# deepomicslab/PALACE

Measured on AMD Instinct MI355X. Metric: contigs/sec eref+generate_graph+matching, 1M-contig synth, 1/2/4/8 GPU, higher is better.
Workload: dtype u32

## Files before the change

include/palace_hip.h:

```cpp
#ifndef PALACE_HIP_H
#define PALACE_HIP_H

#include <stddef.h>
#include <stdint.h>

#ifdef __cplusplus
extern "C" {
#endif

#define PALACE_OK 0
#define PALACE_EINVAL (-1)
#define PALACE_EHIP (-2)
#define PALACE_ENOMEM (-3)
#define PALACE_ESTATE (-4)

typedef struct palace_ctx palace_ctx;

const char *palace_last_error(void);
const char *palace_version(void);

int palace_ctx_create(int device, palace_ctx **out);
int palace_ctx_create_prio(int device, int high_priority, palace_ctx **out);
int palace_ctx_create_on_stream(int device, void *hip_stream, palace_ctx **out);
int palace_ctx_destroy(palace_ctx *ctx);
int palace_sync(palace_ctx *ctx);
void *palace_stream(palace_ctx *ctx);
int palace_malloc(palace_ctx *ctx, size_t bytes, void **d_out);
int palace_free(palace_ctx *ctx, void *d_ptr);
int palace_memset(palace_ctx *ctx, void *d_ptr, int value, size_t bytes);
int palace_h2d(palace_ctx *ctx, void *d_dst, const void *h_src, size_t bytes);
int palace_d2h(palace_ctx *ctx, void *h_dst, const void *d_src, size_t bytes);
int palace_d2d(palace_ctx *ctx, void *d_dst, const void *d_src, size_t bytes);
int palace_host_alloc(palace_ctx *ctx, size_t bytes, void **h_out);
int palace_host_free(palace_ctx *ctx, void *h_ptr);
int palace_h2d_async(palace_ctx *ctx, void *d_dst, const void *h_src, size_t bytes);
int palace_d2h_async(palace_ctx *ctx, void *h_dst, const void *d_src, size_t bytes);
int palace_timer_begin(palace_ctx *ctx);
int palace_timer_end(palace_ctx *ctx, float *ms_out);
int palace_mark(palace_ctx *ctx, int i);
int palace_mark_elapsed(palace_ctx *ctx, int a, int b, float *ms_out);
int palace_mark_wait(palace_ctx *ctx, int i);
int palace_mark_wait_for(palace_ctx *ctx, int i, double seconds);
int palace_wait_for_mark(palace_ctx *ctx, palace_ctx *other, int i);


int palace_eref_set_coder(palace_ctx *ctx, const uint8_t header400[400]);

int palace_eref_index_refs(palace_ctx *ctx, const uint8_t *d_bases, const int64_t *d_offsets,
                           int64_t n_refs, uint32_t *d_out, const int64_t *d_out_offsets);

int palace_eref_table_reset(palace_ctx *ctx);
int palace_eref_reserve(palace_ctx *ctx, int64_t total_bases);
int palace_eref_count_reads(palace_ctx *ctx, const uint8_t *d_bases, const int64_t *d_offsets,
                            int64_t n_reads, const uint8_t *d_keep, int64_t total_bases);

size_t palace_eref_packed_bytes(int64_t n_positions);
int palace_eref_pack_reads(palace_ctx *ctx, const uint8_t *d_bases, const int64_t *d_offsets, int64_t n_reads,
                           const uint8_t *d_keep, int64_t total_bases, uint32_t *d_p0, uint32_t *d_p1, uint32_t *d_u);
int palace_eref_count_reads_packed(palace_ctx *ctx, const uint32_t *d_p0, const uint32_t *d_p1, const uint32_t *d_u,
                                   int64_t n_positions, int64_t n_reads_hint);

int palace_eref_set_count_mode(palace_ctx *ctx, int mode, int64_t bucket_cap);
int palace_eref_set_key_buckets(palace_ctx *ctx, const uint32_t mask128[4]);
int palace_eref_set_option(palace_ctx *ctx, const char *name, int64_t value);

int palace_eref_scan_refs(palace_ctx *ctx, const uint8_t *d_bases, const int64_t *d_offsets,
                          int64_t n_refs, int64_t total_bases, int one_min, int three_min,
                          int32_t *d_rows);

typedef struct palace_eref_probe_index palace_eref_probe_index;
int palace_eref_probe_index_build(palace_ctx *ctx, const uint8_t *d_bases, const int64_t *d_offsets, int64_t n_refs,
                                  int64_t total_bases, palace_eref_probe_index **out);
int palace_eref_probe_index_free(palace_ctx *ctx, palace_eref_probe_index *ix);
int palace_eref_scan_refs_indexed(palace_ctx *ctx, const palace_eref_probe_index *ix, const uint8_t *d_bases,
                                  const int64_t *d_offsets, int64_t n_refs, int64_t total_bases, int one_min,
                                  int three_min, int32_t *d_rows);

int palace_eref_attach_probe_index(palace_ctx *ctx, const palace_eref_probe_index *ix);

int palace_eref_entry_layout(const palace_eref_probe_index *ix, size_t *counts_bytes, size_t *hits_bytes);
int palace_eref_entry_buffers_attach(palace_ctx *ctx, palace_eref_probe_index *ix, void *d_counts, void *d_hits);
int palace_eref_entry_buffers(const palace_eref_probe_index *ix, void **d_counts, void **d_hits);
int palace_eref_entry_hits_from_counts(palace_ctx *ctx, const palace_eref_probe_index *ix, const void *d_parts, int n_parts, size_t part_stride,
                                       size_t off, size_t bytes);
int palace_eref_entry_hits_complete(palace_ctx *ctx, const palace_eref_probe_index *ix, int64_t keys_counted);
int palace_eref_entry_counts_valid(const palace_ctx *ctx, const palace_eref_probe_index *ix);


int palace_eref_table_planes(palace_ctx *ctx, void **d_planes3, size_t *bytes_per_plane);
int palace_eref_table_attach(palace_ctx *ctx, void *const d_planes3[3]);
int palace_eref_table_invalidate(palace_ctx *ctx);
int palace_eref_table_merge_slices(palace_ctx *ctx, const void *d_parts, int n_parts,
                                   size_t slice_off, size_t slice_bytes);

int palace_eref_table_pack_low(palace_ctx *ctx, void *d_low);
int palace_eref_table_merge_slices_packed(palace_ctx *ctx, const void *d_parts, int n_parts, size_t slice_off,
                                          size_t slice_bytes);

int palace_eref_plane_pack(palace_ctx *ctx, const uint32_t mask128[4], uint32_t *d_counts, uint16_t *d_keys, int64_t cap_keys,
                           unsigned long long *d_first);
int palace_eref_plane_unpack(palace_ctx *ctx, const uint32_t mask128[4], const uint32_t *d_counts, const uint16_t *d_keys, int64_t cap_keys,
                             unsigned long long *d_first);

int palace_eref_table_lookup(palace_ctx *ctx, const uint32_t *d_keys, int64_t n, uint8_t *d_counts);
int palace_eref_table_popcounts(palace_ctx *ctx, uint64_t out3[3]);


typedef struct {
    int32_t max_end;
    int32_t min_mapq;
    int32_t max_nm;
    int32_t enable_paired;
    int32_t both_order;
    int32_t reserved;
    double max_span_frac;
} palace_graph_params;

typedef struct {
    int64_t n;
    const int32_t *tid, *pos, *mtid, *mpos, *nm, *ref_len, *read_len, *clip_s, *clip_e;
    const uint16_t *flag;
    const uint8_t *mapq;
    const uint64_t *qkey;
    const int32_t *sa_off;
} palace_bam_cols;

typedef struct {
    int32_t tid2, pos2, mapq2, nm2, clip_s2, clip_e2, len2, rev2;
} palace_sa_item;

typedef struct {
    int64_t ord;
    uint64_t qkey;
    int32_t left, right;
    int32_t mtid, ref_len;
    int32_t dL, dR;
    int32_t nmL, nmR;
    int16_t mapqL, mapqR;
    uint8_t kind, cls, found, in_fastg, oL, oR, pad0, pad1;
    int32_t sa_index;
} palace_graph_cand;

typedef struct {
    int32_t left, right;
    uint32_t counts[4];
    uint8_t oL, oR, pad[6];
} palace_graph_edge;

int palace_graph_classify(palace_ctx *ctx, const palace_bam_cols *cols, const palace_sa_item *d_sa,
                          int32_t n_targets, const int32_t *d_tlen, const int32_t *d_trank,
                          const uint64_t *d_fastg, int64_t n_fastg, const palace_graph_params *prm,
                          int64_t ord_base, uint64_t *d_consumed, palace_graph_cand *d_cands,
                          int64_t cand_cap, int64_t *n_cands_out);

int palace_graph_classify_ex(palace_ctx *ctx, const palace_bam_cols *cols, const palace_sa_item *d_sa,
                             int32_t n_targets, const int32_t *d_tlen, const int32_t *d_trank,
                             const uint64_t *d_fastg, int64_t n_fastg, const palace_graph_params *prm,
                             int64_t ord_base, uint64_t *d_consumed, palace_graph_cand *d_cands,
                             int64_t cand_cap, int64_t *n_cands_out, int64_t *n_border_out);

int palace_graph_fastg_offsets(palace_ctx *ctx, const uint64_t *d_fastg, int64_t n_fastg, int32_t n_targets, uint32_t *d_first);
int palace_graph_classify_ix(palace_ctx *ctx, const palace_bam_cols *cols, const palace_sa_item *d_sa,
                             int32_t n_targets, const int32_t *d_tlen, const int32_t *d_trank,
                             const uint64_t *d_fastg, int64_t n_fastg, const uint32_t *d_fastg_first, const palace_graph_params *prm,
                             int64_t ord_base, uint64_t *d_consumed, palace_graph_cand *d_cands,
                             int64_t cand_cap, int64_t *n_cands_out, int64_t *n_border_out);

int palace_graph_resolve(palace_ctx *ctx, palace_graph_cand *d_cands, int64_t n_cands,
                         int64_t n_records_total, const palace_graph_params *prm, uint64_t *d_consumed,
                         palace_graph_edge *d_edges, int64_t edge_cap, int64_t *n_edges_out);

int palace_graph_resolve_ex(palace_ctx *ctx, palace_graph_cand *d_cands, int64_t n_cands, int64_t n_border,
                            int64_t n_records_total, const palace_graph_params *prm, uint64_t *d_consumed,
                            palace_graph_edge *d_edges, int64_t edge_cap, int64_t *d_n_edges, int64_t *n_edges_out);

int palace_graph_score_border(palace_ctx *ctx, palace_graph_cand *d_cands, int64_t n_cands, int64_t n_border,
                              const palace_graph_params *prm);

int palace_graph_copy_numbers(palace_ctx *ctx, const uint64_t *d_consumed, const int32_t *d_tlen,
                              int32_t n_targets, double avg_depth, int32_t *d_cn);


int palace_bgzf_inflate(palace_ctx *ctx, const uint8_t *d_in, int64_t n_members, const int64_t *d_in_off, const int32_t *d_in_len,
                        const int64_t *d_out_off, const int32_t *d_out_len, uint8_t *d_out, int32_t *d_status);


int palace_bgzf_deflate(palace_ctx *ctx, const uint8_t *d_text, int64_t n_members, const int64_t *d_off, const int32_t *d_len,
                        const uint32_t *d_crc, uint8_t *d_slots, int32_t *d_member_len);

int palace_bgzf_compact(palace_ctx *ctx, const uint8_t *d_slots, int64_t n_members, const int32_t *d_member_len, uint8_t *d_file,
                        int64_t *d_member_off);


int palace_crc32_members(palace_ctx *ctx, const uint8_t *d_data, int64_t n_members, const int64_t *d_off, const int32_t *d_len,
                         uint32_t *d_crc);

typedef struct {
    int64_t line, reads, bases;
    int32_t open, error;
} palace_fastq_cursor;

size_t palace_fastq_scratch_bytes(int64_t max_window);
int palace_fastq_parse(palace_ctx *ctx, const uint8_t *d_text, int64_t n, int final_window, palace_fastq_cursor *d_cursor,
                       uint8_t *d_bases, int64_t bases_cap, int64_t *d_offsets, int64_t offsets_cap, void *d_scratch,
                       size_t scratch_bytes);


typedef struct {
    int64_t stride, span, text_cap;
    int64_t check_guards;
} palace_gzip_params;

enum {
    PALACE_GZ_NONE = 0,
    PALACE_GZ_HEADER = 1,
    PALACE_GZ_DECODE = 2,
    PALACE_GZ_CHAIN_OPEN = 3,
    PALACE_GZ_NO_PROGRESS = 4,
    PALACE_GZ_TOO_BIG = 5,
    PALACE_GZ_TRUNCATED = 6,
    PALACE_GZ_CRC = 7,
    PALACE_GZ_ISIZE = 8,
    PALACE_GZ_TRAILING = 9,
    PALACE_GZ_SINK = 10,
    PALACE_GZ_MARKER = 11
};

typedef struct {
    int64_t chunks_found, chunks_accepted, false_hits, rounds, members, spans, batches, text_bytes;
    int32_t fallback, guards_bad;
    double ms_upload, ms_find, ms_size, ms_decode, ms_chain, ms_resolve, ms_crc, ms_sink;
} palace_gzip_stats;

typedef int (*palace_gzip_sink)(void *user, const uint8_t *d_text, int64_t n, int last);

int palace_gzip_inflate(palace_ctx *ctx, const uint8_t *file, int64_t size, const palace_gzip_params *prm, palace_gzip_sink sink,
                        void *user, palace_gzip_stats *stats);


int palace_depth_sum_covered(palace_ctx *ctx, int64_t n_segs, const int32_t *d_seg_tid, const int32_t *d_seg_pos,
                             const int32_t *d_seg_len, int32_t n_targets, const int32_t *d_tlen, const int64_t *d_tbase,
                             int64_t total_len, uint64_t *sum_out, uint64_t *covered_out);

int palace_depth_per_contig(palace_ctx *ctx, int64_t n_segs, const int32_t *d_seg_tid, const int32_t *d_seg_pos,
                            const int32_t *d_seg_len, int32_t n_targets, const int32_t *d_tlen, const int64_t *d_tbase,
                            int64_t total_len, uint64_t *sum_out, uint64_t *covered_out, uint64_t *d_contig_sum,
                            uint64_t *d_contig_covered);

typedef struct palace_depth_text palace_depth_text;
int palace_depth_text_create(palace_ctx *ctx, int64_t n_segs, const int32_t *d_seg_tid, const int32_t *d_seg_pos,
                             const int32_t *d_seg_len, int32_t n_targets, const int32_t *d_tlen, const int64_t *d_tbase,
                             int64_t total_len, const uint8_t *d_names, const int64_t *d_name_off, palace_depth_text **out,
                             uint64_t *text_bytes_out, uint64_t *lines_out, uint64_t *sum_out);
int palace_depth_text_destroy(palace_ctx *ctx, palace_depth_text *dt);
int palace_depth_text_emit(palace_ctx *ctx, const palace_depth_text *dt, uint64_t text_begin, uint64_t text_end, uint8_t *d_out);
int palace_depth_text_windows(palace_ctx *ctx, const palace_depth_text *dt, int64_t n_windows, const int64_t *d_win_beg,
                              const int64_t *d_win_end, uint64_t *d_text_beg, uint64_t *d_text_end, uint64_t *d_lines);


int palace_match_greedy(palace_ctx *ctx, int32_t n_vertices, int64_t n_arcs, const int32_t *d_src,
                        const int32_t *d_dst, const int64_t *d_out_off, const int32_t *d_out_arcs,
                        const int64_t *d_in_off, const int32_t *d_in_arcs, const uint8_t *d_alive,
                        int32_t *d_next, int32_t *d_prev, int32_t *d_next_arc, int32_t *rounds_out);

int palace_match_arcs_from_edges(const int32_t *cn, int32_t n_segs, const palace_graph_edge *edges, int64_t n_edges,
                                 int32_t min_count, int64_t *copies, int32_t *src, int32_t *dst, int64_t *weight,
                                 int64_t *n_arcs_out);

typedef struct palace_match_result palace_match_result;
int palace_match_set_option(palace_ctx *ctx, const char *name, int64_t value);
int palace_match_decompose(palace_ctx *ctx, int32_t n_segs, const int64_t *copies, int64_t n_arcs,
                           const int32_t *src, const int32_t *dst, int32_t iterations, int32_t aggressive,
                           palace_match_result **out);
int palace_match_decompose_ex(palace_ctx *ctx, int32_t n_segs, const int64_t *copies, int64_t n_arcs,
                              const int32_t *src, const int32_t *dst, int32_t iterations, int32_t aggressive,
                              int32_t compact, palace_match_result **out);
const uint64_t *palace_match_result_bare(const palace_match_result *r);
int64_t palace_match_result_bare_count(const palace_match_result *r);
int64_t palace_match_result_count(const palace_match_result *r);
const int64_t *palace_match_result_offsets(const palace_match_result *r);
const int32_t *palace_match_result_verts(const palace_match_result *r);
const uint8_t *palace_match_result_kind(const palace_match_result *r);
const int32_t *palace_match_result_iter(const palace_match_result *r);
const int32_t *palace_match_result_open_at(const palace_match_result *r);
void palace_match_result_free(palace_match_result *r);


typedef struct {
    int32_t n_segs;
    int32_t min_count;
    const uint8_t *seed;
    const int32_t *tlen;
    const int32_t *rank;
    const int32_t *name_len;
    int64_t n_paths;
    const int64_t *path_off;
    const int32_t *path_tok;
} palace_stage04_inputs;

typedef struct palace_stage04 palace_stage04;
int palace_stage04_create(palace_ctx *ctx, const palace_stage04_inputs *in, palace_stage04 **out);
int palace_stage04_destroy(palace_ctx *ctx, palace_stage04 *s);

int palace_stage04_reserve(palace_ctx *ctx, palace_stage04 *s, int64_t edge_bound);

int palace_stage04_filter(palace_ctx *ctx, palace_stage04 *s, const palace_graph_edge *d_edges, const int64_t *d_n_edges,
                          int64_t edge_bound);
int palace_stage04_flags(palace_ctx *ctx, palace_stage04 *s, uint8_t *h_seg_flags, uint8_t *h_edge_flags, int64_t n_edges);
int palace_stage04_counts(palace_ctx *ctx, palace_stage04 *s, int64_t counts[8]);

int palace_stage04_match(palace_ctx *ctx, palace_stage04 *s, const palace_graph_edge *d_edges, const int32_t *d_cn,
                         int32_t iterations, int32_t aggressive, int32_t use_paths);
int palace_stage04_result(palace_ctx *ctx, palace_stage04 *s, palace_match_result **out, const int32_t **contig_of_out,
                          int64_t *n_segs_filtered_out);

#ifdef __cplusplus
}
#endif
#endif
```

palace_amd/capi.py:

```python
from __future__ import annotations

import ctypes as C
import os
import subprocess

import numpy as np

_HERE = os.path.dirname(os.path.abspath(__file__))
SO_PATH = os.environ.get("PALACE_HIP_SO") or os.path.join(_HERE, "libpalace_hip.so")
_LIB = None


class PalaceError(RuntimeError):
    pass


def build(force: bool = False) -> str:
    args = ["make", "-C", os.path.join(_HERE, "csrc")]
    if force:
        subprocess.run(args + ["clean"], check=True, stdout=subprocess.DEVNULL)
    subprocess.run(args, check=True, stdout=subprocess.DEVNULL)
    return SO_PATH


class GraphParams(C.Structure):
    _fields_ = [("max_end", C.c_int32), ("min_mapq", C.c_int32), ("max_nm", C.c_int32), ("enable_paired", C.c_int32),
                ("both_order", C.c_int32), ("reserved", C.c_int32), ("max_span_frac", C.c_double)]

    @classmethod
    def default(cls):
        return cls(300, 0, 5, 1, 0, 0, 0.80)


class BamCols(C.Structure):
    _fields_ = [("n", C.c_int64)] + [(k, C.c_void_p) for k in
                                     ("tid", "pos", "mtid", "mpos", "nm", "ref_len", "read_len", "clip_s", "clip_e",
                                      "flag", "mapq", "qkey", "sa_off")]


class GzipParams(C.Structure):
    _fields_ = [("stride", C.c_int64), ("span", C.c_int64), ("text_cap", C.c_int64), ("check_guards", C.c_int64)]


class GzipStats(C.Structure):
    _fields_ = [(k, C.c_int64) for k in ("chunks_found", "chunks_accepted", "false_hits", "rounds", "members", "spans", "batches", "text_bytes")] + \
        [("fallback", C.c_int32), ("guards_bad", C.c_int32)] + \
        [(k, C.c_double) for k in ("ms_upload", "ms_find", "ms_size", "ms_decode", "ms_chain", "ms_resolve", "ms_crc", "ms_sink")]


GZIP_SINK = C.CFUNCTYPE(C.c_int, C.c_void_p, C.c_void_p, C.c_int64, C.c_int)


class Stage04Inputs(C.Structure):
    _fields_ = [("n_segs", C.c_int32), ("min_count", C.c_int32), ("seed", C.c_void_p), ("tlen", C.c_void_p), ("rank", C.c_void_p),
                ("name_len", C.c_void_p), ("n_paths", C.c_int64), ("path_off", C.c_void_p), ("path_tok", C.c_void_p)]


SA_ITEM_DTYPE = np.dtype([(k, np.int32) for k in ("tid2", "pos2", "mapq2", "nm2", "clip_s2", "clip_e2", "len2", "rev2")])
CAND_DTYPE = np.dtype([("ord", np.int64), ("qkey", np.uint64), ("left", np.int32), ("right", np.int32),
                       ("mtid", np.int32), ("ref_len", np.int32), ("dL", np.int32), ("dR", np.int32),
                       ("nmL", np.int32), ("nmR", np.int32), ("mapqL", np.int16), ("mapqR", np.int16),
                       ("kind", np.uint8), ("cls", np.uint8), ("found", np.uint8), ("in_fastg", np.uint8),
                       ("oL", np.uint8), ("oR", np.uint8), ("pad0", np.uint8), ("pad1", np.uint8), ("sa_index", np.int32)])
EDGE_DTYPE = np.dtype([("left", np.int32), ("right", np.int32), ("counts", np.uint32, 4), ("oL", np.uint8),
                       ("oR", np.uint8), ("pad", np.uint8, 6)])
FASTQ_CURSOR_DTYPE = np.dtype([("line", np.int64), ("reads", np.int64), ("bases", np.int64), ("open", np.int32), ("error", np.int32)])
assert CAND_DTYPE.itemsize == 64 and EDGE_DTYPE.itemsize == 32 and SA_ITEM_DTYPE.itemsize == 32

_SIGS = {
    "palace_ctx_create": [C.c_int, C.POINTER(C.c_void_p)],
    "palace_ctx_create_prio": [C.c_int, C.c_int, C.POINTER(C.c_void_p)],
    "palace_ctx_create_on_stream": [C.c_int, C.c_void_p, C.POINTER(C.c_void_p)],
    "palace_ctx_destroy": [C.c_void_p],
    "palace_sync": [C.c_void_p],
    "palace_malloc": [C.c_void_p, C.c_size_t, C.POINTER(C.c_void_p)],
    "palace_free": [C.c_void_p, C.c_void_p],
    "palace_memset": [C.c_void_p, C.c_void_p, C.c_int, C.c_size_t],
    "palace_h2d": [C.c_void_p, C.c_void_p, C.c_void_p, C.c_size_t],
    "palace_d2h": [C.c_void_p, C.c_void_p, C.c_void_p, C.c_size_t],
    "palace_d2d": [C.c_void_p, C.c_void_p, C.c_void_p, C.c_size_t],
    "palace_host_alloc": [C.c_void_p, C.c_size_t, C.POINTER(C.c_void_p)],
    "palace_host_free": [C.c_void_p, C.c_void_p],
    "palace_d2h_async": [C.c_void_p, C.c_void_p, C.c_void_p, C.c_size_t],
    "palace_h2d_async": [C.c_void_p, C.c_void_p, C.c_void_p, C.c_size_t],
    "palace_mark_wait": [C.c_void_p, C.c_int],
    "palace_mark_wait_for": [C.c_void_p, C.c_int, C.c_double],
    "palace_wait_for_mark": [C.c_void_p, C.c_void_p, C.c_int],
    "palace_timer_begin": [C.c_void_p],
    "palace_timer_end": [C.c_void_p, C.POINTER(C.c_float)],
    "palace_mark": [C.c_void_p, C.c_int],
    "palace_mark_elapsed": [C.c_void_p, C.c_int, C.c_int, C.POINTER(C.c_float)],
    "palace_eref_set_coder": [C.c_void_p, C.c_void_p],
    "palace_eref_index_refs": [C.c_void_p, C.c_void_p, C.c_void_p, C.c_int64, C.c_void_p, C.c_void_p],
    "palace_eref_table_reset": [C.c_void_p],
    "palace_eref_reserve": [C.c_void_p, C.c_int64],
    "palace_eref_count_reads": [C.c_void_p, C.c_void_p, C.c_void_p, C.c_int64, C.c_void_p, C.c_int64],
    "palace_eref_pack_reads": [C.c_void_p, C.c_void_p, C.c_void_p, C.c_int64, C.c_void_p, C.c_int64, C.c_void_p, C.c_void_p, C.c_void_p],
    "palace_eref_count_reads_packed": [C.c_void_p, C.c_void_p, C.c_void_p, C.c_void_p, C.c_int64, C.c_int64],
    "palace_eref_set_count_mode": [C.c_void_p, C.c_int, C.c_int64],
    "palace_eref_set_key_buckets": [C.c_void_p, C.c_void_p],
    "palace_eref_set_option": [C.c_void_p, C.c_char_p, C.c_int64],
    "palace_eref_scan_refs": [C.c_void_p, C.c_void_p, C.c_void_p, C.c_int64, C.c_int64, C.c_int, C.c_int,
                              C.c_void_p],
    "palace_eref_probe_index_build": [C.c_void_p, C.c_void_p, C.c_void_p, C.c_int64, C.c_int64, C.POINTER(C.c_void_p)],
    "palace_eref_attach_probe_index": [C.c_void_p, C.c_void_p],
    "palace_eref_entry_layout": [C.c_void_p, C.POINTER(C.c_size_t), C.POINTER(C.c_size_t)],
    "palace_eref_entry_buffers_attach": [C.c_void_p, C.c_void_p, C.c_void_p, C.c_void_p],
    "palace_eref_entry_buffers": [C.c_void_p, C.POINTER(C.c_void_p), C.POINTER(C.c_void_p)],
    "palace_eref_entry_hits_from_counts": [C.c_void_p, C.c_void_p, C.c_void_p, C.c_int, C.c_size_t, C.c_size_t, C.c_size_t],
    "palace_eref_entry_hits_complete": [C.c_void_p, C.c_void_p, C.c_int64],
    "palace_eref_entry_counts_valid": [C.c_void_p, C.c_void_p],
    "palace_eref_probe_index_free": [C.c_void_p, C.c_void_p],
    "palace_eref_scan_refs_indexed": [C.c_void_p, C.c_void_p, C.c_void_p, C.c_void_p, C.c_int64, C.c_int64, C.c_int, C.c_int,
                                      C.c_void_p],
    "palace_eref_table_planes": [C.c_void_p, C.POINTER(C.c_void_p), C.POINTER(C.c_size_t)],
    "palace_eref_table_attach": [C.c_void_p, C.POINTER(C.c_void_p)],
    "palace_eref_table_invalidate": [C.c_void_p],
    "palace_eref_table_merge_slices": [C.c_void_p, C.c_void_p, C.c_int, C.c_size_t, C.c_size_t],
    "palace_eref_table_merge_slices_packed": [C.c_void_p, C.c_void_p, C.c_int, C.c_size_t, C.c_size_t],
    "palace_eref_table_pack_low": [C.c_void_p, C.c_void_p],
    "palace_eref_plane_pack": [C.c_void_p, C.c_void_p, C.c_void_p, C.c_void_p, C.c_int64, C.c_void_p],
    "palace_eref_plane_unpack": [C.c_void_p, C.c_void_p, C.c_void_p, C.c_void_p, C.c_int64, C.c_void_p],
    "palace_eref_table_lookup": [C.c_void_p, C.c_void_p, C.c_int64, C.c_void_p],
    "palace_eref_table_popcounts": [C.c_void_p, C.POINTER(C.c_uint64)],
    "palace_graph_classify": [C.c_void_p, C.POINTER(BamCols), C.c_void_p, C.c_int32, C.c_void_p, C.c_void_p,
                              C.c_void_p, C.c_int64, C.POINTER(GraphParams), C.c_int64, C.c_void_p, C.c_void_p,
                              C.c_int64, C.POINTER(C.c_int64)],
    "palace_depth_sum_covered": [C.c_void_p, C.c_int64, C.c_void_p, C.c_void_p, C.c_void_p, C.c_int32, C.c_void_p, C.c_void_p, C.c_int64,
                                 C.POINTER(C.c_uint64), C.POINTER(C.c_uint64)],
    "palace_depth_per_contig": [C.c_void_p, C.c_int64, C.c_void_p, C.c_void_p, C.c_void_p, C.c_int32, C.c_void_p, C.c_void_p, C.c_int64,
                                C.POINTER(C.c_uint64), C.POINTER(C.c_uint64), C.c_void_p, C.c_void_p],
    "palace_graph_copy_numbers": [C.c_void_p, C.c_void_p, C.c_void_p, C.c_int32, C.c_double, C.c_void_p],
    "palace_match_greedy": [C.c_void_p, C.c_int32, C.c_int64] + [C.c_void_p] * 10 + [C.POINTER(C.c_int32)],
    "palace_match_arcs_from_edges": [C.c_void_p, C.c_int32, C.c_void_p, C.c_int64, C.c_int32, C.c_void_p, C.c_void_p,
                                     C.c_void_p, C.c_void_p, C.POINTER(C.c_int64)],
    "palace_match_set_option": [C.c_void_p, C.c_char_p, C.c_int64],
    "palace_match_decompose": [C.c_void_p, C.c_int32, C.c_void_p, C.c_int64, C.c_void_p, C.c_void_p, C.c_int32,
                               C.c_int32, C.POINTER(C.c_void_p)],
    "palace_match_decompose_ex": [C.c_void_p, C.c_int32, C.c_void_p, C.c_int64, C.c_void_p, C.c_void_p, C.c_int32,
                                  C.c_int32, C.c_int32, C.POINTER(C.c_void_p)],
    "palace_graph_resolve": [C.c_void_p, C.c_void_p, C.c_int64, C.c_int64, C.POINTER(GraphParams), C.c_void_p,
                             C.c_void_p, C.c_int64, C.POINTER(C.c_int64)],
    "palace_graph_classify_ex": [C.c_void_p, C.POINTER(BamCols), C.c_void_p, C.c_int32, C.c_void_p, C.c_void_p,
                                 C.c_void_p, C.c_int64, C.POINTER(GraphParams), C.c_int64, C.c_void_p, C.c_void_p,
                                 C.c_int64, C.POINTER(C.c_int64), C.POINTER(C.c_int64)],
    "palace_graph_classify_ix": [C.c_void_p, C.POINTER(BamCols), C.c_void_p, C.c_int32, C.c_void_p, C.c_void_p,
                                 C.c_void_p, C.c_int64, C.c_void_p, C.POINTER(GraphParams), C.c_int64, C.c_void_p, C.c_void_p,
                                 C.c_int64, C.POINTER(C.c_int64), C.POINTER(C.c_int64)],
    "palace_graph_fastg_offsets": [C.c_void_p, C.c_void_p, C.c_int64, C.c_int32, C.c_void_p],
    "palace_bgzf_inflate": [C.c_void_p, C.c_void_p, C.c_int64, C.c_void_p, C.c_void_p, C.c_void_p, C.c_void_p, C.c_void_p, C.c_void_p],
    "palace_fastq_scratch_bytes": [C.c_int64],
    "palace_crc32_members": [C.c_void_p, C.c_void_p, C.c_int64, C.c_void_p, C.c_void_p, C.c_void_p],
    "palace_bgzf_deflate": [C.c_void_p, C.c_void_p, C.c_int64, C.c_void_p, C.c_void_p, C.c_void_p, C.c_void_p, C.c_void_p],
    "palace_bgzf_compact": [C.c_void_p, C.c_void_p, C.c_int64, C.c_void_p, C.c_void_p, C.c_void_p],
    "palace_depth_text_create": [C.c_void_p, C.c_int64, C.c_void_p, C.c_void_p, C.c_void_p, C.c_int32, C.c_void_p, C.c_void_p, C.c_int64,
                                 C.c_void_p, C.c_void_p, C.POINTER(C.c_void_p), C.POINTER(C.c_uint64), C.POINTER(C.c_uint64), C.POINTER(C.c_uint64)],
    "palace_depth_text_destroy": [C.c_void_p, C.c_void_p],
    "palace_depth_text_emit": [C.c_void_p, C.c_void_p, C.c_uint64, C.c_uint64, C.c_void_p],
    "palace_depth_text_windows": [C.c_void_p, C.c_void_p, C.c_int64, C.c_void_p, C.c_void_p, C.c_void_p, C.c_void_p, C.c_void_p],
    "palace_gzip_inflate": [C.c_void_p, C.c_void_p, C.c_int64, C.POINTER(GzipParams), GZIP_SINK, C.c_void_p, C.POINTER(GzipStats)],
    "palace_fastq_parse": [C.c_void_p, C.c_void_p, C.c_int64, C.c_int, C.c_void_p, C.c_void_p, C.c_int64, C.c_void_p, C.c_int64,
                           C.c_void_p, C.c_size_t],
    "palace_graph_score_border": [C.c_void_p, C.c_void_p, C.c_int64, C.c_int64, C.POINTER(GraphParams)],
    "palace_graph_resolve_ex": [C.c_void_p, C.c_void_p, C.c_int64, C.c_int64, C.c_int64, C.POINTER(GraphParams), C.c_void_p,
                                C.c_void_p, C.c_int64, C.c_void_p, C.POINTER(C.c_int64)],
    "palace_stage04_create": [C.c_void_p, C.POINTER(Stage04Inputs), C.POINTER(C.c_void_p)],
    "palace_stage04_destroy": [C.c_void_p, C.c_void_p],
    "palace_stage04_reserve": [C.c_void_p, C.c_void_p, C.c_int64],
    "palace_stage04_filter": [C.c_void_p, C.c_void_p, C.c_void_p, C.c_void_p, C.c_int64],
    "palace_stage04_flags": [C.c_void_p, C.c_void_p, C.c_void_p, C.c_void_p, C.c_int64],
    "palace_stage04_counts": [C.c_void_p, C.c_void_p, C.POINTER(C.c_int64)],
    "palace_stage04_match": [C.c_void_p, C.c_void_p, C.c_void_p, C.c_void_p, C.c_int32, C.c_int32, C.c_int32],
    "palace_stage04_result": [C.c_void_p, C.c_void_p, C.POINTER(C.c_void_p), C.POINTER(C.c_void_p), C.POINTER(C.c_int64)],
}


def declared_symbols():
    import re
    text = open(os.path.join(_HERE, "..", "include", "palace_hip.h")).read()
    text = re.sub(r"/\*.*?\*/", "", text, flags=re.S)
    return sorted(set(re.findall(r"\b(palace_[a-z0-9_]+)\s*\(", text)))


def lib() -> C.CDLL:
    global _LIB
    if _LIB is None:
        if not os.path.exists(SO_PATH):
            raise PalaceError(f"{SO_PATH} is missing: run `python -c 'import __graft_entry__ as g; g.build()'` "
                              "(hipcc --offload-arch=gfx950). There is no CPU fallback.")
        _LIB = C.CDLL(SO_PATH)
        _LIB.palace_last_error.restype = C.c_char_p
        _LIB.palace_version.restype = C.c_char_p
        _LIB.palace_stream.restype = C.c_void_p
        _LIB.palace_stream.argtypes = [C.c_void_p]
        _LIB.palace_eref_packed_bytes.restype = C.c_size_t
        _LIB.palace_eref_packed_bytes.argtypes = [C.c_int64]
        for nm, rt in (("count", C.c_int64), ("bare_count", C.c_int64), ("bare", C.POINTER(C.c_uint64)), ("offsets", C.POINTER(C.c_int64)), ("verts", C.POINTER(C.c_int32)),
                       ("kind", C.POINTER(C.c_uint8)), ("iter", C.POINTER(C.c_int32)), ("open_at", C.POINTER(C.c_int32))):
            fn = getattr(_LIB, "palace_match_result_" + nm)
            fn.argtypes = [C.c_void_p]
            fn.restype = rt
        _LIB.palace_match_result_free.argtypes = [C.c_void_p]
        _LIB.palace_match_result_free.restype = None
        for name, sig in _SIGS.items():
            fn = getattr(_LIB, name)
            fn.argtypes = sig
            fn.restype = C.c_int
        _LIB.palace_fastq_scratch_bytes.restype = C.c_size_t
    return _LIB


def _check(rc: int, what: str):
    if rc != 0:
        raise PalaceError(f"{what} -> {rc}: {lib().palace_last_error().decode()}")


class DevBuf:

    def __init__(self, ctx: "Ctx", nbytes: int, dtype=np.uint8, shape=None):
        self.ctx, self.nbytes, self.dtype, self.shape = ctx, int(nbytes), np.dtype(dtype), shape
        p = C.c_void_p()
        _check(lib().palace_malloc(ctx.h, self.nbytes, C.byref(p)), "palace_malloc")
        self.ptr = p.value

    def to_host(self) -> np.ndarray:
        out = np.empty(self.nbytes // self.dtype.itemsize, dtype=self.dtype)
        _check(lib().palace_d2h(self.ctx.h, out.ctypes.data, self.ptr, self.nbytes), "palace_d2h")
        return out.reshape(self.shape) if self.shape is not None else out

    def free(self):
        if self.ptr:
            lib().palace_free(self.ctx.h, self.ptr)
            self.ptr = None


class Ctx:

    def __init__(self, device: int = 0, high_priority: bool = False, stream: int | None = None):
        h = C.c_void_p()
        if stream:
            _check(lib().palace_ctx_create_on_stream(device, C.c_void_p(stream), C.byref(h)), "palace_ctx_create_on_stream")
        else:
            _check(lib().palace_ctx_create_prio(device, int(high_priority), C.byref(h)), "palace_ctx_create_prio")
        self.h = h
        self.device = device

    def close(self):
        if self.h:
            lib().palace_ctx_destroy(self.h)
            self.h = None

    def __enter__(self):
        return self

    def __exit__(self, *a):
        self.close()

    def upload(self, arr: np.ndarray) -> DevBuf:
        a = np.ascontiguousarray(arr)
        b = DevBuf(self, max(a.nbytes, 1), a.dtype, a.shape)
        if a.nbytes:
            _check(lib().palace_h2d(self.h, b.ptr, a.ctypes.data, a.nbytes), "palace_h2d")
        return b

    def empty(self, shape, dtype) -> DevBuf:
        n = int(np.prod(shape)) * np.dtype(dtype).itemsize
        return DevBuf(self, max(n, 1), dtype, tuple(np.atleast_1d(shape)))

    def d2d(self, dst_ptr: int, src_ptr: int, nbytes: int):
        _check(lib().palace_d2d(self.h, dst_ptr, src_ptr, nbytes), "palace_d2d")

    def sync(self):
        _check(lib().palace_sync(self.h), "palace_sync")

    def timer_begin(self):
        _check(lib().palace_timer_begin(self.h), "palace_timer_begin")

    def timer_end(self) -> float:
        ms = C.c_float()
        _check(lib().palace_timer_end(self.h, C.byref(ms)), "palace_timer_end")
        return ms.value

    def mark(self, i: int):
        _check(lib().palace_mark(self.h, i), "palace_mark")

    def mark_wait(self, i: int):
        _check(lib().palace_mark_wait(self.h, i), "palace_mark_wait")

    def wait_for_mark(self, other: "Ctx", i: int):
        _check(lib().palace_wait_for_mark(self.h, other.h, i), "palace_wait_for_mark")

    def mark_elapsed(self, a: int, b: int) -> float:
        ms = C.c_float()
        _check(lib().palace_mark_elapsed(self.h, a, b, C.byref(ms)), "palace_mark_elapsed")
        return ms.value

    @property
    def stream(self) -> int:
        return lib().palace_stream(self.h)

    def eref_set_coder(self, header400: np.ndarray):
        h = np.ascontiguousarray(header400, dtype=np.uint8)
        assert h.size == 400
        _check(lib().palace_eref_set_coder(self.h, h.ctypes.data), "palace_eref_set_coder")

    def eref_table_reset(self):
        _check(lib().palace_eref_table_reset(self.h), "palace_eref_table_reset")

    def eref_count_reads(self, d_bases: DevBuf, d_offsets: DevBuf, n_reads: int, d_keep: DevBuf | None = None,
                         total_bases: int = -1):
        _check(lib().palace_eref_count_reads(self.h, d_bases.ptr, d_offsets.ptr, n_reads,
                                             d_keep.ptr if d_keep else None, total_bases), "palace_eref_count_reads")

    def eref_pack_reads(self, d_bases: DevBuf, d_offsets: DevBuf, n_reads: int, d_keep, total_bases: int, d_p0: DevBuf, d_p1: DevBuf, d_u: DevBuf):
        _check(lib().palace_eref_pack_reads(self.h, d_bases.ptr, d_offsets.ptr, n_reads, d_keep.ptr if d_keep else None, total_bases,
                                            d_p0.ptr, d_p1.ptr, d_u.ptr), "palace_eref_pack_reads")

    def eref_count_reads_packed(self, d_p0: DevBuf, d_p1: DevBuf, d_u: DevBuf, n_positions: int, n_reads_hint: int = 0):
        _check(lib().palace_eref_count_reads_packed(self.h, d_p0.ptr, d_p1.ptr, d_u.ptr, n_positions, n_reads_hint),
               "palace_eref_count_reads_packed")

    def eref_set_count_mode(self, mode: int, bucket_cap: int = 0):
        _check(lib().palace_eref_set_count_mode(self.h, mode, bucket_cap), "palace_eref_set_count_mode")

    def eref_set_key_buckets(self, buckets=None):
        m = (C.c_uint32 * 4)(*([0xFFFFFFFF] * 4 if buckets is None else [0] * 4))
        for b in ([] if buckets is None else buckets):
            m[b >> 5] |= 1 << (b & 31)
        _check(lib().palace_eref_set_key_buckets(self.h, m), "palace_eref_set_key_buckets")

    def eref_set_option(self, name: str, value: int):
        _check(lib().palace_eref_set_option(self.h, name.encode(), value), "palace_eref_set_option")

    def eref_scan_refs(self, d_bases: DevBuf, d_offsets: DevBuf, n_refs: int, total_bases: int,
                       one_min: int, three_min: int, d_rows: DevBuf):
        _check(lib().palace_eref_scan_refs(self.h, d_bases.ptr, d_offsets.ptr, n_refs, total_bases,
                                           one_min, three_min, d_rows.ptr), "palace_eref_scan_refs")

    def eref_probe_index_build(self, d_bases: DevBuf, d_offsets: DevBuf, n_refs: int, total_bases: int) -> C.c_void_p:
        h = C.c_void_p()
        _check(lib().palace_eref_probe_index_build(self.h, d_bases.ptr, d_offsets.ptr, n_refs, total_bases, C.byref(h)),
               "palace_eref_probe_index_build")
        return h

    def eref_attach_probe_index(self, index):
        _check(lib().palace_eref_attach_probe_index(self.h, index), "palace_eref_attach_probe_index")

    def eref_entry_layout(self, index):
        cb, hb = C.c_size_t(), C.c_size_t()
        _check(lib().palace_eref_entry_layout(index, C.byref(cb), C.byref(hb)), "palace_eref_entry_layout")
        return int(cb.value), int(hb.value)

    def eref_entry_buffers_attach(self, index, counts_ptr: int | None, hits_ptr: int | None):
        _check(lib().palace_eref_entry_buffers_attach(self.h, index, counts_ptr, hits_ptr), "palace_eref_entry_buffers_attach")

    def eref_entry_hits_from_counts(self, index, parts_ptr: int, n_parts: int, part_stride: int, off: int, nbytes: int):
        _check(lib().palace_eref_entry_hits_from_counts(self.h, index, parts_ptr, n_parts, part_stride, off, nbytes), "palace_eref_entry_hits_from_counts")

    def eref_entry_counts_valid(self, index) -> bool:
        return bool(lib().palace_eref_entry_counts_valid(self.h, index))

    def eref_entry_hits_complete(self, index, keys_counted: int = -1):
        _check(lib().palace_eref_entry_hits_complete(self.h, index, keys_counted), "palace_eref_entry_hits_complete")

    def eref_probe_index_free(self, index: C.c_void_p):
        _check(lib().palace_eref_probe_index_free(self.h, index), "palace_eref_probe_index_free")

    def eref_scan_refs_indexed(self, index: C.c_void_p, d_bases: DevBuf, d_offsets: DevBuf, n_refs: int, total_bases: int,
                               one_min: int, three_min: int, d_rows: DevBuf):
        _check(lib().palace_eref_scan_refs_indexed(self.h, index, d_bases.ptr, d_offsets.ptr, n_refs, total_bases,
                                                   one_min, three_min, d_rows.ptr), "palace_eref_scan_refs_indexed")

    def eref_index_refs(self, d_bases: DevBuf, d_offsets: DevBuf, n_refs: int, d_out: DevBuf, d_out_offsets: DevBuf):
        _check(lib().palace_eref_index_refs(self.h, d_bases.ptr, d_offsets.ptr, n_refs, d_out.ptr,
                                            d_out_offsets.ptr), "palace_eref_index_refs")

    def eref_table_lookup(self, keys: np.ndarray) -> np.ndarray:
        k = self.upload(np.ascontiguousarray(keys, dtype=np.uint32))
        out = self.empty(len(keys), np.uint8)
        _check(lib().palace_eref_table_lookup(self.h, k.ptr, len(keys), out.ptr), "palace_eref_table_lookup")
        res = out.to_host()
        k.free()
        out.free()
        return res

    def eref_table_popcounts(self):
        out = (C.c_uint64 * 3)()
        _check(lib().palace_eref_table_popcounts(self.h, out), "palace_eref_table_popcounts")
        return [int(v) for v in out]

    def eref_table_planes(self):
        ptrs = (C.c_void_p * 3)()
        nbytes = C.c_size_t()
        _check(lib().palace_eref_table_planes(self.h, ptrs, C.byref(nbytes)), "palace_eref_table_planes")
        return [int(p) for p in ptrs], int(nbytes.value)

    def eref_table_attach(self, ptrs):
        arr = (C.c_void_p * 3)(*[int(p) for p in ptrs])
        _check(lib().palace_eref_table_attach(self.h, arr), "palace_eref_table_attach")

    def match_set_option(self, name: str, value: int):
        _check(lib().palace_match_set_option(self.h, name.encode(), value), "palace_match_set_option")

    def eref_table_invalidate(self):
        _check(lib().palace_eref_table_invalidate(self.h), "palace_eref_table_invalidate")

    def eref_table_merge_slices(self, parts_ptr: int, n_parts: int, slice_off: int, slice_bytes: int, packed: bool = False):
        fn = lib().palace_eref_table_merge_slices_packed if packed else lib().palace_eref_table_merge_slices
        _check(fn(self.h, parts_ptr, n_parts, slice_off, slice_bytes), "palace_eref_table_merge_slices")

    def eref_table_pack_low(self, low_ptr: int):
        _check(lib().palace_eref_table_pack_low(self.h, low_ptr), "palace_eref_table_pack_low")

    @staticmethod
    def _bucket_mask(buckets):
        m = (C.c_uint32 * 4)(0, 0, 0, 0)
        for b in buckets:
            m[b >> 5] |= 1 << (b & 31)
        return m

    def eref_plane_pack(self, buckets, counts_ptr: int, keys_ptr: int, cap_keys: int, first_ptr: int):
        _check(lib().palace_eref_plane_pack(self.h, self._bucket_mask(buckets), counts_ptr, keys_ptr, cap_keys, first_ptr), "palace_eref_plane_pack")

    def eref_plane_unpack(self, buckets, counts_ptr: int, keys_ptr: int, cap_keys: int, first_ptr: int):
        _check(lib().palace_eref_plane_unpack(self.h, self._bucket_mask(buckets), counts_ptr, keys_ptr, cap_keys, first_ptr), "palace_eref_plane_unpack")

    def crc32_members(self, d_data_ptr: int, n_members: int, d_off: DevBuf, d_len: DevBuf, d_crc: DevBuf):
        _check(lib().palace_crc32_members(self.h, d_data_ptr, n_members, d_off.ptr, d_len.ptr, d_crc.ptr), "palace_crc32_members")

    def bgzf_deflate(self, d_text_ptr: int, n_members: int, d_off: DevBuf, d_len: DevBuf, d_crc: DevBuf, d_slots: DevBuf, d_member_len: DevBuf):
        _check(lib().palace_bgzf_deflate(self.h, d_text_ptr, n_members, d_off.ptr, d_len.ptr, d_crc.ptr, d_slots.ptr, d_member_len.ptr),
               "palace_bgzf_deflate")

    def bgzf_compact(self, d_slots: DevBuf, n_members: int, d_member_len: DevBuf, d_file: DevBuf, d_member_off: DevBuf):
        _check(lib().palace_bgzf_compact(self.h, d_slots.ptr, n_members, d_member_len.ptr, d_file.ptr, d_member_off.ptr), "palace_bgzf_compact")

    def fastq_parse(self, d_text_ptr: int, n: int, final_window: bool, d_cursor: DevBuf, d_bases: DevBuf, bases_cap: int,
                    d_offsets: DevBuf, offsets_cap: int, d_scratch: DevBuf):
        _check(lib().palace_fastq_parse(self.h, d_text_ptr, n, int(final_window), d_cursor.ptr, d_bases.ptr, bases_cap, d_offsets.ptr,
                                        offsets_cap, d_scratch.ptr, d_scratch.nbytes), "palace_fastq_parse")


def fastq_scratch_bytes(max_window: int) -> int:
    return int(lib().palace_fastq_scratch_bytes(max_window))


def crc32_members(ctx: Ctx, data: bytes, lengths) -> np.ndarray:
    lens = np.asarray(lengths, dtype=np.int32)
    offs = np.concatenate([[0], np.cumsum(lens, dtype=np.int64)[:-1]]).astype(np.int64) if len(lens) else np.zeros(0, np.int64)
    d_data = ctx.upload(np.frombuffer(bytes(data), dtype=np.uint8) if len(data) else np.zeros(1, np.uint8))
    d_off, d_len, d_crc = ctx.upload(offs), ctx.upload(lens), ctx.empty(max(1, len(lens)), np.uint32)
    try:
        ctx.crc32_members(d_data.ptr, len(lens), d_off, d_len, d_crc)
        return d_crc.to_host()[:len(lens)]
    finally:
        for b in (d_data, d_off, d_len, d_crc):
            b.free()


def bgzf_deflate(ctx: Ctx, pieces, lead: int = 0):
    lens = np.array([len(p) for p in pieces], dtype=np.int32)
    n = len(lens)
    offs = (lead + np.concatenate([[0], np.cumsum(lens, dtype=np.int64)[:-1]])).astype(np.int64) if n else np.zeros(0, np.int64)
    blob = bytes(lead) + b"".join(bytes(p) for p in pieces) + bytes(4)
    bufs = [ctx.upload(np.frombuffer(blob, dtype=np.uint8)), ctx.upload(offs if n else np.zeros(1, np.int64)),
            ctx.upload(lens if n else np.zeros(1, np.int32)), ctx.empty(max(1, n), np.uint32), ctx.empty(max(1, n) * 65536, np.uint8),
            ctx.empty(max(1, n), np.int32), ctx.empty(max(1, n) * 65536, np.uint8), ctx.empty(n + 1, np.int64)]
    d_text, d_off, d_len, d_crc, d_slots, d_mlen, d_file, d_moff = bufs
    try:
        ctx.crc32_members(d_text.ptr, n, d_off, d_len, d_crc)
        ctx.bgzf_deflate(d_text.ptr, n, d_off, d_len, d_crc, d_slots, d_mlen)
        ctx.bgzf_compact(d_slots, n, d_mlen, d_file, d_moff)
        moff = d_moff.to_host()
        return d_file.to_host()[:int(moff[-1])].tobytes(), moff
    finally:
        for b in bufs:
            b.free()


def gzip_inflate(ctx: Ctx, blob: bytes, stride: int = 0, span: int = 0, text_cap: int = 0, check_guards: bool = False):
    blob = bytes(blob)
    parts, seen_last = [], []

    def take(_user, d_text, n, last):
        if n:
            part = np.empty(n, np.uint8)
            if lib().palace_d2h(ctx.h, part.ctypes.data, d_text, n):
                return 1
            parts.append(part.tobytes())
        if last:
            seen_last.append(True)
        return 0

    prm = GzipParams(stride, span, text_cap, int(check_guards))
    st = GzipStats()
    buf = np.frombuffer(blob, dtype=np.uint8) if blob else np.zeros(1, np.uint8)
    _check(lib().palace_gzip_inflate(ctx.h, buf.ctypes.data, len(blob), C.byref(prm), GZIP_SINK(take), None, C.byref(st)), "palace_gzip_inflate")
    stats = {k: getattr(st, k) for k, _ in GzipStats._fields_}
    text = b"".join(parts) if stats["fallback"] == 0 and seen_last else None
    return text, stats


def fastq_read_set(ctx: Ctx, text: bytes, cuts=(), reads0: int = 0, bases0: int = 0):
    text = bytes(text)
    bounds = [0] + [c for c in cuts if 0 < c < len(text)] + [len(text)]
    widest = max(b - a for a, b in zip(bounds, bounds[1:])) if len(bounds) > 1 else 0
    bases_cap = bases0 + len(text) + 1
    offsets_cap = reads0 + len(text) // 4 + 3
    d_win = DevBuf(ctx, max(16, widest + 16))
    d_bases, d_offsets = DevBuf(ctx, bases_cap), ctx.empty(offsets_cap, np.int64)
    d_scratch = DevBuf(ctx, fastq_scratch_bytes(widest))
    cur = np.zeros(1, FASTQ_CURSOR_DTYPE)
    cur["reads"], cur["bases"] = reads0, bases0
    d_cur = ctx.upload(cur)
    try:
        first = np.zeros(1, np.int64)
        first[0] = bases0
        _check(lib().palace_h2d(ctx.h, d_offsets.ptr + 8 * reads0, first.ctypes.data, 8), "palace_h2d")
        for k, (a, b) in enumerate(zip(bounds, bounds[1:])):
            chunk = np.frombuffer(text[a:b], dtype=np.uint8)
            if len(chunk):
                _check(lib().palace_h2d(ctx.h, d_win.ptr, chunk.ctypes.data, len(chunk)), "palace_h2d")
            ctx.fastq_parse(d_win.ptr, len(chunk), k == len(bounds) - 2, d_cur, d_bases, bases_cap, d_offsets, offsets_cap, d_scratch)
            ctx.sync()
        cur = d_cur.to_host()[0]
        if cur["error"]:
            raise PalaceError("palace_fastq_parse: capacity exceeded")
        n_reads = int(cur["reads"]) - reads0
        offsets = d_offsets.to_host()[reads0:reads0 + n_reads + 1].copy()
        bases = d_bases.to_host()[bases0:int(cur["bases"])].copy()
        return bases, offsets, cur
    finally:
        for buf in (d_win, d_bases, d_offsets, d_scratch, d_cur):
            buf.free()


_ARC_BUFFERS = {}


def match_arcs_from_edges(cn: np.ndarray, edges: np.ndarray, min_count: int = 5, reuse: bool = False):
    cn = np.ascontiguousarray(cn, dtype=np.int32)
    e = np.ascontiguousarray(edges, dtype=EDGE_DTYPE)
    key = (len(cn), len(e))
    if reuse and key in _ARC_BUFFERS:
        copies, src, dst, w = _ARC_BUFFERS[key]
    else:
        copies = np.empty(len(cn), np.int64)
        src = np.empty(2 * len(e), np.int32); dst = np.empty(2 * len(e), np.int32); w = np.empty(2 * len(e), np.int64)
        if reuse:
            _ARC_BUFFERS.clear()
            _ARC_BUFFERS[key] = (copies, src, dst, w)
    n = C.c_int64()
    _check(lib().palace_match_arcs_from_edges(cn.ctypes.data, len(cn), e.ctypes.data, len(e), min_count, copies.ctypes.data,
                                              src.ctypes.data, dst.ctypes.data, w.ctypes.data, C.byref(n)),
           "palace_match_arcs_from_edges")
    return copies, src[:n.value], dst[:n.value], w[:n.value]


class MatchResult:

    def __init__(self, handle):
        L = lib()
        self._h = handle
        n = self.n = L.palace_match_result_count(handle)
        self.off = np.ctypeslib.as_array(L.palace_match_result_offsets(handle), shape=(n + 1,))
        nv = int(self.off[-1])
        self.verts = np.ctypeslib.as_array(L.palace_match_result_verts(handle), shape=(max(nv, 1),))[:nv]
        mk = lambda f, dt: (np.ctypeslib.as_array(f(handle), shape=(max(n, 1),))[:n] if n else np.zeros(0, dt))
        self.kind = mk(L.palace_match_result_kind, np.uint8)
        self.iter = mk(L.palace_match_result_iter, np.int32)
        self.open_at = mk(L.palace_match_result_open_at, np.int32)

    def free(self):
        if self._h is not None:
            self.off = self.verts = self.kind = self.iter = self.open_at = None
            lib().palace_match_result_free(self._h)
            self._h = None

    def __enter__(self):
        return self

    def __exit__(self, *exc):
        self.free()


def match_decompose_views(ctx: "Ctx", copies: np.ndarray, src: np.ndarray, dst: np.ndarray, iterations: int = 10,
                          aggressive: bool = False, compact: bool = False) -> MatchResult:
    cp = np.ascontiguousarray(copies, dtype=np.int64)
    s = np.ascontiguousarray(src, dtype=np.int32)
    d = np.ascontiguousarray(dst, dtype=np.int32)
    res = C.c_void_p()
    _check(lib().palace_match_decompose_ex(ctx.h, len(cp), cp.ctypes.data, len(s), s.ctypes.data, d.ctypes.data,
                                           iterations, int(aggressive), int(compact), C.byref(res)), "palace_match_decompose")
    r = MatchResult(res)
    if compact:
        r.n_bare = int(lib().palace_match_result_bare_count(res))
        words = (len(cp) + 63) // 64
        r.bare = np.ctypeslib.as_array(lib().palace_match_result_bare(res), shape=(max(1, words),))[:words]
    return r


def match_decompose(ctx: "Ctx", copies: np.ndarray, src: np.ndarray, dst: np.ndarray, iterations: int = 10,
                    aggressive: bool = False):
    with match_decompose_views(ctx, copies, src, dst, iterations, aggressive) as r:
        return r.off.copy(), r.verts.copy(), r.kind.copy(), r.iter.copy(), r.open_at.copy()


class Stage04:
    COUNT_NAMES = ("edges", "juncs", "kept_pass2", "kept_pass3_more", "segs_selected", "segs_rescued", "arcs", "segs_filtered")

    def __init__(self, ctx: "Ctx", seed, tlen, rank, name_len, path_off, path_tok, min_count: int = 5):
        self.ctx = ctx
        self._keep = [np.ascontiguousarray(seed, np.uint8), np.ascontiguousarray(tlen, np.int32), np.ascontiguousarray(rank, np.int32),
                      np.ascontiguousarray(name_len, np.int32), np.ascontiguousarray(path_off, np.int64),
                      np.ascontiguousarray(path_tok, np.int32)]
        sd, tl, rk, nl, po, pt = self._keep
        assert len(sd) == len(tl) == len(rk) == len(nl) and len(po) >= 1
        inp = Stage04Inputs(len(sd), min_count, sd.ctypes.data, tl.ctypes.data, rk.ctypes.data, nl.ctypes.data, len(po) - 1,
                            po.ctypes.data, pt.ctypes.data if len(pt) else None)
        h = C.c_void_p()
        _check(lib().palace_stage04_create(ctx.h, C.byref(inp), C.byref(h)), "palace_stage04_create")
        self.h, self.n_segs = h, len(sd)

    def filter(self, d_edges_ptr: int, d_n_edges_ptr: int, edge_bound: int):
        _check(lib().palace_stage04_filter(self.ctx.h, self.h, d_edges_ptr, d_n_edges_ptr, edge_bound), "palace_stage04_filter")

    def counts(self) -> dict:
        out = (C.c_int64 * 8)()
        _check(lib().palace_stage04_counts(self.ctx.h, self.h, out), "palace_stage04_counts")
        return dict(zip(self.COUNT_NAMES, (int(v) for v in out)))

    def flags(self, n_edges: int):
        seg = np.zeros(self.n_segs, np.uint8)
        edge = np.zeros(n_edges, np.uint8)
        _check(lib().palace_stage04_flags(self.ctx.h, self.h, seg.ctypes.data, edge.ctypes.data if n_edges else None, n_edges),
               "palace_stage04_flags")
        return seg, edge

    def match(self, d_edges_ptr: int, d_cn_ptr: int, iterations: int = 10, aggressive: bool = False, use_paths: bool = True):
        _check(lib().palace_stage04_match(self.ctx.h, self.h, d_edges_ptr, d_cn_ptr, iterations, int(aggressive), int(use_paths)), "palace_stage04_match")

    def result(self):
        res, cof, n = C.c_void_p(), C.c_void_p(), C.c_int64()
        _check(lib().palace_stage04_result(self.ctx.h, self.h, C.byref(res), C.byref(cof), C.byref(n)), "palace_stage04_result")
        r = MatchResult(res)
        r.n_bare = int(lib().palace_match_result_bare_count(res))
        words = (n.value + 63) // 64
        r.bare = np.ctypeslib.as_array(lib().palace_match_result_bare(res), shape=(max(1, words),))[:words]
        contig_of = np.ctypeslib.as_array(C.cast(cof, C.POINTER(C.c_int32)), shape=(max(1, n.value),))[: n.value]
        return r, contig_of

    def close(self):
        if self.h:
            lib().palace_stage04_destroy(self.ctx.h, self.h)
            self.h = None


def window_minimums(hit_ratio: float, perfect_ratio: float):
    w = np.float32(500)
    return int(w * np.float32(hit_ratio)), int(w * np.float32(perfect_ratio))
```

palace_amd/csrc/decomp.hip:

```cpp
#include "decomp.hpp"

#include <algorithm>

namespace palace {

namespace {

constexpr uint64_t kNoKey = ~0ull;
constexpr uint64_t kClosed = 0;
constexpr int kStampShift = 42;
constexpr int kPackedShift = 52, kPackedStamps = 1 << (64 - kPackedShift);
constexpr uint64_t kLenMask = (1ull << 40) - 1;


__device__ __forceinline__ uint64_t wave_incl_scan(uint64_t v, int lane)
{
#pragma unroll
    for (int d = 1; d < 64; d <<= 1) {
        const uint64_t u = __shfl_up(v, d);
        if (lane >= d) v += u;
    }
    return v;
}

constexpr int kMaxWaves = 16;

__device__ void scan_partials_body(const uint64_t *__restrict__ in, int64_t n, uint64_t *__restrict__ partials, int blk, int nblk)
{
    __shared__ uint64_t part[kMaxWaves];
    const int64_t chunk = (n + nblk - 1) / nblk;
    const int64_t a = min(n, static_cast<int64_t>(blk) * chunk), e = min(n, a + chunk);
    uint64_t s = 0;
    for (int64_t i = a + threadIdx.x; i < e; i += blockDim.x) s += in[i];
    const int lane = threadIdx.x & 63, waves = static_cast<int>(blockDim.x >> 6);
    s = wave_incl_scan(s, lane);
    if (lane == 63) part[threadIdx.x >> 6] = s;
    __syncthreads();
    if (threadIdx.x == 0) {
        uint64_t t = 0;
        for (int w = 0; w < waves; w++) t += part[w];
        partials[blk] = t;
    }
    __syncthreads();
}

__device__ void scan_prefix_body(uint64_t *__restrict__ partials, int n_parts, uint64_t *__restrict__ total)
{
    __shared__ uint64_t part[kMaxWaves];
    const int lane = threadIdx.x & 63, wv = threadIdx.x >> 6;
    const uint64_t x = static_cast<int>(threadIdx.x) < n_parts ? partials[threadIdx.x] : 0;
    const uint64_t incl = wave_incl_scan(x, lane);
    if (lane == 63) part[wv] = incl;
    __syncthreads();
    uint64_t before = 0;
    for (int w = 0; w < wv; w++) before += part[w];
    if (static_cast<int>(threadIdx.x) < n_parts) partials[threadIdx.x] = before + incl - x;
    if (threadIdx.x == blockDim.x - 1) *total = before + incl;
    __syncthreads();
}

__device__ void scan_apply_body(const uint64_t *__restrict__ in, uint64_t *__restrict__ out, int64_t n, const uint64_t *__restrict__ partials,
                                int blk, int nblk)
{
    __shared__ uint64_t part[kMaxWaves];
    const int64_t chunk = (n + nblk - 1) / nblk;
    const int64_t a = min(n, static_cast<int64_t>(blk) * chunk), e = min(n, a + chunk);
    const int lane = threadIdx.x & 63, wv = threadIdx.x >> 6, waves = static_cast<int>(blockDim.x >> 6);
    uint64_t carry = partials[blk];
    for (int64_t base = a; base < e; base += blockDim.x) {
        const int64_t i = base + threadIdx.x;
        const uint64_t x = i < e ? in[i] : 0;
        const uint64_t incl = wave_incl_scan(x, lane);
        if (lane == 63) part[wv] = incl;
        __syncthreads();
        uint64_t before = 0, all = 0;
        for (int w = 0; w < waves; w++) { if (w < wv) before += part[w]; all += part[w]; }
        if (i < e) out[i] = carry + before + incl - x;
        carry += all;
        __syncthreads();
    }
}

__global__ __launch_bounds__(kDecompBlock) void scan_partials_kernel(const uint64_t *__restrict__ in, const int32_t *__restrict__ n_dev,
                                                                     uint64_t *__restrict__ partials)
{
    scan_partials_body(in, *n_dev, partials, static_cast<int>(blockIdx.x), static_cast<int>(gridDim.x));
}
__global__ __launch_bounds__(kDecompBlock) void scan_prefix_kernel(uint64_t *__restrict__ partials, int n_parts, uint64_t *__restrict__ total)
{
    scan_prefix_body(partials, n_parts, total);
}
__global__ __launch_bounds__(kDecompBlock) void scan_apply_kernel(const uint64_t *__restrict__ in, uint64_t *__restrict__ out,
                                                                  const int32_t *__restrict__ n_dev, const uint64_t *__restrict__ partials)
{
    scan_apply_body(in, out, *n_dev, partials, static_cast<int>(blockIdx.x), static_cast<int>(gridDim.x));
}

struct Span { int tid, n; };
__device__ __forceinline__ Span whole_grid() { return Span{static_cast<int>(blockIdx.x * blockDim.x + threadIdx.x), static_cast<int>(gridDim.x * blockDim.x)}; }

__device__ void ph_init(const DecompBufs &b, Span T, int64_t comp_cap, int64_t vert_cap, int n_flags, int allow_packed)
{
    DecompState *st = b.st;
    const int V = st->V;
    for (int i = T.tid; i < V; i += T.n) { b.bo_hi[i] = kNoKey; b.bi_hi[i] = kNoKey; b.on_path[i] = 0; }
    for (int i = T.tid; i < n_flags; i += T.n) b.changed[i] = 0;
    if (T.tid == 0) {
        st->n_comp = 0; st->n_vert = 0; st->comp_cap = comp_cap; st->vert_cap = vert_cap;
        st->unsettled = 0; st->overflow = 0; st->bad = 0; st->dead = 0; st->scan_total = 0; st->alive_after = 0;
        st->packed = (allow_packed && b.kc && b.pack_bad && *b.pack_bad == 0) ? 1u : 0u;
        if (comp_cap >= 0) b.o_off[0] = 0;
    }
}

__device__ void ph_round_begin(const DecompBufs &b, Span T, int reset_left)
{
    const int V = b.st->V;
    if (!reset_left && b.st->dead) return;
    if (T.tid == 0) { b.st->alive_after = 0; if (reset_left) b.st->dead = 0; }
    const int64_t E = b.st->E;
    for (int64_t e = T.tid; e < E; e += T.n) b.done[e] = 0;
    const bool packed = b.st->packed != 0;
    for (int i = T.tid; i < V; i += T.n) {
        const int s = i >> 1;
        const int64_t l = reset_left ? 1 : b.left[s];
        if (reset_left && !(i & 1)) b.left[s] = 1;
        b.alive[i] = l > 0;
        b.next[i] = -1; b.prev[i] = -1;
        b.bo_hi[i] = b.bi_hi[i] = l > 0 ? kNoKey : kClosed;
        if (!packed) { b.bo_lo[i] = kNoKey; b.bo_lo[V + i] = kNoKey; b.bi_lo[i] = kNoKey; b.bi_lo[V + i] = kNoKey; }
        b.len_a[i] = 0;
    }
}

struct IterArgs {
    uint64_t stamp;
    uint64_t stamp_p;
    int parity;
    int prev_flag, flag;
    int unique_hi;
};


__device__ void ph_propose_hi(const DecompBufs &b, Span T, const IterArgs &a)
{
    if (b.st->dead) return;
    if (a.prev_flag >= 0 && !b.changed[a.prev_flag]) return;
    const int64_t E = b.st->E;
    const int V = b.st->V;
    const int other = (a.parity ^ 1) * V;
    const bool packed = b.st->packed != 0;
    for (int64_t e = T.tid; e < E; e += T.n) {
        if (b.done[e]) continue;
        const int u = b.src[e], v = b.dst[e];
        if (b.bi_hi[v] == kClosed) { b.done[e] = 1; continue; }
        const uint64_t k = packed ? (a.stamp_p | b.kc[e]) : (a.stamp | b.khi[e]);
        if (atomicMin(reinterpret_cast<unsigned long long *>(&b.bo_hi[u]), static_cast<unsigned long long>(k)) == kClosed) { b.done[e] = 1; continue; }
        atomicMin(reinterpret_cast<unsigned long long *>(&b.bi_hi[v]), static_cast<unsigned long long>(k));
        if (!a.unique_hi && !packed) { b.bo_lo[other + u] = kNoKey; b.bi_lo[other + v] = kNoKey; }
    }
}

__device__ void ph_propose_lo(const DecompBufs &b, Span T, const IterArgs &a)
{
    if (b.st->dead) return;
    if (a.prev_flag >= 0 && !b.changed[a.prev_flag]) return;
    if (b.st->packed) return;
    const int64_t E = b.st->E;
    const int mine = a.parity * b.st->V;
    for (int64_t e = T.tid; e < E; e += T.n) {
        if (b.done[e]) continue;
        const int u = b.src[e], v = b.dst[e];
        const uint64_t k = a.stamp | b.khi[e], lo = b.klo[e];
        if (b.bo_hi[u] == k) atomicMin(reinterpret_cast<unsigned long long *>(&b.bo_lo[mine + u]), static_cast<unsigned long long>(lo));
        if (b.bi_hi[v] == k) atomicMin(reinterpret_cast<unsigned long long *>(&b.bi_lo[mine + v]), static_cast<unsigned long long>(lo));
    }
}

__device__ void ph_commit_flag(const DecompBufs &b, Span T, const IterArgs &a, volatile unsigned int *took);
__device__ void ph_commit(const DecompBufs &b, Span T, const IterArgs &a)
{
    if (b.st->dead) return;
    if (a.prev_flag >= 0 && !b.changed[a.prev_flag]) return;
    ph_commit_flag(b, T, a, b.changed + a.flag);
}
__device__ void ph_commit_flag(const DecompBufs &b, Span T, const IterArgs &a, volatile unsigned int *took)
{
    bool any = false;
    const int64_t E = b.st->E;
    const int mine = a.parity * b.st->V;
    const bool packed = b.st->packed != 0;
    for (int64_t e = T.tid; e < E; e += T.n) {
        if (b.done[e]) continue;
        const int u = b.src[e], v = b.dst[e];
        const uint64_t k = packed ? (a.stamp_p | b.kc[e]) : (a.stamp | b.khi[e]);
        if (b.bo_hi[u] != k || b.bi_hi[v] != k) continue;
        const uint64_t lo = b.klo[e];
        if (!a.unique_hi && !packed && (b.bo_lo[mine + u] != lo || b.bi_lo[mine + v] != lo)) continue;
        b.next[u] = v; b.prev[v] = u;
        b.nhi[u] = b.khi[e]; b.nlo[u] = lo;
        b.bo_hi[u] = kClosed; b.bi_hi[v] = kClosed;
        b.done[e] = 1;
        any = true;
    }
    if (__syncthreads_or(any) && threadIdx.x == 0) *took = 1u;
}

__device__ void ph_heads(const DecompBufs &b, Span T, int round, int last_flag)
{
    DecompState *st = b.st;
    if (st->dead) return;
    if (T.tid == 0 && last_flag >= 0 && b.changed[last_flag]) st->unsettled = 1;
    const int V = st->V;
    for (int v = T.tid; v < V; v += T.n) {
        if (!b.alive[v] || b.prev[v] >= 0) continue;
        int len = 0, last = v;
        int64_t least = b.left[v >> 1];
        for (int x = v; x >= 0; x = b.next[x]) {
            b.on_path[x] = round + 1;
            last = x;
            len++;
            least = min(least, b.left[x >> 1]);
        }
        const int twin_first = last ^ 1;
        if (v > twin_first) continue;
        const int64_t uses = twin_first == v ? 2 : 1;
        b.len_a[v] = (1ull << 40) | static_cast<uint64_t>(len);
        b.pay[v] = max(static_cast<int64_t>(1), least / uses);
        b.kind[v] = 0;
        b.open_at[v] = 0;
    }
}

__device__ void ph_cycles(const DecompBufs &b, Span T, int round)
{
    const int V = b.st->V;
    if (b.st->dead) return;
    for (int v = T.tid; v < V; v += T.n) {
        if (!b.alive[v] || b.on_path[v] == round + 1) continue;
        int len = 1, twin_least = v ^ 1, worst = 0;
        uint64_t whi = b.nhi[v], wlo = b.nlo[v];
        int64_t least = b.left[v >> 1];
        bool first = true;
        for (int x = b.next[v]; x != v; x = b.next[x]) {
            if (x < v) { first = false; break; }
            twin_least = min(twin_least, x ^ 1);
            const uint64_t hi = b.nhi[x], lo = b.nlo[x];
            if (hi > whi || (hi == whi && lo > wlo)) { whi = hi; wlo = lo; worst = len; }
            least = min(least, b.left[x >> 1]);
            len++;
        }
        if (!first || v > twin_least) continue;
        const int64_t uses = twin_least == v ? 2 : 1;
        b.len_a[v] = (1ull << 40) | static_cast<uint64_t>(len);
        b.pay[v] = max(static_cast<int64_t>(1), least / uses);
        b.kind[v] = 1;
        b.open_at[v] = (worst + 1) % len;
    }
}

__device__ void ph_emit(const DecompBufs &b, Span T, int round, int64_t c0, int64_t v0)
{
    DecompState *st = b.st;
    const int V = st->V;
    if (st->dead) return;
    int64_t alive = 0;
    for (int v = T.tid; v < V; v += T.n) {
        const uint64_t la = b.len_a[v];
        if (!la) continue;
        const int64_t len = static_cast<int64_t>(la & kLenMask);
        const uint64_t p = b.pos[v];
        const int64_t c = c0 + static_cast<int64_t>(p >> 40), at = v0 + static_cast<int64_t>(p & kLenMask);
        const int64_t pay = b.pay[v];
        const bool room = c < st->comp_cap && at + len <= st->vert_cap;
        if (!room) st->overflow = 1;
        else { b.o_off[c] = at; b.o_kind[c] = b.kind[v]; b.o_iter[c] = round; b.o_open[c] = b.open_at[v]; }
        int x = v;
        int64_t still = 0;
        for (int64_t k = 0; k < len; k++) {
            if (room) b.o_verts[at + k] = 2 * b.orig[x >> 1] + (x & 1);
            const int64_t l = b.left[x >> 1];
            b.left[x >> 1] = max(static_cast<int64_t>(0), l - pay);
            still += l - pay > 0;
            x = b.next[x];
        }
        alive += still;
    }
    __shared__ unsigned long long wg_alive;
    if (threadIdx.x == 0) wg_alive = 0;
    __syncthreads();
    if (alive) atomicAdd(&wg_alive, static_cast<unsigned long long>(alive));
    __syncthreads();
    if (threadIdx.x == 0 && wg_alive) atomicAdd(reinterpret_cast<unsigned long long *>(&st->alive_after), wg_alive);
}


__global__ void dec_init_kernel(DecompBufs b, int64_t comp_cap, int64_t vert_cap, int n_flags, int allow_packed) { ph_init(b, whole_grid(), comp_cap, vert_cap, n_flags, allow_packed); }
__global__ void dec_round_begin_kernel(DecompBufs b, int reset_left) { ph_round_begin(b, whole_grid(), reset_left); }
__global__ void dec_propose_hi_kernel(DecompBufs b, IterArgs a) { ph_propose_hi(b, whole_grid(), a); }
__global__ void dec_propose_lo_kernel(DecompBufs b, IterArgs a) { ph_propose_lo(b, whole_grid(), a); }
__global__ void dec_commit_kernel(DecompBufs b, IterArgs a) { ph_commit(b, whole_grid(), a); }
__global__ void dec_heads_kernel(DecompBufs b, int round, int last_flag) { ph_heads(b, whole_grid(), round, last_flag); }
__global__ void dec_cycles_kernel(DecompBufs b, int round) { ph_cycles(b, whole_grid(), round); }
__global__ void dec_emit_kernel(DecompBufs b, int round) { ph_emit(b, whole_grid(), round, b.st->n_comp, b.st->n_vert); }

__global__ void dec_round_end_kernel(DecompBufs b)
{
    DecompState *st = b.st;
    if (blockIdx.x || threadIdx.x || st->dead) return;
    st->dead = st->alive_after == 0;
    st->n_comp += static_cast<int64_t>(st->scan_total >> 40);
    st->n_vert += static_cast<int64_t>(st->scan_total & kLenMask);
    if (st->n_comp <= st->comp_cap) b.o_off[st->n_comp] = st->n_vert;
}

size_t up256(size_t v) { return (v + 255) / 256 * 256; }

struct Carver {
    char *base;
    size_t used = 0;
    template <class T>
    T *take(size_t n)
    {
        T *p = base ? reinterpret_cast<T *>(base + used) : nullptr;
        used += up256(std::max<size_t>(1, n) * sizeof(T));
        return p;
    }
};

size_t carve_all(DecompBufs &b, char *base, int64_t s_cap, int64_t e_cap, int64_t comp_cap, int64_t vert_cap, int rounds, int iters)
{
    Carver c{base};
    const size_t S = static_cast<size_t>(std::max<int64_t>(1, s_cap)), V = 2 * S, E = static_cast<size_t>(std::max<int64_t>(1, e_cap));
    b.st = c.take<DecompState>(1);
    b.src = c.take<int32_t>(E); b.dst = c.take<int32_t>(E);
    b.khi = c.take<uint64_t>(E); b.klo = c.take<uint64_t>(E);
    b.done = c.take<uint8_t>(E);
    b.kc = c.take<uint64_t>(E);
    b.left = c.take<int64_t>(S); b.orig = c.take<int32_t>(S);
    b.next = c.take<int32_t>(V); b.prev = c.take<int32_t>(V); b.on_path = c.take<int32_t>(V); b.open_at = c.take<int32_t>(V);
    b.nhi = c.take<uint64_t>(V); b.nlo = c.take<uint64_t>(V);
    b.bo_hi = c.take<uint64_t>(V); b.bi_hi = c.take<uint64_t>(V);
    b.bo_lo = c.take<uint64_t>(2 * V); b.bi_lo = c.take<uint64_t>(2 * V);
    b.len_a = c.take<uint64_t>(V); b.pos = c.take<uint64_t>(V);
    b.pay = c.take<int64_t>(V);
    b.alive = c.take<uint8_t>(V); b.kind = c.take<uint8_t>(V);
    b.partials = c.take<uint64_t>(kDecompGrid + 1);
    b.changed = c.take<uint32_t>(static_cast<size_t>(rounds) * static_cast<size_t>(iters));
    b.o_off = c.take<int64_t>(static_cast<size_t>(comp_cap) + 1);
    b.o_verts = c.take<int32_t>(static_cast<size_t>(vert_cap));
    b.o_iter = c.take<int32_t>(static_cast<size_t>(comp_cap));
    b.o_open = c.take<int32_t>(static_cast<size_t>(comp_cap));
    b.o_kind = c.take<uint8_t>(static_cast<size_t>(comp_cap));
    return c.used;
}

}

size_t decomp_bytes(int64_t s_cap, int64_t e_cap, int64_t comp_cap, int64_t vert_cap, int rounds, int iters)
{
    DecompBufs tmp;
    return carve_all(tmp, nullptr, s_cap, e_cap, comp_cap, vert_cap, rounds, iters);
}

void decomp_carve(DecompBufs &b, char *base, int64_t s_cap, int64_t e_cap, int64_t comp_cap, int64_t vert_cap, int rounds, int iters)
{
    carve_all(b, base, s_cap, e_cap, comp_cap, vert_cap, rounds, iters);
}

int scan_u64(palace_ctx *ctx, const uint64_t *in, uint64_t *out, const int32_t *n_dev, uint64_t *partials, uint64_t *total_dev)
{
    hipLaunchKernelGGL(scan_partials_kernel, dim3(kDecompGrid), dim3(kDecompBlock), 0, ctx->stream, in, n_dev, partials);
    hipLaunchKernelGGL(scan_prefix_kernel, dim3(1), dim3(kDecompBlock), 0, ctx->stream, partials, kDecompGrid, total_dev);
    hipLaunchKernelGGL(scan_apply_kernel, dim3(kDecompGrid), dim3(kDecompBlock), 0, ctx->stream, in, out, n_dev, partials);
    PALACE_HIP_TRY(hipGetLastError());
    return PALACE_OK;
}

namespace {

const dim3 kBlock(kDecompBlock);
constexpr int kWideGridDefault = 2048;
inline dim3 wide_grid(const palace_ctx *ctx) { return dim3(ctx->match_grid > 0 ? ctx->match_grid : kWideGridDefault); }

void enqueue_iterations(palace_ctx *ctx, const DecompBufs &b, int first, int n, uint64_t *count, int flag0, bool unique_hi)
{
    for (int k = 0; k < n; k++) {
        IterArgs a{((1ull << 21) - 1 - *count) << kStampShift, static_cast<uint64_t>((kPackedStamps - 1 - *count) & (kPackedStamps - 1)) << kPackedShift,
                   (first + k) & 1, k ? flag0 + k - 1 : -1, flag0 + k, unique_hi ? 1 : 0};
        (*count)++;
        hipLaunchKernelGGL(dec_propose_hi_kernel, wide_grid(ctx), kBlock, 0, ctx->stream, b, a);
        if (!unique_hi) hipLaunchKernelGGL(dec_propose_lo_kernel, wide_grid(ctx), kBlock, 0, ctx->stream, b, a);
        hipLaunchKernelGGL(dec_commit_kernel, wide_grid(ctx), kBlock, 0, ctx->stream, b, a);
    }
}

int enqueue_read_off(palace_ctx *ctx, const DecompBufs &b, int round, int last_flag)
{
    hipLaunchKernelGGL(dec_heads_kernel, wide_grid(ctx), kBlock, 0, ctx->stream, b, round, last_flag);
    hipLaunchKernelGGL(dec_cycles_kernel, wide_grid(ctx), kBlock, 0, ctx->stream, b, round);
    int rc = scan_u64(ctx, b.len_a, b.pos, &b.st->V, b.partials, &b.st->scan_total);
    if (rc) return rc;
    hipLaunchKernelGGL(dec_emit_kernel, wide_grid(ctx), kBlock, 0, ctx->stream, b, round);
    hipLaunchKernelGGL(dec_round_end_kernel, dim3(1), dim3(64), 0, ctx->stream, b);
    PALACE_HIP_TRY(hipGetLastError());
    return PALACE_OK;
}

}

int decomp_begin(palace_ctx *ctx, const DecompBufs &b, int rounds, int64_t comp_cap, int64_t vert_cap)
{
    PALACE_REQUIRE(rounds >= 1 && rounds <= kMaxRounds, "round count out of range");
    static_assert(kDecompGrid <= kDecompBlock, "scan_prefix_kernel scans the block sums with one workgroup");
    const int allow_packed = !ctx->match_two_word_keys && static_cast<int64_t>(rounds) * kMaxIters < kPackedStamps ? 1 : 0;
    hipLaunchKernelGGL(dec_init_kernel, wide_grid(ctx), kBlock, 0, ctx->stream, b, comp_cap, vert_cap, rounds * kMaxIters, allow_packed);
    PALACE_HIP_TRY(hipGetLastError());
    return PALACE_OK;
}

int decomp_rounds(palace_ctx *ctx, const DecompBufs &b, int t0, int t1, int rounds, int aggressive, int iters, bool unique_hi,
                  uint64_t *count)
{
    PALACE_REQUIRE(0 <= t0 && t0 <= t1 && t1 <= rounds && rounds <= kMaxRounds && iters >= 1 && iters <= kMaxIters, "round / iteration count out of range");
    for (int t = t0; t < t1; t++) {
        hipLaunchKernelGGL(dec_round_begin_kernel, wide_grid(ctx), kBlock, 0, ctx->stream, b, (aggressive && t == rounds - 1) ? 1 : 0);
        enqueue_iterations(ctx, b, 0, iters, count, t * kMaxIters, unique_hi);
        int rc = enqueue_read_off(ctx, b, t, t * kMaxIters + iters - 1);
        if (rc) return rc;
    }
    PALACE_HIP_TRY(hipGetLastError());
    return PALACE_OK;
}

int decomp_run_checked(palace_ctx *ctx, const DecompBufs &b, int rounds, int aggressive, bool unique_hi, int64_t comp_cap,
                       int64_t vert_cap, int64_t max_iterations)
{
    PALACE_REQUIRE(rounds >= 1 && rounds <= kMaxRounds, "round count out of range");
    constexpr int kBatch = 16;
    hipLaunchKernelGGL(dec_init_kernel, wide_grid(ctx), kBlock, 0, ctx->stream, b, comp_cap, vert_cap, kBatch, 0);
    uint64_t count = 0;
    for (int t = 0; t < rounds; t++) {
        hipLaunchKernelGGL(dec_round_begin_kernel, wide_grid(ctx), kBlock, 0, ctx->stream, b, (aggressive && t == rounds - 1) ? 1 : 0);
        for (int first = 0;; first += kBatch) {
            PALACE_HIP_TRY(hipMemsetAsync(b.changed, 0, kBatch * sizeof(uint32_t), ctx->stream));
            enqueue_iterations(ctx, b, first, kBatch, &count, 0, unique_hi);
            uint32_t last = 0;
            PALACE_HIP_TRY(hipMemcpyAsync(&last, b.changed + kBatch - 1, sizeof last, hipMemcpyDeviceToHost, ctx->stream));
            PALACE_HIP_TRY(hipStreamSynchronize(ctx->stream));
            if (!last) break;
            if (static_cast<int64_t>(count) > max_iterations || count + kBatch >= (1ull << 21)) {
                set_error("matching: no fixed point after %llu iterations", static_cast<unsigned long long>(count));
                return PALACE_ESTATE;
            }
        }
        PALACE_HIP_TRY(hipMemsetAsync(b.changed, 0, kBatch * sizeof(uint32_t), ctx->stream));
        int rc = enqueue_read_off(ctx, b, t, kBatch - 1);
        if (rc) return rc;
    }
    return PALACE_OK;
}

int decomp_group(palace_ctx *ctx, const DecompBufs &b, DecompRun &run, int rounds, int aggressive, bool unique_hi)
{
    const int first = kFirstGroupRounds;
    const int t0 = run.next_round, t1 = std::min(rounds, t0 + (t0 == 0 ? first : kRoundsPerGroup));
    for (int t = t0; t < t1; t++) {
        const int iters = ctx->match_iters > 0 ? std::min(ctx->match_iters, kMaxIters) : (t == 0 ? kFirstRoundIters : kLaterRoundIters);
        int rc = decomp_rounds(ctx, b, t, t + 1, rounds, aggressive, iters, unique_hi, &run.count);
        if (rc) return rc;
    }
    run.next_round = t1;
    return PALACE_OK;
}

int decomp_finish(palace_ctx *ctx, const DecompBufs &b, DecompRun &run, int rounds, int aggressive, bool unique_hi, int64_t comp_cap,
                  int64_t vert_cap, int64_t max_iterations, DecompState *h_state, const std::function<int()> &reset_left)
{
    for (;;) {
        PALACE_HIP_TRY(hipMemcpyAsync(h_state, b.st, sizeof *h_state, hipMemcpyDeviceToHost, ctx->stream));
        PALACE_HIP_TRY(hipStreamSynchronize(ctx->stream));
        if (h_state->unsettled) {
            int rc = reset_left();
            if (rc) return rc;
            rc = decomp_run_checked(ctx, b, rounds, aggressive, unique_hi, comp_cap, vert_cap, max_iterations);
            if (rc) return rc;
            PALACE_HIP_TRY(hipMemcpyAsync(h_state, b.st, sizeof *h_state, hipMemcpyDeviceToHost, ctx->stream));
            PALACE_HIP_TRY(hipStreamSynchronize(ctx->stream));
            return PALACE_OK;
        }
        if (run.next_round >= rounds) return PALACE_OK;
        if (h_state->alive_after == 0) {
            if (!aggressive) return PALACE_OK;
            run.next_round = rounds - 1;
        }
        int rc = decomp_group(ctx, b, run, rounds, aggressive, unique_hi);
        if (rc) return rc;
    }
}

}
```

palace_amd/csrc/decomp.hpp:

```cpp
#pragma once
#include <functional>

#include "common.hpp"

struct palace_match_result {
    int64_t n = 0;
    int64_t *off = nullptr;
    int32_t *verts = nullptr, *iter = nullptr, *open_at = nullptr;
    uint8_t *kind = nullptr;
    uint64_t *bare = nullptr;
    int64_t n_bare = 0;
    bool borrowed = false;
    ~palace_match_result();
};

namespace palace {

constexpr int kDecompGrid = 256;
constexpr int kDecompBlock = 256;
constexpr int kMaxRounds = 1024;
constexpr int kMaxIters = 64;

struct DecompState {
    int32_t S, V;
    int64_t E;
    int64_t n_comp, n_vert;
    int64_t comp_cap, vert_cap;
    uint32_t unsettled;
    uint32_t overflow;
    uint32_t bad;
    uint32_t dead;
    uint32_t packed;
    uint64_t scan_total;
    int64_t alive_after;
};

struct DecompBufs {
    DecompState *st = nullptr;
    int32_t *src = nullptr, *dst = nullptr;
    uint64_t *khi = nullptr, *klo = nullptr;
    uint8_t *done = nullptr;
    uint64_t *kc = nullptr;
    const uint32_t *pack_bad = nullptr;
    int64_t *left = nullptr;
    int32_t *orig = nullptr;
    int32_t *next = nullptr, *prev = nullptr, *on_path = nullptr, *open_at = nullptr;
    uint64_t *nhi = nullptr, *nlo = nullptr;
    uint64_t *bo_hi = nullptr, *bi_hi = nullptr;
    uint64_t *bo_lo = nullptr, *bi_lo = nullptr;
    uint64_t *len_a = nullptr, *pos = nullptr;
    int64_t *pay = nullptr;
    uint8_t *alive = nullptr, *kind = nullptr;
    uint64_t *partials = nullptr;
    uint32_t *changed = nullptr;
    int64_t *o_off = nullptr;
    int32_t *o_verts = nullptr, *o_iter = nullptr, *o_open = nullptr;
    uint8_t *o_kind = nullptr;
};

size_t decomp_bytes(int64_t s_cap, int64_t e_cap, int64_t comp_cap, int64_t vert_cap, int rounds, int iters);
void decomp_carve(DecompBufs &b, char *base, int64_t s_cap, int64_t e_cap, int64_t comp_cap, int64_t vert_cap, int rounds, int iters);
constexpr int kFirstRoundIters = 7, kLaterRoundIters = 4, kRoundsPerGroup = 5, kFirstGroupRounds = 5;
int decomp_begin(palace_ctx *ctx, const DecompBufs &b, int rounds, int64_t comp_cap, int64_t vert_cap);
int decomp_rounds(palace_ctx *ctx, const DecompBufs &b, int t0, int t1, int rounds, int aggressive, int iters, bool unique_hi,
                  uint64_t *count);

struct DecompRun { int next_round = 0; uint64_t count = 0; };
int decomp_group(palace_ctx *ctx, const DecompBufs &b, DecompRun &run, int rounds, int aggressive, bool unique_hi);
int decomp_finish(palace_ctx *ctx, const DecompBufs &b, DecompRun &run, int rounds, int aggressive, bool unique_hi, int64_t comp_cap,
                  int64_t vert_cap, int64_t max_iterations, DecompState *h_state, const std::function<int()> &reset_left);

int decomp_run_checked(palace_ctx *ctx, const DecompBufs &b, int rounds, int aggressive, bool unique_hi, int64_t comp_cap,
                       int64_t vert_cap, int64_t max_iterations);

int scan_u64(palace_ctx *ctx, const uint64_t *in, uint64_t *out, const int32_t *n_dev, uint64_t *partials, uint64_t *total_dev);

}
```

palace_amd/csrc/filter.hip:

```cpp
#include <algorithm>
#include <cstdlib>
#include <memory>
#include <vector>

#include "common.hpp"
#include "decomp.hpp"

namespace palace {
namespace {

constexpr uint64_t kEmptyKey = ~0ull;
constexpr uint64_t kWeightTop = 1ull << 40;

struct FilterState {
    int32_t n_segs, S_f, n_sel, n_resc;
    int64_t n_edges, n_junc, n_kept2, n_kept3, n_arcs;
    int64_t n_static, n_dyn;
    int64_t n_path_arcs;
    uint32_t bad, pack_bad;
    uint64_t scan_total;
};
enum : uint32_t { kBadPathToken = 1, kBadNoSeg = 2, kBadEdgeBound = 4, kBadArcTable = 8 };

struct ArcTable {
    uint64_t *key;
    unsigned long long *w;
    uint32_t *backed;
    uint64_t mask;
    int64_t *list, list_cap;
};

struct PathArcs {
    uint64_t *key;
    int32_t *idx;
    uint64_t mask;
    int32_t *u, *v;
    int32_t *arc_of;
    int64_t n, cap;
};

struct F {
    FilterState *fs;
    int32_t n_segs, min_count;
    const uint8_t *seed;
    const int32_t *tlen, *rank, *name_len;
    int32_t *by_rank;
    int64_t n_paths;
    const int64_t *path_off;
    const int32_t *path_tok;
    uint8_t *core, *sel, *near, *resc, *seg_flags, *edge_flags, *has_arc;
    int32_t *fid, *contig_of;
    uint64_t *scan_in, *scan_out;
    int64_t edge_bound;
    ArcTable t;
    PathArcs pa;
    int32_t *arc_u, *arc_v;
    unsigned long long *arc_w;
    uint8_t *arc_backed;
    int64_t arc_cap;
    int use_paths;
    uint64_t *bare;
};

__device__ __forceinline__ int gtid() { return static_cast<int>(blockIdx.x * blockDim.x + threadIdx.x); }
__device__ __forceinline__ int gsize() { return static_cast<int>(gridDim.x * blockDim.x); }

__global__ void st4_by_rank_kernel(F f)
{
    for (int s = gtid(); s < f.n_segs; s += gsize()) f.by_rank[f.rank[s]] = s;
}

__global__ void st4_begin_kernel(F f, const int64_t *__restrict__ d_n_edges, int64_t call_bound)
{
    for (int s = gtid(); s < f.n_segs; s += gsize()) {
        const uint8_t c = f.seed[s] != 0 && f.tlen[s] > 0;
        f.core[s] = c; f.sel[s] = c; f.near[s] = 0; f.resc[s] = 0;
    }
    if (gtid() == 0) {
        FilterState *fs = f.fs;
        const int64_t n = *d_n_edges;
        fs->n_segs = f.n_segs; fs->S_f = 0; fs->n_sel = 0; fs->n_resc = 0;
        const int64_t bound = call_bound < f.edge_bound ? call_bound : f.edge_bound;
        fs->n_edges = n < 0 ? 0 : (n > bound ? bound : n);
        fs->n_junc = 0; fs->n_kept2 = 0; fs->n_kept3 = 0; fs->n_arcs = 0; fs->n_static = 0; fs->n_dyn = 0;
        fs->bad = n > bound ? kBadEdgeBound : 0u;
        fs->pack_bad = 0;
        fs->scan_total = 0;
    }
}

__device__ __forceinline__ int64_t edge_total(const palace_graph_edge &e)
{
    return static_cast<int64_t>(e.counts[0]) + e.counts[1] + e.counts[2] + e.counts[3];
}

__global__ void st4_pass2_kernel(F f, const palace_graph_edge *__restrict__ edges)
{
    const int64_t n = f.fs->n_edges;
    int64_t juncs = 0, kept = 0;
    for (int64_t i = gtid(); i < n; i += gsize()) {
        const palace_graph_edge e = edges[i];
        uint8_t fl = 0;
        if (edge_total(e) >= f.min_count) {
            fl = 1; juncs++;
            if (e.left == e.right || f.core[e.left] || f.core[e.right]) {
                fl |= 2; kept++;
                f.near[e.left] = 1; f.near[e.right] = 1;
                f.sel[e.left] = 1; f.sel[e.right] = 1;
            }
        }
        f.edge_flags[i] = fl;
    }
    if (juncs) atomicAdd(reinterpret_cast<unsigned long long *>(&f.fs->n_junc), static_cast<unsigned long long>(juncs));
    if (kept) atomicAdd(reinterpret_cast<unsigned long long *>(&f.fs->n_kept2), static_cast<unsigned long long>(kept));
}

__global__ void st4_pass3_kernel(F f, const palace_graph_edge *__restrict__ edges)
{
    const int64_t n = f.fs->n_edges;
    int64_t kept = 0;
    for (int64_t i = gtid(); i < n; i += gsize()) {
        const uint8_t fl = f.edge_flags[i];
        if (!(fl & 1)) continue;
        const palace_graph_edge e = edges[i];
        if (f.core[e.left] || f.near[e.left] || f.core[e.right] || f.near[e.right]) {
            f.edge_flags[i] = fl | 4;
            if (!(fl & 2)) kept++;
            f.sel[e.left] = 1; f.sel[e.right] = 1;
        }
    }
    if (kept) atomicAdd(reinterpret_cast<unsigned long long *>(&f.fs->n_kept3), static_cast<unsigned long long>(kept));
}

__global__ void st4_paths_kernel(F f)
{
    for (int64_t p = gtid(); p < f.n_paths; p += gsize()) {
        const int64_t a = f.path_off[p], b = f.path_off[p + 1];
        int64_t total = 0, backed = 0;
        bool known = true;
        for (int64_t k = a; k < b; k++) {
            const int32_t t = f.path_tok[k];
            if (t < 0) { known = false; break; }
            const int32_t m = t >> 1;
            total += f.name_len[m];
            if (f.seed[m]) backed += f.name_len[m];
        }
        if (!known) { atomicOr(&f.fs->bad, kBadPathToken); continue; }
        if (backed > 0 && (static_cast<double>(backed) / static_cast<double>(total) >= 0.5 || backed > 2000))
            for (int64_t k = a; k < b; k++) f.resc[f.path_tok[k] >> 1] = 1;
    }
}

__global__ void st4_order_kernel(F f)
{
    for (int r = gtid(); r < f.n_segs; r += gsize()) {
        const int s = f.by_rank[r];
        const bool sel = f.sel[s], resc = f.resc[s] && !sel;
        if (resc && f.tlen[s] <= 0) atomicOr(&f.fs->bad, kBadNoSeg);
        f.scan_in[r] = (sel ? (1ull << 32) : 0ull) | (resc ? 1ull : 0ull);
    }
}

__global__ void st4_ids_kernel(F f)
{
    FilterState *fs = f.fs;
    const int32_t n_sel = static_cast<int32_t>(fs->scan_total >> 32), n_resc = static_cast<int32_t>(fs->scan_total & 0xffffffffu);
    for (int r = gtid(); r < f.n_segs; r += gsize()) {
        const int s = f.by_rank[r];
        const uint64_t in = f.scan_in[r], before = f.scan_out[r];
        int32_t id = -1;
        if (in >> 32) id = static_cast<int32_t>(before >> 32);
        else if (in & 1) id = n_sel + static_cast<int32_t>(before & 0xffffffffu);
        f.fid[s] = id;
        if (id >= 0) { f.contig_of[id] = s; f.has_arc[id] = 0; }
        f.seg_flags[s] = static_cast<uint8_t>((in >> 32 ? 1 : 0) | (in & 1 ? 2 : 0) | (f.core[s] ? 4 : 0));
    }
    if (gtid() == 0) { fs->n_sel = n_sel; fs->n_resc = n_resc; fs->S_f = n_sel + n_resc; }
}

__device__ __forceinline__ uint64_t mix(uint64_t x)
{
    x ^= x >> 33; x *= 0xff51afd7ed558ccdull; x ^= x >> 33; x *= 0xc4ceb9fe1a85ec53ull; x ^= x >> 33;
    return x;
}

__device__ void path_arc_insert(const F &f, int32_t u, int32_t v)
{
    const PathArcs &pa = f.pa;
    const uint64_t key = (static_cast<uint64_t>(static_cast<uint32_t>(u)) << 32) | static_cast<uint32_t>(v);
    uint64_t s = mix(key) & pa.mask;
    for (uint64_t probes = 0; probes <= pa.mask; probes++) {
        const uint64_t cur = pa.key[s];
        if (cur == key) return;
        if (cur == kEmptyKey) {
            const uint64_t old = atomicCAS(reinterpret_cast<unsigned long long *>(&pa.key[s]), kEmptyKey, key);
            if (old == kEmptyKey) {
                const int64_t at = static_cast<int64_t>(atomicAdd(reinterpret_cast<unsigned long long *>(&f.fs->n_path_arcs), 1ull));
                if (at < pa.cap) { pa.u[at] = u; pa.v[at] = v; pa.idx[s] = static_cast<int32_t>(at); }
                return;
            }
            if (old == key) return;
        }
        s = (s + 1) & pa.mask;
    }
}
__global__ void st4_path_arcs_kernel(F f)
{
    for (int64_t p = gtid(); p < f.n_paths; p += gsize()) {
        int32_t before = -1;
        for (int64_t k = f.path_off[p]; k < f.path_off[p + 1]; k++) {
            const int32_t here = f.path_tok[k];
            if (before >= 0 && here >= 0) {
                path_arc_insert(f, before, here);
                if ((here ^ 1) != before) path_arc_insert(f, here ^ 1, before ^ 1);
            }
            before = here;
        }
    }
}
__device__ __forceinline__ int32_t path_arc_find(const PathArcs &pa, int32_t u, int32_t v)
{
    const uint64_t key = (static_cast<uint64_t>(static_cast<uint32_t>(u)) << 32) | static_cast<uint32_t>(v);
    uint64_t s = mix(key) & pa.mask;
    for (;;) {
        const uint64_t cur = pa.key[s];
        if (cur == key) return pa.idx[s];
        if (cur == kEmptyKey) return -1;
        s = (s + 1) & pa.mask;
    }
}

__global__ __launch_bounds__(kDecompBlock) void st4_arcs_static_kernel(F f)
{
    __shared__ uint32_t wave_n[kDecompBlock / 64];
    __shared__ long long block_base;
    const PathArcs &pa = f.pa;
    const int lane = threadIdx.x & 63, wave = threadIdx.x >> 6;
    for (int64_t p0 = static_cast<int64_t>(blockIdx.x) * blockDim.x; p0 < pa.n; p0 += static_cast<int64_t>(gridDim.x) * blockDim.x) {
        const int64_t p = p0 + threadIdx.x;
        int32_t fu = -1, fv = -1;
        if (p < pa.n) {
            const int32_t cu = pa.u[p] >> 1, cv = pa.v[p] >> 1;
            if ((f.seg_flags[cu] & 3) && (f.seg_flags[cv] & 3)) { fu = f.fid[cu]; fv = f.fid[cv]; }
        }
        const bool in = fu >= 0 && fv >= 0;
        const unsigned long long m = __ballot(in);
        if (lane == 0) wave_n[wave] = static_cast<uint32_t>(__popcll(m));
        __syncthreads();
        if (threadIdx.x == 0) {
            uint32_t total = 0;
            for (int w = 0; w < kDecompBlock / 64; w++) { const uint32_t c = wave_n[w]; wave_n[w] = total; total += c; }
            block_base = total ? static_cast<long long>(atomicAdd(reinterpret_cast<unsigned long long *>(&f.fs->n_static), static_cast<unsigned long long>(total))) : 0ll;
        }
        __syncthreads();
        if (p < pa.n) {
            int32_t at = -1;
            if (in) {
                const int64_t slot = block_base + wave_n[wave] + __popcll(m & ((1ull << lane) - 1));
                if (slot < f.arc_cap) {
                    at = static_cast<int32_t>(slot);
                    f.arc_u[at] = 2 * fu + (pa.u[p] & 1); f.arc_v[at] = 2 * fv + (pa.v[p] & 1);
                    f.arc_w[at] = 0; f.arc_backed[at] = 1;
                } else atomicOr(&f.fs->bad, kBadArcTable);
            }
            pa.arc_of[p] = at;
        }
        __syncthreads();
    }
}

__device__ void bump_arc(const F &f, int32_t cu, int32_t cv, int32_t u, int32_t v, int64_t w)
{
    if (f.use_paths) {
        const int32_t p = path_arc_find(f.pa, cu, cv);
        if (p >= 0) {
            const int32_t at = f.pa.arc_of[p];
            if (at >= 0) { atomicAdd(&f.arc_w[at], static_cast<unsigned long long>(w)); return; }
        }
    }
    const ArcTable &t = f.t;
    const uint64_t key = (static_cast<uint64_t>(static_cast<uint32_t>(u)) << 32) | static_cast<uint32_t>(v);
    uint64_t s = mix(key) & t.mask;
    for (uint64_t probes = 0;; probes++) {
        if (probes > t.mask) { atomicOr(&f.fs->bad, kBadArcTable); return; }
        const uint64_t cur = t.key[s];
        if (cur == key) break;
        if (cur == kEmptyKey) {
            const uint64_t old = atomicCAS(reinterpret_cast<unsigned long long *>(&t.key[s]), kEmptyKey, key);
            if (old == kEmptyKey) {
                const int64_t at = static_cast<int64_t>(atomicAdd(reinterpret_cast<unsigned long long *>(&f.fs->n_dyn), 1ull));
                if (at < t.list_cap) t.list[at] = static_cast<int64_t>(s);
                else atomicOr(&f.fs->bad, kBadArcTable);
                break;
            }
            if (old == key) break;
        }
        s = (s + 1) & t.mask;
    }
    if (w) atomicAdd(&t.w[s], static_cast<unsigned long long>(w));
}

__global__ void st4_arcs_juncs_kernel(F f, const palace_graph_edge *__restrict__ edges)
{
    const int64_t n = f.fs->n_edges;
    for (int64_t i = gtid(); i < n; i += gsize()) {
        if (!(f.edge_flags[i] & 6)) continue;
        const palace_graph_edge e = edges[i];
        const int64_t w = min(edge_total(e), static_cast<int64_t>(kWeightTop - 1));
        const int32_t cu = 2 * e.left + (e.oL & 1), cv = 2 * e.right + (e.oR & 1);
        const int32_t u = 2 * f.fid[e.left] + (e.oL & 1), v = 2 * f.fid[e.right] + (e.oR & 1);
        bump_arc(f, cu, cv, u, v, w);
        if ((v ^ 1) != u) bump_arc(f, cv ^ 1, cu ^ 1, v ^ 1, u ^ 1, w);
    }
}

__global__ void st4_arcs_dyn_kernel(F f)
{
    FilterState *fs = f.fs;
    const int64_t n_static = min(fs->n_static, f.arc_cap), n = min(fs->n_dyn, f.t.list_cap);
    for (int64_t a = gtid(); a < n; a += gsize()) {
        const int64_t s = f.t.list[a];
        const uint64_t key = f.t.key[s];
        const int64_t at = n_static + a;
        if (at < f.arc_cap) {
            f.arc_u[at] = static_cast<int32_t>(key >> 32); f.arc_v[at] = static_cast<int32_t>(key & 0xffffffffu);
            f.arc_w[at] = f.t.w[s]; f.arc_backed[at] = 0;
        } else atomicOr(&fs->bad, kBadArcTable);
        f.t.key[s] = kEmptyKey; f.t.w[s] = 0;
    }
    if (gtid() == 0) fs->n_arcs = min(n_static + n, f.arc_cap);
}

__global__ void st4_arc_keys_kernel(F f, DecompBufs b)
{
    const int64_t n = min(f.fs->n_static, f.arc_cap) + min(f.fs->n_dyn, f.t.list_cap);
    for (int64_t a = gtid(); a < n && a < f.arc_cap; a += gsize()) {
        const int32_t u = f.arc_u[a], v = f.arc_v[a];
        const uint64_t w = min(static_cast<uint64_t>(f.arc_w[a]), kWeightTop - 1);
        b.khi[a] = ((kWeightTop - w) << 1) | (f.arc_backed[a] ? 0u : 1u);
        const uint64_t key = (static_cast<uint64_t>(static_cast<uint32_t>(u)) << 32) | static_cast<uint32_t>(v);
        const uint64_t twin = (static_cast<uint64_t>(static_cast<uint32_t>(v ^ 1)) << 32) | static_cast<uint32_t>(u ^ 1);
        const uint64_t cls = min(key, twin);
        b.klo[a] = (cls << 1) | (key != cls ? 1u : 0u);
        f.has_arc[u >> 1] = 1; f.has_arc[v >> 1] = 1;
    }
}

__global__ void st4_sub_in_kernel(F f)
{
    const int n = f.fs->S_f;
    for (int i = gtid(); i < n; i += gsize()) f.scan_in[i] = f.has_arc[i];
}

__global__ void st4_sub_kernel(F f, DecompBufs b, const int32_t *__restrict__ cn)
{
    FilterState *fs = f.fs;
    const int n = fs->S_f;
    const int32_t n_sub = static_cast<int32_t>(fs->scan_total);
    for (int i = gtid(); i < n; i += gsize()) {
        if (!f.has_arc[i]) continue;
        const int32_t sub = static_cast<int32_t>(f.scan_out[i]);
        b.orig[sub] = i;
        b.left[sub] = max(1, cn[f.contig_of[i]]);
    }
    const int64_t n_arcs = min(fs->n_arcs, f.arc_cap);
    const int vbits = 32 - __clz(max(1, 2 * n_sub - 1)), wbits = min(40, 51 - 2 * vbits);
    const uint64_t wmax = wbits > 0 ? (1ull << wbits) - 1 : 0;
    if (gtid() == 0 && wbits <= 0) fs->pack_bad = 1;
    for (int64_t a = gtid(); a < n_arcs; a += gsize()) {
        const int32_t u = f.arc_u[a], v = f.arc_v[a];
        const int32_t su = 2 * static_cast<int32_t>(f.scan_out[u >> 1]) + (u & 1), sv = 2 * static_cast<int32_t>(f.scan_out[v >> 1]) + (v & 1);
        b.src[a] = su;
        b.dst[a] = sv;
        if (wbits > 0) {
            const uint64_t w = f.arc_w[a];
            if (w > wmax) atomicOr(&fs->pack_bad, 1u);
            const uint64_t key = (static_cast<uint64_t>(su) << vbits) | static_cast<uint32_t>(sv);
            const uint64_t twin = (static_cast<uint64_t>(sv ^ 1) << vbits) | static_cast<uint32_t>(su ^ 1);
            b.kc[a] = ((wmax - min(w, wmax)) << (2 * vbits + 1)) | (static_cast<uint64_t>(f.arc_backed[a] ? 0u : 1u) << (2 * vbits)) | min(key, twin);
        }
    }
    if (gtid() == 0) { b.st->S = n_sub; b.st->V = 2 * n_sub; b.st->E = n_arcs; }
}

__global__ void st4_left_kernel(F f, DecompBufs b, const int32_t *__restrict__ cn)
{
    const int n = f.fs->S_f;
    for (int i = gtid(); i < n; i += gsize())
        if (f.has_arc[i]) b.left[static_cast<int32_t>(f.scan_out[i])] = max(1, cn[f.contig_of[i]]);
}

__global__ void st4_bare_kernel(F f)
{
    const int n = f.fs->S_f, words = (n + 63) / 64;
    for (int w = gtid(); w < words; w += gsize()) {
        uint64_t bits = 0;
        for (int k = 0; k < 64 && w * 64 + k < n; k++)
            if (!f.has_arc[w * 64 + k]) bits |= 1ull << k;
        f.bare[w] = bits;
    }
}

size_t up(size_t v) { return (v + 255) / 256 * 256; }
uint64_t pow2_at_least(uint64_t v) { uint64_t p = 1024; while (p < v) p <<= 1; return p; }

template <class T>
T *carve(char *&p, size_t n)
{
    T *r = reinterpret_cast<T *>(p);
    p += up(std::max<size_t>(1, n) * sizeof(T));
    return r;
}

}
}

struct palace_stage04 {
    palace::F f{};
    palace::DecompBufs b{};
    char *fixed = nullptr;
    char *grown = nullptr;
    size_t grown_bytes = 0;
    int64_t n_tok = 0, edge_bound = 0, s_cap = 0, e_cap = 0, comp_cap = 0, vert_cap = 0;
    int rounds = 0, aggressive = 0, last_rounds = 0;
    palace::DecompRun run;
    bool filtered = false, matched = false;
    const int32_t *d_cn = nullptr;
    char *pin = nullptr;
    size_t pin_bytes = 0;
    palace::FilterState *h_fs = nullptr;
    palace::DecompState *h_ds = nullptr;
    palace_match_result res;
    int32_t *h_contig_of = nullptr;
};

using namespace palace;

namespace {

const dim3 kG(1024), kB(kDecompBlock);

int grow_pinned(palace_ctx *ctx, palace_stage04 *s, size_t bytes)
{
    if (s->pin_bytes >= bytes) return PALACE_OK;
    if (s->pin) { PALACE_HIP_TRY(hipStreamSynchronize(ctx->stream)); PALACE_HIP_TRY(hipHostFree(s->pin)); s->pin = nullptr; s->pin_bytes = 0; }
    const size_t want = bytes + bytes / 4 + (1 << 16);
    hipError_t e = hipHostMalloc(reinterpret_cast<void **>(&s->pin), want, hipHostMallocDefault);
    if (e != hipSuccess) { set_error("stage04: hipHostMalloc(%zu) failed: %s", want, hipGetErrorString(e)); return PALACE_ENOMEM; }
    s->pin_bytes = want;
    return PALACE_OK;
}

int grow_device(palace_ctx *ctx, palace_stage04 *s, int64_t edge_bound, int rounds)
{
    const int64_t e_dyn = 2 * edge_bound + 16;
    const int64_t e_cap = e_dyn + s->f.pa.n + 16;
    const int64_t s_cap = std::min<int64_t>(s->f.n_segs, e_cap);
    const int64_t comp_cap = static_cast<int64_t>(rounds) * s_cap + 16, vert_cap = 2 * comp_cap;
    const uint64_t slots = pow2_at_least(2 * static_cast<uint64_t>(e_dyn));
    const size_t dec = decomp_bytes(s_cap, e_cap, comp_cap, vert_cap, rounds, kMaxIters);
    const size_t bytes = up(static_cast<size_t>(edge_bound) + 1) + up(slots * 8) * 2 + up(static_cast<size_t>(e_dyn) * 8) +
                         2 * up(static_cast<size_t>(e_cap) * 4) + up(static_cast<size_t>(e_cap) * 8) + up(static_cast<size_t>(e_cap)) + dec + 8192;
    if (s->grown_bytes < bytes || s->edge_bound < edge_bound || s->rounds < rounds) {
        if (s->grown) { PALACE_HIP_TRY(hipStreamSynchronize(ctx->stream)); PALACE_HIP_TRY(hipFree(s->grown)); s->grown = nullptr; s->grown_bytes = 0; }
        hipError_t e = hipMalloc(reinterpret_cast<void **>(&s->grown), bytes);
        if (e != hipSuccess) { set_error("stage04: hipMalloc(%zu) failed: %s", bytes, hipGetErrorString(e)); return PALACE_ENOMEM; }
        s->grown_bytes = bytes;
        char *p = s->grown;
        s->f.edge_flags = carve<uint8_t>(p, static_cast<size_t>(edge_bound) + 1);
        s->f.t.key = carve<uint64_t>(p, slots);
        s->f.t.w = carve<unsigned long long>(p, slots);
        s->f.t.backed = nullptr;
        s->f.t.mask = slots - 1;
        s->f.t.list = carve<int64_t>(p, static_cast<size_t>(e_dyn));
        s->f.t.list_cap = e_dyn;
        s->f.arc_u = carve<int32_t>(p, static_cast<size_t>(e_cap));
        s->f.arc_v = carve<int32_t>(p, static_cast<size_t>(e_cap));
        s->f.arc_w = carve<unsigned long long>(p, static_cast<size_t>(e_cap));
        s->f.arc_backed = carve<uint8_t>(p, static_cast<size_t>(e_cap));
        s->f.arc_cap = e_cap;
        decomp_carve(s->b, p, s_cap, e_cap, comp_cap, vert_cap, rounds, kMaxIters);
        s->b.pack_bad = &s->f.fs->pack_bad;
        PALACE_HIP_TRY(hipMemsetAsync(s->f.t.key, 0xff, slots * 8, ctx->stream));
        PALACE_HIP_TRY(hipMemsetAsync(s->f.t.w, 0, slots * 8, ctx->stream));
        s->edge_bound = edge_bound; s->s_cap = s_cap; s->e_cap = e_cap; s->comp_cap = comp_cap; s->vert_cap = vert_cap; s->rounds = rounds;
    }
    s->f.edge_bound = s->edge_bound;
    return PALACE_OK;
}

}

extern "C" {

int palace_stage04_create(palace_ctx *ctx, const palace_stage04_inputs *in, palace_stage04 **out)
{
    PALACE_REQUIRE(ctx && in && out, "null argument");
    PALACE_REQUIRE(in->n_segs >= 0 && in->n_segs < (1 << 30) && in->n_paths >= 0 && in->min_count >= 0, "bad size");
    PALACE_REQUIRE(in->n_segs == 0 || (in->seed && in->tlen && in->rank && in->name_len), "null per-contig array");
    PALACE_REQUIRE(in->n_paths == 0 || (in->path_off && in->path_tok), "null path arrays");
    PALACE_HIP_TRY(hipSetDevice(ctx->device));
    const size_t n = static_cast<size_t>(in->n_segs);
    const int64_t n_tok = in->n_paths ? in->path_off[in->n_paths] : 0;
    PALACE_REQUIRE(n_tok >= 0 && (in->n_paths == 0 || in->path_off[0] == 0), "path offsets must start at 0 and ascend");
    int64_t n_pairs = 0;
    for (int64_t k = 0; k < in->n_paths; k++) {
        const int64_t len = in->path_off[k + 1] - in->path_off[k];
        PALACE_REQUIRE(len >= 0 && in->path_off[k + 1] <= n_tok, "path offsets must start at 0 and ascend");
        n_pairs += len > 1 ? len - 1 : 0;
    }
    for (int32_t i = 0; i < in->n_segs; i++) PALACE_REQUIRE(in->rank[i] >= 0 && in->rank[i] < in->n_segs, "rank out of range");
    for (int64_t k = 0; k < n_tok; k++) PALACE_REQUIRE(in->path_tok[k] < 2 * static_cast<int64_t>(in->n_segs), "path token out of range");
    std::unique_ptr<palace_stage04> s(new palace_stage04());
    const int64_t pa_cap = 2 * n_pairs + 16;
    const uint64_t pa_slots = pow2_at_least(2 * static_cast<uint64_t>(pa_cap));
    const size_t bytes = up(sizeof(FilterState)) + up(n) * 8 + up(n * 4) * 6 + up(n * 8) * 2 + up((static_cast<size_t>(in->n_paths) + 1) * 8) +
                         up(static_cast<size_t>(n_tok) * 4 + 4) + up((n + 63) / 64 * 8 + 8) + up(pa_slots * 8) + up(pa_slots * 4) +
                         3 * up(static_cast<size_t>(pa_cap) * 4) + 16384;
    hipError_t e = hipMalloc(reinterpret_cast<void **>(&s->fixed), bytes);
    if (e != hipSuccess) { set_error("stage04: hipMalloc(%zu) failed: %s", bytes, hipGetErrorString(e)); return PALACE_ENOMEM; }
    char *p = s->fixed;
    F &f = s->f;
    f.fs = carve<FilterState>(p, 1);
    f.n_segs = in->n_segs; f.min_count = in->min_count; f.n_paths = in->n_paths;
    uint8_t *seed = carve<uint8_t>(p, n);
    f.core = carve<uint8_t>(p, n); f.sel = carve<uint8_t>(p, n); f.near = carve<uint8_t>(p, n); f.resc = carve<uint8_t>(p, n);
    f.seg_flags = carve<uint8_t>(p, n); f.has_arc = carve<uint8_t>(p, n);
    int32_t *tlen = carve<int32_t>(p, n), *rank = carve<int32_t>(p, n), *name_len = carve<int32_t>(p, n);
    f.by_rank = carve<int32_t>(p, n); f.fid = carve<int32_t>(p, n); f.contig_of = carve<int32_t>(p, n);
    f.scan_in = carve<uint64_t>(p, n); f.scan_out = carve<uint64_t>(p, n);
    int64_t *path_off = carve<int64_t>(p, static_cast<size_t>(in->n_paths) + 1);
    int32_t *path_tok = carve<int32_t>(p, static_cast<size_t>(n_tok) + 1);
    f.bare = carve<uint64_t>(p, (n + 63) / 64 + 1);
    f.pa.key = carve<uint64_t>(p, pa_slots); f.pa.idx = carve<int32_t>(p, pa_slots); f.pa.mask = pa_slots - 1;
    f.pa.u = carve<int32_t>(p, static_cast<size_t>(pa_cap)); f.pa.v = carve<int32_t>(p, static_cast<size_t>(pa_cap));
    f.pa.arc_of = carve<int32_t>(p, static_cast<size_t>(pa_cap));
    f.pa.cap = pa_cap; f.pa.n = 0;
    f.seed = seed; f.tlen = tlen; f.rank = rank; f.name_len = name_len; f.path_off = path_off; f.path_tok = path_tok;
    s->n_tok = n_tok;
    auto fail = [&](hipError_t err) {
        set_error("stage04: upload failed: %s", hipGetErrorString(err));
        (void)hipFree(s->fixed);
        return PALACE_EHIP;
    };
    hipStream_t st = ctx->stream;
    if (n) {
        if ((e = hipMemcpyAsync(seed, in->seed, n, hipMemcpyHostToDevice, st)) != hipSuccess) return fail(e);
        if ((e = hipMemcpyAsync(tlen, in->tlen, n * 4, hipMemcpyHostToDevice, st)) != hipSuccess) return fail(e);
        if ((e = hipMemcpyAsync(rank, in->rank, n * 4, hipMemcpyHostToDevice, st)) != hipSuccess) return fail(e);
        if ((e = hipMemcpyAsync(name_len, in->name_len, n * 4, hipMemcpyHostToDevice, st)) != hipSuccess) return fail(e);
    }
    if (in->n_paths) {
        if ((e = hipMemcpyAsync(path_off, in->path_off, (static_cast<size_t>(in->n_paths) + 1) * 8, hipMemcpyHostToDevice, st)) != hipSuccess) return fail(e);
        if (n_tok && (e = hipMemcpyAsync(path_tok, in->path_tok, static_cast<size_t>(n_tok) * 4, hipMemcpyHostToDevice, st)) != hipSuccess) return fail(e);
    } else if ((e = hipMemsetAsync(path_off, 0, 8, st)) != hipSuccess) return fail(e);
    hipLaunchKernelGGL(st4_by_rank_kernel, kG, kB, 0, st, f);
    if ((e = hipMemsetAsync(f.fs, 0, sizeof(FilterState), st)) != hipSuccess) return fail(e);
    if ((e = hipMemsetAsync(f.pa.key, 0xff, pa_slots * 8, st)) != hipSuccess) return fail(e);
    hipLaunchKernelGGL(st4_path_arcs_kernel, kG, kB, 0, st, f);
    FilterState h_fs{};
    if ((e = hipMemcpyAsync(&h_fs, f.fs, sizeof h_fs, hipMemcpyDeviceToHost, st)) != hipSuccess) return fail(e);
    if ((e = hipStreamSynchronize(st)) != hipSuccess) return fail(e);
    if (h_fs.n_path_arcs > pa_cap) { (void)hipFree(s->fixed); set_error("stage04: path arc table too small"); return PALACE_ESTATE; }
    f.pa.n = h_fs.n_path_arcs;
    e = hipHostMalloc(reinterpret_cast<void **>(&s->h_fs), up(sizeof(FilterState)) + up(sizeof(DecompState)), hipHostMallocDefault);
    if (e != hipSuccess) { (void)hipFree(s->fixed); set_error("stage04: hipHostMalloc failed: %s", hipGetErrorString(e)); return PALACE_ENOMEM; }
    s->h_ds = reinterpret_cast<DecompState *>(reinterpret_cast<char *>(s->h_fs) + up(sizeof(FilterState)));
    s->res.borrowed = true;
    *out = s.release();
    return PALACE_OK;
}

int palace_stage04_destroy(palace_ctx *ctx, palace_stage04 *s)
{
    if (!s) return PALACE_OK;
    if (ctx) { (void)hipSetDevice(ctx->device); (void)hipStreamSynchronize(ctx->stream); }
    if (s->fixed) (void)hipFree(s->fixed);
    if (s->grown) (void)hipFree(s->grown);
    if (s->pin) (void)hipHostFree(s->pin);
    if (s->h_fs) (void)hipHostFree(s->h_fs);
    delete s;
    return PALACE_OK;
}

int palace_stage04_reserve(palace_ctx *ctx, palace_stage04 *s, int64_t edge_bound)
{
    PALACE_REQUIRE(ctx && s && edge_bound >= 0, "bad argument");
    PALACE_HIP_TRY(hipSetDevice(ctx->device));
    return grow_device(ctx, s, std::max<int64_t>(edge_bound, s->edge_bound), std::max(s->rounds, 11));
}

int palace_stage04_filter(palace_ctx *ctx, palace_stage04 *s, const palace_graph_edge *d_edges, const int64_t *d_n_edges,
                          int64_t edge_bound)
{
    PALACE_REQUIRE(ctx && s && d_n_edges && edge_bound >= 0, "bad argument");
    PALACE_REQUIRE(edge_bound == 0 || d_edges, "null edge array");
    PALACE_HIP_TRY(hipSetDevice(ctx->device));
    int rc = grow_device(ctx, s, std::max<int64_t>(edge_bound, s->edge_bound), std::max(s->rounds, 11));
    if (rc) return rc;
    rc = [&]() -> int {
        const F &f = s->f;
        hipStream_t st = ctx->stream;
        hipLaunchKernelGGL(st4_begin_kernel, kG, kB, 0, st, f, d_n_edges, edge_bound);
        hipLaunchKernelGGL(st4_pass2_kernel, kG, kB, 0, st, f, d_edges);
        hipLaunchKernelGGL(st4_pass3_kernel, kG, kB, 0, st, f, d_edges);
        hipLaunchKernelGGL(st4_paths_kernel, kG, kB, 0, st, f);
        hipLaunchKernelGGL(st4_order_kernel, kG, kB, 0, st, f);
        PALACE_HIP_TRY(hipGetLastError());
        int rc2 = scan_u64(ctx, f.scan_in, f.scan_out, &f.fs->n_segs, s->b.partials, &f.fs->scan_total);
        if (rc2) return rc2;
        hipLaunchKernelGGL(st4_ids_kernel, kG, kB, 0, st, f);
        PALACE_HIP_TRY(hipGetLastError());
        return PALACE_OK;
    }();
    if (rc) return rc;
    s->filtered = true;
    s->matched = false;
    return PALACE_OK;
}

static int enqueue_match(palace_ctx *ctx, palace_stage04 *s, const palace_graph_edge *d_edges, bool use_paths)
{
    s->f.use_paths = use_paths ? 1 : 0;
    const F &f = s->f;
    hipStream_t st = ctx->stream;
    if (use_paths) hipLaunchKernelGGL(st4_arcs_static_kernel, kG, kB, 0, st, f);
    hipLaunchKernelGGL(st4_arcs_juncs_kernel, kG, kB, 0, st, f, d_edges);
    hipLaunchKernelGGL(st4_arcs_dyn_kernel, kG, kB, 0, st, f);
    hipLaunchKernelGGL(st4_arc_keys_kernel, kG, kB, 0, st, f, s->b);
    hipLaunchKernelGGL(st4_sub_in_kernel, kG, kB, 0, st, f);
    PALACE_HIP_TRY(hipGetLastError());
    int rc = scan_u64(ctx, f.scan_in, f.scan_out, &f.fs->S_f, s->b.partials, &f.fs->scan_total);
    if (rc) return rc;
    hipLaunchKernelGGL(st4_sub_kernel, kG, kB, 0, st, f, s->b, s->d_cn);
    hipLaunchKernelGGL(st4_bare_kernel, kG, kB, 0, st, f);
    PALACE_HIP_TRY(hipGetLastError());
    return PALACE_OK;
}

int palace_stage04_match(palace_ctx *ctx, palace_stage04 *s, const palace_graph_edge *d_edges, const int32_t *d_cn,
                         int32_t iterations, int32_t aggressive, int32_t use_paths)
{
    PALACE_REQUIRE(ctx && s && d_cn && iterations >= 1, "bad argument");
    PALACE_REQUIRE(s->filtered, "palace_stage04_filter has not run");
    const int rounds = iterations + (aggressive ? 1 : 0);
    PALACE_REQUIRE(rounds <= kMaxRounds, "too many iterations");
    PALACE_REQUIRE(rounds <= s->rounds, "more rounds than the filter call reserved room for (at most 10 iterations + aggressive)");
    PALACE_HIP_TRY(hipSetDevice(ctx->device));
    s->d_cn = d_cn; s->aggressive = aggressive ? 1 : 0;
    s->f.use_paths = use_paths ? 1 : 0;
    int rc = enqueue_match(ctx, s, d_edges, use_paths != 0);
    if (rc) return rc;
    s->run = DecompRun{};
    if ((rc = decomp_begin(ctx, s->b, rounds, s->comp_cap, s->vert_cap))) return rc;
    if ((rc = decomp_group(ctx, s->b, s->run, rounds, s->aggressive, false))) return rc;
    PALACE_HIP_TRY(hipMemcpyAsync(s->h_fs, s->f.fs, sizeof(FilterState), hipMemcpyDeviceToHost, ctx->stream));
    s->rounds = std::max(s->rounds, rounds);
    s->matched = true;
    s->last_rounds = rounds;
    return PALACE_OK;
}

static int check_filter_state(const FilterState &fs)
{
    if (fs.bad & kBadPathToken) { set_error("stage04: contigs.paths names an unknown contig id (filter_graph.py:138 raises)"); return PALACE_EINVAL; }
    if (fs.bad & kBadNoSeg) { set_error("stage04: contigs.paths rescues a contig without SEG line (filter_graph.py:257 raises)"); return PALACE_EINVAL; }
    if (fs.bad & kBadEdgeBound) { set_error("stage04: more edges on the device than the bound given to palace_stage04_filter"); return PALACE_EINVAL; }
    if (fs.bad & kBadArcTable) { set_error("stage04: arc table full"); return PALACE_ESTATE; }
    return PALACE_OK;
}

int palace_stage04_counts(palace_ctx *ctx, palace_stage04 *s, int64_t counts[8])
{
    PALACE_REQUIRE(ctx && s && counts && s->filtered, "bad argument");
    PALACE_HIP_TRY(hipMemcpyAsync(s->h_fs, s->f.fs, sizeof(FilterState), hipMemcpyDeviceToHost, ctx->stream));
    PALACE_HIP_TRY(hipStreamSynchronize(ctx->stream));
    const FilterState &fs = *s->h_fs;
    int rc = check_filter_state(fs);
    if (rc) return rc;
    counts[0] = fs.n_edges; counts[1] = fs.n_junc; counts[2] = fs.n_kept2; counts[3] = fs.n_kept3;
    counts[4] = fs.n_sel; counts[5] = fs.n_resc; counts[6] = s->matched ? fs.n_arcs : -1; counts[7] = fs.S_f;
    return PALACE_OK;
}

int palace_stage04_flags(palace_ctx *ctx, palace_stage04 *s, uint8_t *h_seg_flags, uint8_t *h_edge_flags, int64_t n_edges)
{
    PALACE_REQUIRE(ctx && s && s->filtered && n_edges >= 0 && n_edges <= s->edge_bound, "bad argument");
    if (h_seg_flags && s->f.n_segs)
        PALACE_HIP_TRY(hipMemcpyAsync(h_seg_flags, s->f.seg_flags, static_cast<size_t>(s->f.n_segs), hipMemcpyDeviceToHost, ctx->stream));
    if (h_edge_flags && n_edges)
        PALACE_HIP_TRY(hipMemcpyAsync(h_edge_flags, s->f.edge_flags, static_cast<size_t>(n_edges), hipMemcpyDeviceToHost, ctx->stream));
    PALACE_HIP_TRY(hipStreamSynchronize(ctx->stream));
    return PALACE_OK;
}

int palace_stage04_result(palace_ctx *ctx, palace_stage04 *s, palace_match_result **out, const int32_t **contig_of_out,
                          int64_t *n_segs_filtered_out)
{
    PALACE_REQUIRE(ctx && s && out, "null argument");
    PALACE_REQUIRE(s->matched, "palace_stage04_match has not run");
    PALACE_HIP_TRY(hipSetDevice(ctx->device));
    hipStream_t st = ctx->stream;
    const int rounds = s->last_rounds;
    auto reset_left = [&]() -> int {
        hipLaunchKernelGGL(st4_left_kernel, kG, kB, 0, st, s->f, s->b, s->d_cn);
        PALACE_HIP_TRY(hipGetLastError());
        return PALACE_OK;
    };
    int rc = decomp_finish(ctx, s->b, s->run, rounds, s->aggressive, false, s->comp_cap, s->vert_cap, 2 * s->e_cap + 64, s->h_ds, reset_left);
    if (rc) return rc;
    rc = check_filter_state(*s->h_fs);
    if (rc) return rc;
    const DecompState &ds = *s->h_ds;
    if (ds.overflow || ds.n_comp > s->comp_cap || ds.n_vert > s->vert_cap) { set_error("stage04: component arrays too small"); return PALACE_ESTATE; }
    const size_t nc = static_cast<size_t>(ds.n_comp), nv = static_cast<size_t>(ds.n_vert), sf = static_cast<size_t>(s->h_fs->S_f);
    const size_t words = (sf + 63) / 64;
    rc = grow_pinned(ctx, s, up((nc + 1) * 8) + up(nv * 4 + 4) + 2 * up(nc * 4 + 4) + up(nc + 1) + up(words * 8 + 8) + up(sf * 4 + 4));
    if (rc) return rc;
    char *p = s->pin;
    palace_match_result &r = s->res;
    r.off = carve<int64_t>(p, nc + 1); r.verts = carve<int32_t>(p, nv + 1); r.iter = carve<int32_t>(p, nc + 1);
    r.open_at = carve<int32_t>(p, nc + 1); r.kind = carve<uint8_t>(p, nc + 1); r.bare = carve<uint64_t>(p, words + 1);
    s->h_contig_of = carve<int32_t>(p, sf + 1);
    PALACE_HIP_TRY(hipMemcpyAsync(r.off, s->b.o_off, (nc + 1) * 8, hipMemcpyDeviceToHost, st));
    if (nv) PALACE_HIP_TRY(hipMemcpyAsync(r.verts, s->b.o_verts, nv * 4, hipMemcpyDeviceToHost, st));
    if (nc) {
        PALACE_HIP_TRY(hipMemcpyAsync(r.iter, s->b.o_iter, nc * 4, hipMemcpyDeviceToHost, st));
        PALACE_HIP_TRY(hipMemcpyAsync(r.open_at, s->b.o_open, nc * 4, hipMemcpyDeviceToHost, st));
        PALACE_HIP_TRY(hipMemcpyAsync(r.kind, s->b.o_kind, nc, hipMemcpyDeviceToHost, st));
    }
    if (words) PALACE_HIP_TRY(hipMemcpyAsync(r.bare, s->f.bare, words * 8, hipMemcpyDeviceToHost, st));
    if (sf) PALACE_HIP_TRY(hipMemcpyAsync(s->h_contig_of, s->f.contig_of, sf * 4, hipMemcpyDeviceToHost, st));
    PALACE_HIP_TRY(hipStreamSynchronize(st));
    r.n = static_cast<int64_t>(nc);
    r.n_bare = static_cast<int64_t>(sf) - ds.S;
    *out = &s->res;
    if (contig_of_out) *contig_of_out = s->h_contig_of;
    if (n_segs_filtered_out) *n_segs_filtered_out = static_cast<int64_t>(sf);
    return PALACE_OK;
}

}
```

palace_amd/csrc/match.hip:

```cpp
#include "common.hpp"
#include "decomp.hpp"
#include <algorithm>
#include <map>
#include <memory>
#include <mutex>
#include <numeric>
#include <thread>

namespace palace {

constexpr int32_t kNone = -1;

struct MatchArgs {
    int32_t n_vertices;
    int64_t n_arcs;
    const int32_t *src, *dst;
    const int64_t *out_off, *in_off;
    const int32_t *out_arcs, *in_arcs;
    const uint8_t *alive;
    int32_t *next, *prev, *next_arc, *want_out, *want_in;
    unsigned int *changed;
};

__global__ void match_propose_kernel(MatchArgs a)
{
    int32_t v = blockIdx.x * blockDim.x + threadIdx.x;
    if (v >= a.n_vertices) return;
    int32_t wo = kNone, wi = kNone;
    if (a.alive[v]) {
        if (a.next[v] == kNone)
            for (int64_t k = a.out_off[v]; k < a.out_off[v + 1]; k++) {
                int32_t e = a.out_arcs[k], h = a.dst[e];
                if (a.alive[h] && a.prev[h] == kNone) { wo = e; break; }
            }
        if (a.prev[v] == kNone)
            for (int64_t k = a.in_off[v]; k < a.in_off[v + 1]; k++) {
                int32_t e = a.in_arcs[k], t = a.src[e];
                if (a.alive[t] && a.next[t] == kNone) { wi = e; break; }
            }
    }
    a.want_out[v] = wo;
    a.want_in[v] = wi;
}

__global__ void match_commit_kernel(MatchArgs a)
{
    int32_t v = blockIdx.x * blockDim.x + threadIdx.x;
    if (v >= a.n_vertices) return;
    int32_t e = a.want_out[v];
    if (e == kNone) return;
    int32_t h = a.dst[e];
    if (a.want_in[h] != e) return;
    a.next[v] = h;
    a.prev[h] = v;
    a.next_arc[v] = e;
    *a.changed = 1u;
}

__global__ void match_init_kernel(MatchArgs a)
{
    int32_t v = blockIdx.x * blockDim.x + threadIdx.x;
    if (v >= a.n_vertices) return;
    a.next[v] = kNone; a.prev[v] = kNone; a.next_arc[v] = kNone;
}

}

using namespace palace;

constexpr int kRoundsPerCheck = 4;

static int enqueue_rounds(palace_ctx *ctx, const MatchArgs &a, int n)
{
    const unsigned blocks = static_cast<unsigned>((a.n_vertices + 255) / 256);
    PALACE_HIP_TRY(hipMemsetAsync(a.changed, 0, 4, ctx->stream));
    for (int k = 0; k < n; k++) {
        hipLaunchKernelGGL(match_propose_kernel, dim3(blocks), dim3(256), 0, ctx->stream, a);
        hipLaunchKernelGGL(match_commit_kernel, dim3(blocks), dim3(256), 0, ctx->stream, a);
    }
    PALACE_HIP_TRY(hipGetLastError());
    return PALACE_OK;
}

extern "C" int palace_match_greedy(palace_ctx *ctx, int32_t n_vertices, int64_t n_arcs, const int32_t *d_src,
                                   const int32_t *d_dst, const int64_t *d_out_off, const int32_t *d_out_arcs,
                                   const int64_t *d_in_off, const int32_t *d_in_arcs, const uint8_t *d_alive,
                                   int32_t *d_next, int32_t *d_prev, int32_t *d_next_arc, int32_t *rounds_out)
{
    PALACE_REQUIRE(ctx && n_vertices >= 0 && n_arcs >= 0, "bad argument");
    if (rounds_out) *rounds_out = 0;
    if (n_vertices == 0) return PALACE_OK;
    PALACE_REQUIRE(d_out_off && d_in_off && d_alive && d_next && d_prev && d_next_arc, "null device pointer");
    PALACE_REQUIRE(n_arcs == 0 || (d_src && d_dst && d_out_arcs && d_in_arcs), "null arc arrays");
    PALACE_REQUIRE(n_arcs < (1ll << 31), "arc ids must fit in int32");
    PALACE_HIP_TRY(hipSetDevice(ctx->device));
    int rc = ensure_workspace(ctx, static_cast<size_t>(n_vertices) * 8 + 256);
    if (rc) return rc;
    MatchArgs a{};
    a.n_vertices = n_vertices; a.n_arcs = n_arcs; a.src = d_src; a.dst = d_dst;
    a.out_off = d_out_off; a.in_off = d_in_off; a.out_arcs = d_out_arcs; a.in_arcs = d_in_arcs;
    a.alive = d_alive; a.next = d_next; a.prev = d_prev; a.next_arc = d_next_arc;
    a.want_out = static_cast<int32_t *>(ctx->ws.ptr);
    a.want_in = a.want_out + n_vertices;
    a.changed = reinterpret_cast<unsigned int *>(ctx->d_small);
    const unsigned blocks = static_cast<unsigned>((n_vertices + 255) / 256);
    hipLaunchKernelGGL(match_init_kernel, dim3(blocks), dim3(256), 0, ctx->stream, a);
    int rounds = 0;
    for (;;) {
        unsigned int changed = 0;
        rc = enqueue_rounds(ctx, a, kRoundsPerCheck);
        if (rc) return rc;
        PALACE_HIP_TRY(hipMemcpyAsync(&changed, ctx->d_small, 4, hipMemcpyDeviceToHost, ctx->stream));
        PALACE_HIP_TRY(hipStreamSynchronize(ctx->stream));
        rounds += kRoundsPerCheck;
        if (!changed) break;
        if (rounds > n_vertices + 2 + kRoundsPerCheck) { set_error("palace_match_greedy: no fixed point"); return PALACE_ESTATE; }
    }
    if (rounds_out) *rounds_out = rounds;
    return PALACE_OK;
}

struct SubResult {
    std::vector<int64_t> off{0};
    std::vector<int32_t> verts, iter, open_at;
    std::vector<uint8_t> kind;
};

namespace palace {

class BlockPool {
public:
    void *take(size_t bytes)
    {
        bytes = std::max<size_t>(bytes, 64);
        {
            std::lock_guard<std::mutex> g(mu_);
            for (size_t i = 0; i < free_.size(); i++)
                if (free_[i].second >= bytes && free_[i].second <= 2 * bytes + (1 << 20)) {
                    void *p = free_[i].first;
                    sizes_[p] = free_[i].second;
                    free_.erase(free_.begin() + i);
                    return p;
                }
        }
        void *p = std::malloc(bytes);
        if (p) { std::lock_guard<std::mutex> g(mu_); sizes_[p] = bytes; }
        return p;
    }
    void give(void *p)
    {
        if (!p) return;
        std::lock_guard<std::mutex> g(mu_);
        const size_t bytes = sizes_[p];
        sizes_.erase(p);
        if (free_.size() < 16) free_.emplace_back(p, bytes);
        else std::free(p);
    }

private:
    std::mutex mu_;
    std::vector<std::pair<void *, size_t>> free_;
    std::map<void *, size_t> sizes_;
};
static BlockPool g_result_pool;

struct MatchScratch {
    std::vector<int32_t> new_id, old_id, ssrc, sdst;
    std::vector<int64_t> sub_copies;
    std::vector<uint64_t> has_arc;
    SubResult sub;
};
void free_match_scratch(MatchScratch *m) { delete m; }

template <class T>
struct Borrowed {
    T &home;
    T v;
    explicit Borrowed(T &h) : home(h), v(std::move(h)) {}
    ~Borrowed() { home = std::move(v); }
    Borrowed(const Borrowed &) = delete;
    Borrowed &operator=(const Borrowed &) = delete;
};

__global__ void iota_keys_kernel(uint64_t *__restrict__ khi, uint64_t *__restrict__ klo, int64_t n)
{
    for (int64_t i = static_cast<int64_t>(blockIdx.x) * blockDim.x + threadIdx.x; i < n; i += static_cast<int64_t>(gridDim.x) * blockDim.x) {
        khi[i] = static_cast<uint64_t>(i);
        klo[i] = 0;
    }
}

}

palace_match_result::~palace_match_result()
{
    if (borrowed) return;
    for (void *p : {(void *)off, (void *)verts, (void *)iter, (void *)open_at, (void *)kind, (void *)bare}) palace::g_result_pool.give(p);
}

static int decompose_core(palace_ctx *ctx, int32_t n_segs, const int64_t *copies, const int32_t *orig, int64_t n_arcs,
                          const int32_t *src, const int32_t *dst, int32_t iterations, int32_t aggressive, SubResult *res)
{
    using namespace palace;
    const int64_t S = n_segs, E = n_arcs;
    const int rounds = iterations + (aggressive ? 1 : 0);
    PALACE_REQUIRE(rounds <= kMaxRounds, "too many iterations");
    int64_t live_rounds = 0;
    for (int64_t s = 0; s < S; s++) live_rounds += std::min<int64_t>(iterations, std::max<int64_t>(1, copies[s]));
    if (aggressive) live_rounds += S;
    const int64_t comp_cap = live_rounds, vert_cap = 2 * live_rounds;
    const size_t dev_bytes = decomp_bytes(S, E, comp_cap, vert_cap, rounds, kMaxIters);
    int rc = ensure_workspace(ctx, dev_bytes);
    if (rc) return rc;
    DecompBufs b;
    decomp_carve(b, static_cast<char *>(ctx->ws.ptr), S, E, comp_cap, vert_cap, rounds, kMaxIters);
    const size_t e4 = (static_cast<size_t>(E) * 4 + 255) / 256 * 256, s8 = (static_cast<size_t>(S) * 8 + 255) / 256 * 256,
                 s4 = (static_cast<size_t>(S) * 4 + 255) / 256 * 256;
    rc = ensure_pinned(ctx, 2 * e4 + s8 + s4 + 512);
    if (rc) return rc;
    char *pin = static_cast<char *>(ctx->pin.ptr);
    int32_t *p_src = reinterpret_cast<int32_t *>(pin), *p_dst = reinterpret_cast<int32_t *>(pin + e4);
    int64_t *p_left = reinterpret_cast<int64_t *>(pin + 2 * e4);
    int32_t *p_orig = reinterpret_cast<int32_t *>(pin + 2 * e4 + s8);
    DecompState *p_st = reinterpret_cast<DecompState *>(pin + 2 * e4 + s8 + s4);
    DecompState *p_back = p_st + 1;
    std::copy(src, src + E, p_src); std::copy(dst, dst + E, p_dst);
    for (int64_t s = 0; s < S; s++) p_left[s] = std::max<int64_t>(1, copies[s]);
    std::copy(orig, orig + S, p_orig);
    std::memset(p_st, 0, sizeof *p_st);
    p_st->S = n_segs; p_st->V = 2 * n_segs; p_st->E = E;
    hipStream_t st = ctx->stream;
    auto upload = [&]() -> int {
        PALACE_HIP_TRY(hipMemcpyAsync(b.st, p_st, sizeof *p_st, hipMemcpyHostToDevice, st));
        if (E) {
            PALACE_HIP_TRY(hipMemcpyAsync(b.src, p_src, static_cast<size_t>(E) * 4, hipMemcpyHostToDevice, st));
            PALACE_HIP_TRY(hipMemcpyAsync(b.dst, p_dst, static_cast<size_t>(E) * 4, hipMemcpyHostToDevice, st));
            hipLaunchKernelGGL(iota_keys_kernel, dim3(kDecompGrid), dim3(kDecompBlock), 0, st, b.khi, b.klo, E);
        }
        PALACE_HIP_TRY(hipMemcpyAsync(b.left, p_left, static_cast<size_t>(S) * 8, hipMemcpyHostToDevice, st));
        PALACE_HIP_TRY(hipMemcpyAsync(b.orig, p_orig, static_cast<size_t>(S) * 4, hipMemcpyHostToDevice, st));
        return PALACE_OK;
    };
    auto fail = [&](int code) { (void)hipStreamSynchronize(st); return code; };
    hipError_t e = hipSuccess;
    if ((rc = upload())) return fail(rc);
    if ((rc = decomp_begin(ctx, b, rounds, comp_cap, vert_cap))) return fail(rc);
    DecompRun run;
    if ((rc = decomp_group(ctx, b, run, rounds, aggressive, true))) return fail(rc);
    auto reset_left = [&]() -> int {
        PALACE_HIP_TRY(hipMemcpyAsync(b.left, p_left, static_cast<size_t>(S) * 8, hipMemcpyHostToDevice, st));
        return PALACE_OK;
    };
    if ((rc = decomp_finish(ctx, b, run, rounds, aggressive, true, comp_cap, vert_cap, 2 * E + 64, p_back, reset_left))) return fail(rc);
    if (p_back->overflow || p_back->n_comp > comp_cap || p_back->n_vert > vert_cap) {
        set_error("decompose: component arrays too small (%lld components, %lld vertices)", (long long)p_back->n_comp, (long long)p_back->n_vert);
        return PALACE_ESTATE;
    }
    const size_t nc = static_cast<size_t>(p_back->n_comp), nv = static_cast<size_t>(p_back->n_vert);
    res->off.resize(nc + 1); res->verts.resize(nv); res->iter.resize(nc); res->open_at.resize(nc); res->kind.resize(nc);
    e = hipMemcpyAsync(res->off.data(), b.o_off, (nc + 1) * 8, hipMemcpyDeviceToHost, st);
    if (e == hipSuccess && nv) e = hipMemcpyAsync(res->verts.data(), b.o_verts, nv * 4, hipMemcpyDeviceToHost, st);
    if (e == hipSuccess && nc) e = hipMemcpyAsync(res->iter.data(), b.o_iter, nc * 4, hipMemcpyDeviceToHost, st);
    if (e == hipSuccess && nc) e = hipMemcpyAsync(res->open_at.data(), b.o_open, nc * 4, hipMemcpyDeviceToHost, st);
    if (e == hipSuccess && nc) e = hipMemcpyAsync(res->kind.data(), b.o_kind, nc, hipMemcpyDeviceToHost, st);
    if (e == hipSuccess) e = hipStreamSynchronize(st);
    if (e != hipSuccess) { set_error("decompose: %s", hipGetErrorString(e)); return fail(PALACE_EHIP); }
    return PALACE_OK;
}

namespace {

void radix_by(const std::vector<uint64_t> &key, std::vector<uint32_t> &perm, std::vector<uint32_t> &tmp)
{
    const size_t n = perm.size();
    uint64_t all_or = 0, all_and = ~0ull;
    for (size_t i = 0; i < n; i++) { all_or |= key[i]; all_and &= key[i]; }
    const uint64_t varying = all_or ^ all_and;
    std::vector<uint32_t> hist(65536);
    for (int shift = 0; shift < 64; shift += 16) {
        if (((varying >> shift) & 0xffffu) == 0) continue;
        std::fill(hist.begin(), hist.end(), 0u);
        for (size_t i = 0; i < n; i++) hist[(key[perm[i]] >> shift) & 0xffffu]++;
        uint32_t run = 0;
        for (auto &h : hist) { const uint32_t c = h; h = run; run += c; }
        for (size_t i = 0; i < n; i++) tmp[hist[(key[perm[i]] >> shift) & 0xffffu]++] = perm[i];
        perm.swap(tmp);
    }
}

}

extern "C" {

int palace_match_arcs_from_edges(const int32_t *cn, int32_t n_segs, const palace_graph_edge *edges, int64_t n_edges,
                                 int32_t min_count, int64_t *copies, int32_t *src, int32_t *dst, int64_t *weight,
                                 int64_t *n_arcs_out)
{
    PALACE_REQUIRE(n_segs >= 0 && n_edges >= 0 && n_arcs_out, "bad argument");
    PALACE_REQUIRE(n_segs == 0 || (cn && copies), "null segment arrays");
    PALACE_REQUIRE(n_edges == 0 || (edges && src && dst && weight), "null edge arrays");
    PALACE_REQUIRE(n_segs < (1 << 30) && n_edges < (1ll << 30), "graph too large for int32 ids");
    for (int32_t s = 0; s < n_segs; s++) copies[s] = std::max(1, cn[s]);
    const uint64_t V = 2ull * static_cast<uint64_t>(n_segs);
    static thread_local std::vector<uint64_t> pair, m_pair, m_cls, m_wkey;
    static thread_local std::vector<int64_t> w, m_w;
    static thread_local std::vector<uint32_t> perm, tmp;
    pair.clear(); w.clear(); m_pair.clear(); m_w.clear();
    pair.reserve(2 * n_edges); w.reserve(2 * n_edges);
    for (int64_t e = 0; e < n_edges; e++) {
        const palace_graph_edge &x = edges[e];
        const int64_t tot = static_cast<int64_t>(x.counts[0]) + x.counts[1] + x.counts[2] + x.counts[3];
        if (tot < min_count) continue;
        PALACE_REQUIRE(x.left >= 0 && x.left < n_segs && x.right >= 0 && x.right < n_segs, "edge endpoint out of range");
        const uint64_t u = 2ull * x.left + (x.oL & 1), v = 2ull * x.right + (x.oR & 1);
        pair.push_back(u * V + v); w.push_back(tot);
        if ((v ^ 1) != u) { pair.push_back((v ^ 1) * V + (u ^ 1)); w.push_back(tot); }
    }
    const size_t n = pair.size();
    perm.resize(n); tmp.resize(n);
    std::iota(perm.begin(), perm.end(), 0u);
    radix_by(pair, perm, tmp);
    m_pair.reserve(n); m_w.reserve(n);
    for (size_t i = 0; i < n; i++) {
        if (!m_pair.empty() && m_pair.back() == pair[perm[i]]) m_w.back() += w[perm[i]];
        else { m_pair.push_back(pair[perm[i]]); m_w.push_back(w[perm[i]]); }
    }
    const size_t m = m_pair.size();
    int64_t w_max = 0;
    for (int64_t x : m_w) w_max = std::max(w_max, x);
    m_cls.resize(m); m_wkey.resize(m);
    for (size_t i = 0; i < m; i++) {
        const uint64_t u = m_pair[i] / V, v = m_pair[i] % V;
        m_cls[i] = std::min(m_pair[i], (v ^ 1) * V + (u ^ 1));
        m_wkey[i] = static_cast<uint64_t>(w_max - m_w[i]);
    }
    perm.resize(m); tmp.resize(m);
    std::iota(perm.begin(), perm.end(), 0u);
    radix_by(m_cls, perm, tmp);
    radix_by(m_wkey, perm, tmp);
    for (size_t i = 0; i < m; i++) {
        const uint64_t p = m_pair[perm[i]];
        src[i] = static_cast<int32_t>(p / V); dst[i] = static_cast<int32_t>(p % V); weight[i] = m_w[perm[i]];
    }
    *n_arcs_out = static_cast<int64_t>(m);
    return PALACE_OK;
}

int palace_match_set_option(palace_ctx *ctx, const char *name, int64_t value)
{
    PALACE_REQUIRE(ctx && name, "null argument");
    if (!std::strcmp(name, "iters_per_round")) {
        PALACE_REQUIRE(value >= 0 && value <= palace::kMaxIters, "iters_per_round out of range");
        ctx->match_iters = static_cast<int>(value);
    } else if (!std::strcmp(name, "one_word_keys")) {
        PALACE_REQUIRE(value == 0 || value == 1, "one_word_keys must be 0 or 1");
        ctx->match_two_word_keys = value == 0;
    } else if (!std::strcmp(name, "decomp_grid")) {
        PALACE_REQUIRE(value >= 0 && value <= 65536, "decomp_grid out of range");
        ctx->match_grid = static_cast<int>(value);
    } else {
        palace::set_error("palace_match_set_option: unknown option '%s'", name);
        return PALACE_EINVAL;
    }
    return PALACE_OK;
}

int palace_match_decompose(palace_ctx *ctx, int32_t n_segs, const int64_t *copies, int64_t n_arcs,
                           const int32_t *src, const int32_t *dst, int32_t iterations, int32_t aggressive,
                           palace_match_result **out)
{
    return palace_match_decompose_ex(ctx, n_segs, copies, n_arcs, src, dst, iterations, aggressive, 0, out);
}

int palace_match_decompose_ex(palace_ctx *ctx, int32_t n_segs, const int64_t *copies, int64_t n_arcs,
                              const int32_t *src, const int32_t *dst, int32_t iterations, int32_t aggressive,
                              int32_t compact, palace_match_result **out)
{
    PALACE_REQUIRE(ctx && out && n_segs >= 0 && n_arcs >= 0 && iterations >= 1, "bad argument");
    PALACE_REQUIRE(n_segs == 0 || copies, "null copies");
    PALACE_REQUIRE(n_arcs == 0 || (src && dst), "null arc arrays");
    PALACE_REQUIRE(n_segs < (1 << 30) && n_arcs < (1ll << 31), "graph too large for int32 ids");
    PALACE_HIP_TRY(hipSetDevice(ctx->device));
    const int32_t V = 2 * n_segs;
    for (int64_t e = 0; e < n_arcs; e++)
        PALACE_REQUIRE(src[e] >= 0 && src[e] < V && dst[e] >= 0 && dst[e] < V, "arc endpoint out of range");
    if (!ctx->match_scratch) ctx->match_scratch = new palace::MatchScratch();
    palace::MatchScratch &ms = *ctx->match_scratch;
    palace::Borrowed<std::vector<int32_t>> b_new(ms.new_id), b_old(ms.old_id), b_ssrc(ms.ssrc), b_sdst(ms.sdst);
    palace::Borrowed<std::vector<int64_t>> b_sc(ms.sub_copies);
    auto &new_id = b_new.v, &old_id = b_old.v, &ssrc = b_ssrc.v, &sdst = b_sdst.v;
    auto &sub_copies = b_sc.v;
    SubResult &sub = ms.sub;
    const size_t n_words = (static_cast<size_t>(n_segs) + 63) / 64;
    palace::Borrowed<std::vector<uint64_t>> b_bits(ms.has_arc);
    auto &has_arc = b_bits.v;
    has_arc.assign(n_words, 0);
    for (int64_t e = 0; e < n_arcs; e++) {
        const int32_t a = src[e] >> 1, b = dst[e] >> 1;
        has_arc[a >> 6] |= 1ull << (a & 63);
        has_arc[b >> 6] |= 1ull << (b & 63);
    }
    new_id.resize(n_words + 1);
    old_id.clear();
    for (size_t w = 0; w < n_words; w++) {
        new_id[w] = static_cast<int32_t>(old_id.size());
        for (uint64_t x = has_arc[w]; x; x &= x - 1) old_id.push_back(static_cast<int32_t>(w * 64 + __builtin_ctzll(x)));
    }
    new_id[n_words] = static_cast<int32_t>(old_id.size());
    auto is_sub = [&](int32_t sg) { return (has_arc[sg >> 6] >> (sg & 63)) & 1ull; };
    auto sub_rank = [&](int32_t sg) {
        if (sg >= n_segs) return new_id[n_words];
        return new_id[sg >> 6] + __builtin_popcountll(has_arc[sg >> 6] & ((1ull << (sg & 63)) - 1));
    };
    const int32_t n_sub = static_cast<int32_t>(old_id.size());
    sub_copies.resize(n_sub);
    for (int32_t k = 0; k < n_sub; k++) sub_copies[k] = copies[old_id[k]];
    ssrc.resize(n_arcs); sdst.resize(n_arcs);
    for (int64_t e = 0; e < n_arcs; e++) {
        ssrc[e] = 2 * sub_rank(src[e] >> 1) + (src[e] & 1);
        sdst[e] = 2 * sub_rank(dst[e] >> 1) + (dst[e] & 1);
    }
    sub.off.assign(1, 0); sub.verts.clear(); sub.iter.clear(); sub.open_at.clear(); sub.kind.clear();
    int rc = n_sub ? decompose_core(ctx, n_sub, sub_copies.data(), old_id.data(), n_arcs, ssrc.data(), sdst.data(), iterations, aggressive, &sub)
                   : PALACE_OK;
    if (rc) return rc;
    const int64_t n_sub_comp = static_cast<int64_t>(sub.kind.size());
    const int last_round = iterations + (aggressive ? 1 : 0) - 1;
    const int64_t n_bare = static_cast<int64_t>(n_segs) - n_sub;
    if (compact) {
        palace_match_result *res = new palace_match_result();
        const int64_t nv = static_cast<int64_t>(sub.verts.size());
        res->off = static_cast<int64_t *>(palace::g_result_pool.take((n_sub_comp + 1) * 8));
        res->kind = static_cast<uint8_t *>(palace::g_result_pool.take(n_sub_comp + 1));
        res->iter = static_cast<int32_t *>(palace::g_result_pool.take((n_sub_comp + 1) * 4));
        res->open_at = static_cast<int32_t *>(palace::g_result_pool.take((n_sub_comp + 1) * 4));
        res->verts = static_cast<int32_t *>(palace::g_result_pool.take((nv + 1) * 4));
        res->bare = static_cast<uint64_t *>(palace::g_result_pool.take((n_words + 1) * 8));
        if (!res->off || !res->kind || !res->iter || !res->open_at || !res->verts || !res->bare) {
            delete res;
            palace::set_error("palace_match_decompose: out of host memory");
            return PALACE_ENOMEM;
        }
        std::copy(sub.off.begin(), sub.off.end(), res->off);
        std::copy(sub.kind.begin(), sub.kind.end(), res->kind);
        std::copy(sub.iter.begin(), sub.iter.end(), res->iter);
        std::copy(sub.open_at.begin(), sub.open_at.end(), res->open_at);
        std::copy(sub.verts.begin(), sub.verts.end(), res->verts);
        for (size_t w = 0; w < n_words; w++) res->bare[w] = ~has_arc[w];
        if (n_segs & 63) res->bare[n_words - 1] &= (1ull << (n_segs & 63)) - 1;
        res->n = n_sub_comp;
        res->n_bare = n_bare;
        *out = res;
        return PALACE_OK;
    }
    const int64_t n_out = n_sub_comp + n_bare * (aggressive && last_round > 0 ? 2 : 1);
    const int64_t nv_out = static_cast<int64_t>(sub.verts.size()) + (n_out - n_sub_comp);
    palace_match_result *res = new palace_match_result();
    res->off = static_cast<int64_t *>(palace::g_result_pool.take((n_out + 1) * 8));
    res->kind = static_cast<uint8_t *>(palace::g_result_pool.take(n_out));
    res->iter = static_cast<int32_t *>(palace::g_result_pool.take(n_out * 4));
    res->open_at = static_cast<int32_t *>(palace::g_result_pool.take(n_out * 4));
    res->verts = static_cast<int32_t *>(palace::g_result_pool.take(nv_out * 4));
    if (!res->off || !res->kind || !res->iter || !res->open_at || !res->verts) {
        delete res;
        palace::set_error("palace_match_decompose: out of host memory");
        return PALACE_ENOMEM;
    }
    int64_t *r_off = res->off;
    int32_t *r_verts = res->verts, *r_iter = res->iter, *r_open = res->open_at;
    uint8_t *r_kind = res->kind;
    r_off[0] = 0;
    auto split = [&](int64_t c) { return (sub.verts[sub.off[c]] + 1) >> 1; };
    auto merge_range = [&](int32_t a, int32_t b, int64_t c_lo, int64_t c_hi, int64_t oc, int64_t ov, int round) {
        int32_t s = a;
        auto bare_until = [&](int32_t until) {
            for (; s < until; s++) {
                if (is_sub(s)) continue;
                r_verts[ov++] = 2 * s;
                r_kind[oc] = 0; r_iter[oc] = round; r_open[oc] = 0;
                r_off[++oc] = ov;
            }
        };
        for (int64_t c = c_lo; c < c_hi; c++) {
            bare_until(std::min<int32_t>(b, split(c)));
            const int64_t len = sub.off[c + 1] - sub.off[c];
            std::copy(sub.verts.begin() + sub.off[c], sub.verts.begin() + sub.off[c + 1], r_verts + ov);
            ov += len;
            r_kind[oc] = sub.kind[c]; r_iter[oc] = sub.iter[c]; r_open[oc] = sub.open_at[c];
            r_off[++oc] = ov;
        }
        bare_until(b);
    };
    int64_t oc = 0, ov = 0, c = 0;
    for (int round = 0; round <= last_round; round++) {
        int64_t c_end = c;
        while (c_end < n_sub_comp && sub.iter[c_end] == round) c_end++;
        const bool bare_round = round == 0 || (aggressive && round == last_round);
        if (!bare_round) {
            merge_range(0, 0, c, c_end, oc, ov, round);
            oc += c_end - c; ov += sub.off[c_end] - sub.off[c];
            c = c_end;
            continue;
        }
        const int n_thr = n_segs >= (1 << 17) ? 4 : 1;
        std::vector<std::thread> pool;
        int64_t c_lo = c;
        for (int k = 0; k < n_thr; k++) {
            const int32_t a = static_cast<int32_t>(static_cast<int64_t>(n_segs) * k / n_thr);
            const int32_t b = static_cast<int32_t>(static_cast<int64_t>(n_segs) * (k + 1) / n_thr);
            int64_t c_hi = c_end;
            if (k + 1 < n_thr) {
                int64_t lo = c_lo, hi = c_end;
                while (lo < hi) { const int64_t mid = (lo + hi) / 2; if (split(mid) < b) lo = mid + 1; else hi = mid; }
                c_hi = lo;
            }
            const int64_t n_sub_in = sub_rank(b) - sub_rank(a);
            const int64_t n_bare_in = (b - a) - n_sub_in;
            if (n_thr == 1) merge_range(a, b, c_lo, c_hi, oc, ov, round);
            else pool.emplace_back(merge_range, a, b, c_lo, c_hi, oc, ov, round);
            oc += n_bare_in + (c_hi - c_lo);
            ov += n_bare_in + (sub.off[c_hi] - sub.off[c_lo]);
            c_lo = c_hi;
        }
        for (auto &t : pool) t.join();
        c = c_end;
    }
    res->n = oc;
    *out = res;
    return PALACE_OK;
}

int64_t palace_match_result_count(const palace_match_result *r) { return r ? r->n : 0; }
const int64_t *palace_match_result_offsets(const palace_match_result *r) { return r ? r->off : nullptr; }
const int32_t *palace_match_result_verts(const palace_match_result *r) { return r ? r->verts : nullptr; }
const uint8_t *palace_match_result_kind(const palace_match_result *r) { return r ? r->kind : nullptr; }
const int32_t *palace_match_result_iter(const palace_match_result *r) { return r ? r->iter : nullptr; }
const int32_t *palace_match_result_open_at(const palace_match_result *r) { return r ? r->open_at : nullptr; }
const uint64_t *palace_match_result_bare(const palace_match_result *r) { return r ? r->bare : nullptr; }
int64_t palace_match_result_bare_count(const palace_match_result *r) { return r ? r->n_bare : 0; }
void palace_match_result_free(palace_match_result *r) { if (r && !r->borrowed) delete r; }

}
```

Measured before the change: 112.9 million.

## Fuse decomposition scan into cycles/emit kernels and drop lo-proposal pass with packed keys

Per-round decomposition no longer runs a separate multi-kernel prefix scan and a single-thread round-end kernel. Cycle detection now writes per-block range sums, and emit computes its own offsets from them, with the last block finalizing state through an atomic ticket. The lo-proposal kernel is skipped when packed keys are expected; if packing turns out unavailable, the run is marked stalled and redone via the existing unsettled fallback. Filter kernels are also merged (pass3 with paths, bare with sub) to cut launches, at the cost of fixed range partitioning, which may limit parallelism inside emit.

```diff
diff --git a/include/palace_hip.h b/include/palace_hip.h
--- a/include/palace_hip.h
+++ b/include/palace_hip.h
@@ -313,6 +313,7 @@
                          int32_t iterations, int32_t aggressive, int32_t use_paths);
 int palace_stage04_result(palace_ctx *ctx, palace_stage04 *s, palace_match_result **out, const int32_t **contig_of_out,
                           int64_t *n_segs_filtered_out);
+int palace_stage04_redone(const palace_stage04 *s);
 
 #ifdef __cplusplus
 }
diff --git a/palace_amd/capi.py b/palace_amd/capi.py
--- a/palace_amd/capi.py
+++ b/palace_amd/capi.py
@@ -172,6 +172,7 @@
     "palace_stage04_counts": [C.c_void_p, C.c_void_p, C.POINTER(C.c_int64)],
     "palace_stage04_match": [C.c_void_p, C.c_void_p, C.c_void_p, C.c_void_p, C.c_int32, C.c_int32, C.c_int32],
     "palace_stage04_result": [C.c_void_p, C.c_void_p, C.POINTER(C.c_void_p), C.POINTER(C.c_void_p), C.POINTER(C.c_int64)],
+    "palace_stage04_redone": [C.c_void_p],
 }
 
 
@@ -650,6 +651,9 @@
         contig_of = np.ctypeslib.as_array(C.cast(cof, C.POINTER(C.c_int32)), shape=(max(1, n.value),))[: n.value]
         return r, contig_of
 
+    def redone(self) -> bool:
+        return bool(lib().palace_stage04_redone(self.h))
+
     def close(self):
         if self.h:
             lib().palace_stage04_destroy(self.ctx.h, self.h)
diff --git a/palace_amd/csrc/decomp.hip b/palace_amd/csrc/decomp.hip
--- a/palace_amd/csrc/decomp.hip
+++ b/palace_amd/csrc/decomp.hip
@@ -99,7 +99,7 @@
 struct Span { int tid, n; };
 __device__ __forceinline__ Span whole_grid() { return Span{static_cast<int>(blockIdx.x * blockDim.x + threadIdx.x), static_cast<int>(gridDim.x * blockDim.x)}; }
 
-__device__ void ph_init(const DecompBufs &b, Span T, int64_t comp_cap, int64_t vert_cap, int n_flags, int allow_packed)
+__device__ void ph_init(const DecompBufs &b, Span T, int64_t comp_cap, int64_t vert_cap, int n_flags, int allow_packed, int need_packed)
 {
     DecompState *st = b.st;
     const int V = st->V;
@@ -107,8 +107,10 @@
     for (int i = T.tid; i < n_flags; i += T.n) b.changed[i] = 0;
     if (T.tid == 0) {
         st->n_comp = 0; st->n_vert = 0; st->comp_cap = comp_cap; st->vert_cap = vert_cap;
-        st->unsettled = 0; st->overflow = 0; st->bad = 0; st->dead = 0; st->scan_total = 0; st->alive_after = 0;
+        st->overflow = 0; st->dead = 0; st->scan_total = 0; st->alive_after = 0; st->ticket = 0;
         st->packed = (allow_packed && b.kc && b.pack_bad && *b.pack_bad == 0) ? 1u : 0u;
+        st->stalled = need_packed && !st->packed ? 1u : 0u;
+        st->unsettled = st->stalled;
         if (comp_cap >= 0) b.o_off[0] = 0;
     }
 }
@@ -116,6 +118,7 @@
 __device__ void ph_round_begin(const DecompBufs &b, Span T, int reset_left)
 {
     const int V = b.st->V;
+    if (b.st->stalled) return;
     if (!reset_left && b.st->dead) return;
     if (T.tid == 0) { b.st->alive_after = 0; if (reset_left) b.st->dead = 0; }
     const int64_t E = b.st->E;
@@ -144,7 +147,7 @@
 
 __device__ void ph_propose_hi(const DecompBufs &b, Span T, const IterArgs &a)
 {
-    if (b.st->dead) return;
+    if (b.st->dead || b.st->stalled) return;
     if (a.prev_flag >= 0 && !b.changed[a.prev_flag]) return;
     const int64_t E = b.st->E;
     const int V = b.st->V;
@@ -180,7 +183,7 @@
 __device__ void ph_commit_flag(const DecompBufs &b, Span T, const IterArgs &a, volatile unsigned int *took);
 __device__ void ph_commit(const DecompBufs &b, Span T, const IterArgs &a)
 {
-    if (b.st->dead) return;
+    if (b.st->dead || b.st->stalled) return;
     if (a.prev_flag >= 0 && !b.changed[a.prev_flag]) return;
     ph_commit_flag(b, T, a, b.changed + a.flag);
 }
@@ -209,7 +212,7 @@
 __device__ void ph_heads(const DecompBufs &b, Span T, int round, int last_flag)
 {
     DecompState *st = b.st;
-    if (st->dead) return;
+    if (st->dead || st->stalled) return;
     if (T.tid == 0 && last_flag >= 0 && b.changed[last_flag]) st->unsettled = 1;
     const int V = st->V;
     for (int v = T.tid; v < V; v += T.n) {
@@ -232,87 +235,143 @@
     }
 }
 
-__device__ void ph_cycles(const DecompBufs &b, Span T, int round)
-{
-    const int V = b.st->V;
-    if (b.st->dead) return;
-    for (int v = T.tid; v < V; v += T.n) {
-        if (!b.alive[v] || b.on_path[v] == round + 1) continue;
-        int len = 1, twin_least = v ^ 1, worst = 0;
-        uint64_t whi = b.nhi[v], wlo = b.nlo[v];
-        int64_t least = b.left[v >> 1];
-        bool first = true;
-        for (int x = b.next[v]; x != v; x = b.next[x]) {
-            if (x < v) { first = false; break; }
-            twin_least = min(twin_least, x ^ 1);
-            const uint64_t hi = b.nhi[x], lo = b.nlo[x];
-            if (hi > whi || (hi == whi && lo > wlo)) { whi = hi; wlo = lo; worst = len; }
-            least = min(least, b.left[x >> 1]);
-            len++;
-        }
-        if (!first || v > twin_least) continue;
-        const int64_t uses = twin_least == v ? 2 : 1;
-        b.len_a[v] = (1ull << 40) | static_cast<uint64_t>(len);
-        b.pay[v] = max(static_cast<int64_t>(1), least / uses);
-        b.kind[v] = 1;
-        b.open_at[v] = (worst + 1) % len;
-    }
-}
-
-__device__ void ph_emit(const DecompBufs &b, Span T, int round, int64_t c0, int64_t v0)
+struct Range { int a, e, parts; };
+__device__ __forceinline__ Range own_range(int V)
+{
+    const int parts = min(static_cast<int>(gridDim.x), kMaxRangeParts);
+    if (static_cast<int>(blockIdx.x) >= parts) return Range{0, 0, parts};
+    const int64_t chunk = (static_cast<int64_t>(V) + parts - 1) / parts;
+    const int64_t a = min(static_cast<int64_t>(V), static_cast<int64_t>(blockIdx.x) * chunk);
+    return Range{static_cast<int>(a), static_cast<int>(min(static_cast<int64_t>(V), a + chunk)), parts};
+}
+
+__device__ __forceinline__ uint64_t block_sum(uint64_t v, uint64_t *part)
+{
+    const int lane = threadIdx.x & 63, waves = static_cast<int>(blockDim.x >> 6);
+    v = wave_incl_scan(v, lane);
+    if (lane == 63) part[threadIdx.x >> 6] = v;
+    __syncthreads();
+    uint64_t t = 0;
+    for (int w = 0; w < waves; w++) t += part[w];
+    __syncthreads();
+    return t;
+}
+
+__device__ void cycle_from(const DecompBufs &b, int v, int round)
+{
+    if (!b.alive[v] || b.on_path[v] == round + 1) return;
+    int len = 1, twin_least = v ^ 1, worst = 0;
+    uint64_t whi = b.nhi[v], wlo = b.nlo[v];
+    int64_t least = b.left[v >> 1];
+    bool first = true;
+    for (int x = b.next[v]; x != v; x = b.next[x]) {
+        if (x < v) { first = false; break; }
+        twin_least = min(twin_least, x ^ 1);
+        const uint64_t hi = b.nhi[x], lo = b.nlo[x];
+        if (hi > whi || (hi == whi && lo > wlo)) { whi = hi; wlo = lo; worst = len; }
+        least = min(least, b.left[x >> 1]);
+        len++;
+    }
+    if (!first || v > twin_least) return;
+    const int64_t uses = twin_least == v ? 2 : 1;
+    b.len_a[v] = (1ull << 40) | static_cast<uint64_t>(len);
+    b.pay[v] = max(static_cast<int64_t>(1), least / uses);
+    b.kind[v] = 1;
+    b.open_at[v] = (worst + 1) % len;
+}
+
+__global__ __launch_bounds__(kDecompBlock) void dec_cycles_kernel(DecompBufs b, int round)
+{
+    __shared__ uint64_t part[kMaxWaves];
+    if (b.st->dead || b.st->stalled) return;
+    const Range r = own_range(b.st->V);
+    uint64_t sum = 0;
+    for (int v = r.a + static_cast<int>(threadIdx.x); v < r.e; v += blockDim.x) {
+        cycle_from(b, v, round);
+        sum += b.len_a[v];
+    }
+    sum = block_sum(sum, part);
+    if (threadIdx.x == 0 && static_cast<int>(blockIdx.x) < r.parts) b.range_sums[blockIdx.x] = sum;
+}
+
+__device__ int64_t emit_from(const DecompBufs &b, int v, uint64_t la, uint64_t p, int round, int64_t c0, int64_t v0)
 {
     DecompState *st = b.st;
-    const int V = st->V;
-    if (st->dead) return;
+    const int64_t len = static_cast<int64_t>(la & kLenMask);
+    const int64_t c = c0 + static_cast<int64_t>(p >> 40), at = v0 + static_cast<int64_t>(p & kLenMask);
+    const int64_t pay = b.pay[v];
+    const bool room = c < st->comp_cap && at + len <= st->vert_cap;
+    if (!room) st->overflow = 1;
+    else { b.o_off[c] = at; b.o_kind[c] = b.kind[v]; b.o_iter[c] = round; b.o_open[c] = b.open_at[v]; }
+    int x = v;
+    int64_t still = 0;
+    for (int64_t k = 0; k < len; k++) {
+        if (room) b.o_verts[at + k] = 2 * b.orig[x >> 1] + (x & 1);
+        const int64_t l = b.left[x >> 1];
+        b.left[x >> 1] = max(static_cast<int64_t>(0), l - pay);
+        still += l - pay > 0;
+        x = b.next[x];
+    }
+    return still;
+}
+
+__global__ __launch_bounds__(kDecompBlock) void dec_emit_kernel(DecompBufs b, int round)
+{
+    __shared__ uint64_t part[kMaxWaves];
+    __shared__ unsigned long long wg_alive;
+    DecompState *st = b.st;
+    if (st->dead || st->stalled) return;
+    const int64_t c0 = st->n_comp, v0 = st->n_vert;
+    const Range r = own_range(st->V);
+    const int blk = static_cast<int>(blockIdx.x), lane = threadIdx.x & 63, wv = threadIdx.x >> 6, waves = static_cast<int>(blockDim.x >> 6);
+    uint64_t before = 0, total = 0;
+    for (int j = threadIdx.x; j < r.parts; j += blockDim.x) {
+        const uint64_t x = b.range_sums[j];
+        total += x;
+        if (j < blk) before += x;
+    }
+    before = block_sum(before, part);
+    total = block_sum(total, part);
+    if (threadIdx.x == 0) wg_alive = 0;
     int64_t alive = 0;
-    for (int v = T.tid; v < V; v += T.n) {
-        const uint64_t la = b.len_a[v];
-        if (!la) continue;
-        const int64_t len = static_cast<int64_t>(la & kLenMask);
-        const uint64_t p = b.pos[v];
-        const int64_t c = c0 + static_cast<int64_t>(p >> 40), at = v0 + static_cast<int64_t>(p & kLenMask);
-        const int64_t pay = b.pay[v];
-        const bool room = c < st->comp_cap && at + len <= st->vert_cap;
-        if (!room) st->overflow = 1;
-        else { b.o_off[c] = at; b.o_kind[c] = b.kind[v]; b.o_iter[c] = round; b.o_open[c] = b.open_at[v]; }
-        int x = v;
-        int64_t still = 0;
-        for (int64_t k = 0; k < len; k++) {
-            if (room) b.o_verts[at + k] = 2 * b.orig[x >> 1] + (x & 1);
-            const int64_t l = b.left[x >> 1];
-            b.left[x >> 1] = max(static_cast<int64_t>(0), l - pay);
-            still += l - pay > 0;
-            x = b.next[x];
-        }
-        alive += still;
-    }
-    __shared__ unsigned long long wg_alive;
-    if (threadIdx.x == 0) wg_alive = 0;
+    uint64_t carry = before;
+    for (int base = r.a; base < r.e; base += blockDim.x) {
+        const int v = base + static_cast<int>(threadIdx.x);
+        const uint64_t la = v < r.e ? b.len_a[v] : 0;
+        const uint64_t incl = wave_incl_scan(la, lane);
+        if (lane == 63) part[wv] = incl;
+        __syncthreads();
+        uint64_t ahead = 0, all = 0;
+        for (int w = 0; w < waves; w++) { if (w < wv) ahead += part[w]; all += part[w]; }
+        if (la) alive += emit_from(b, v, la, carry + ahead + incl - la, round, c0, v0);
+        carry += all;
+        __syncthreads();
+    }
     __syncthreads();
     if (alive) atomicAdd(&wg_alive, static_cast<unsigned long long>(alive));
     __syncthreads();
-    if (threadIdx.x == 0 && wg_alive) atomicAdd(reinterpret_cast<unsigned long long *>(&st->alive_after), wg_alive);
-}
-
-
-__global__ void dec_init_kernel(DecompBufs b, int64_t comp_cap, int64_t vert_cap, int n_flags, int allow_packed) { ph_init(b, whole_grid(), comp_cap, vert_cap, n_flags, allow_packed); }
+    if (threadIdx.x) return;
+    if (wg_alive) atomicAdd(reinterpret_cast<unsigned long long *>(&st->alive_after), wg_alive);
+    __threadfence();
+    if (atomicAdd(&st->ticket, 1u) != gridDim.x - 1) return;
+    __threadfence();
+    st->ticket = 0;
+    st->dead = atomicAdd(reinterpret_cast<unsigned long long *>(&st->alive_after), 0ull) == 0;
+    st->scan_total = total;
+    const int64_t n_comp = c0 + static_cast<int64_t>(total >> 40), n_vert = v0 + static_cast<int64_t>(total & kLenMask);
+    st->n_comp = n_comp; st->n_vert = n_vert;
+    if (n_comp <= st->comp_cap) b.o_off[n_comp] = n_vert;
+}
+
+__global__ void dec_init_kernel(DecompBufs b, int64_t comp_cap, int64_t vert_cap, int n_flags, int allow_packed, int need_packed)
+{
+    ph_init(b, whole_grid(), comp_cap, vert_cap, n_flags, allow_packed, need_packed);
+}
 __global__ void dec_round_begin_kernel(DecompBufs b, int reset_left) { ph_round_begin(b, whole_grid(), reset_left); }
 __global__ void dec_propose_hi_kernel(DecompBufs b, IterArgs a) { ph_propose_hi(b, whole_grid(), a); }
 __global__ void dec_propose_lo_kernel(DecompBufs b, IterArgs a) { ph_propose_lo(b, whole_grid(), a); }
 __global__ void dec_commit_kernel(DecompBufs b, IterArgs a) { ph_commit(b, whole_grid(), a); }
 __global__ void dec_heads_kernel(DecompBufs b, int round, int last_flag) { ph_heads(b, whole_grid(), round, last_flag); }
-__global__ void dec_cycles_kernel(DecompBufs b, int round) { ph_cycles(b, whole_grid(), round); }
-__global__ void dec_emit_kernel(DecompBufs b, int round) { ph_emit(b, whole_grid(), round, b.st->n_comp, b.st->n_vert); }
-
-__global__ void dec_round_end_kernel(DecompBufs b)
-{
-    DecompState *st = b.st;
-    if (blockIdx.x || threadIdx.x || st->dead) return;
-    st->dead = st->alive_after == 0;
-    st->n_comp += static_cast<int64_t>(st->scan_total >> 40);
-    st->n_vert += static_cast<int64_t>(st->scan_total & kLenMask);
-    if (st->n_comp <= st->comp_cap) b.o_off[st->n_comp] = st->n_vert;
-}
 
 size_t up256(size_t v) { return (v + 255) / 256 * 256; }
 
@@ -342,10 +401,11 @@
     b.nhi = c.take<uint64_t>(V); b.nlo = c.take<uint64_t>(V);
     b.bo_hi = c.take<uint64_t>(V); b.bi_hi = c.take<uint64_t>(V);
     b.bo_lo = c.take<uint64_t>(2 * V); b.bi_lo = c.take<uint64_t>(2 * V);
-    b.len_a = c.take<uint64_t>(V); b.pos = c.take<uint64_t>(V);
+    b.len_a = c.take<uint64_t>(V);
     b.pay = c.take<int64_t>(V);
     b.alive = c.take<uint8_t>(V); b.kind = c.take<uint8_t>(V);
     b.partials = c.take<uint64_t>(kDecompGrid + 1);
+    b.range_sums = c.take<uint64_t>(kMaxRangeParts);
     b.changed = c.take<uint32_t>(static_cast<size_t>(rounds) * static_cast<size_t>(iters));
     b.o_off = c.take<int64_t>(static_cast<size_t>(comp_cap) + 1);
     b.o_verts = c.take<int32_t>(static_cast<size_t>(vert_cap));
@@ -383,14 +443,14 @@
 constexpr int kWideGridDefault = 2048;
 inline dim3 wide_grid(const palace_ctx *ctx) { return dim3(ctx->match_grid > 0 ? ctx->match_grid : kWideGridDefault); }
 
-void enqueue_iterations(palace_ctx *ctx, const DecompBufs &b, int first, int n, uint64_t *count, int flag0, bool unique_hi)
+void enqueue_iterations(palace_ctx *ctx, const DecompBufs &b, int first, int n, uint64_t *count, int flag0, bool unique_hi, bool no_lo)
 {
     for (int k = 0; k < n; k++) {
         IterArgs a{((1ull << 21) - 1 - *count) << kStampShift, static_cast<uint64_t>((kPackedStamps - 1 - *count) & (kPackedStamps - 1)) << kPackedShift,
                    (first + k) & 1, k ? flag0 + k - 1 : -1, flag0 + k, unique_hi ? 1 : 0};
         (*count)++;
         hipLaunchKernelGGL(dec_propose_hi_kernel, wide_grid(ctx), kBlock, 0, ctx->stream, b, a);
-        if (!unique_hi) hipLaunchKernelGGL(dec_propose_lo_kernel, wide_grid(ctx), kBlock, 0, ctx->stream, b, a);
+        if (!unique_hi && !no_lo) hipLaunchKernelGGL(dec_propose_lo_kernel, wide_grid(ctx), kBlock, 0, ctx->stream, b, a);
         hipLaunchKernelGGL(dec_commit_kernel, wide_grid(ctx), kBlock, 0, ctx->stream, b, a);
     }
 }
@@ -399,33 +459,33 @@
 {
     hipLaunchKernelGGL(dec_heads_kernel, wide_grid(ctx), kBlock, 0, ctx->stream, b, round, last_flag);
     hipLaunchKernelGGL(dec_cycles_kernel, wide_grid(ctx), kBlock, 0, ctx->stream, b, round);
-    int rc = scan_u64(ctx, b.len_a, b.pos, &b.st->V, b.partials, &b.st->scan_total);
-    if (rc) return rc;
     hipLaunchKernelGGL(dec_emit_kernel, wide_grid(ctx), kBlock, 0, ctx->stream, b, round);
-    hipLaunchKernelGGL(dec_round_end_kernel, dim3(1), dim3(64), 0, ctx->stream, b);
     PALACE_HIP_TRY(hipGetLastError());
     return PALACE_OK;
 }
 
 }
 
-int decomp_begin(palace_ctx *ctx, const DecompBufs &b, int rounds, int64_t comp_cap, int64_t vert_cap)
+int decomp_begin(palace_ctx *ctx, const DecompBufs &b, DecompRun &run, int rounds, int64_t comp_cap, int64_t vert_cap, bool unique_hi)
 {
     PALACE_REQUIRE(rounds >= 1 && rounds <= kMaxRounds, "round count out of range");
     static_assert(kDecompGrid <= kDecompBlock, "scan_prefix_kernel scans the block sums with one workgroup");
     const int allow_packed = !ctx->match_two_word_keys && static_cast<int64_t>(rounds) * kMaxIters < kPackedStamps ? 1 : 0;
-    hipLaunchKernelGGL(dec_init_kernel, wide_grid(ctx), kBlock, 0, ctx->stream, b, comp_cap, vert_cap, rounds * kMaxIters, allow_packed);
+    run = DecompRun{};
+    run.no_lo = !unique_hi && allow_packed && b.kc && b.pack_bad;
+    hipLaunchKernelGGL(dec_init_kernel, wide_grid(ctx), kBlock, 0, ctx->stream, b, comp_cap, vert_cap, rounds * kMaxIters, allow_packed,
+                       run.no_lo ? 1 : 0);
     PALACE_HIP_TRY(hipGetLastError());
     return PALACE_OK;
 }
 
 int decomp_rounds(palace_ctx *ctx, const DecompBufs &b, int t0, int t1, int rounds, int aggressive, int iters, bool unique_hi,
-                  uint64_t *count)
+                  bool no_lo, uint64_t *count)
 {
     PALACE_REQUIRE(0 <= t0 && t0 <= t1 && t1 <= rounds && rounds <= kMaxRounds && iters >= 1 && iters <= kMaxIters, "round / iteration count out of range");
     for (int t = t0; t < t1; t++) {
         hipLaunchKernelGGL(dec_round_begin_kernel, wide_grid(ctx), kBlock, 0, ctx->stream, b, (aggressive && t == rounds - 1) ? 1 : 0);
-        enqueue_iterations(ctx, b, 0, iters, count, t * kMaxIters, unique_hi);
+        enqueue_iterations(ctx, b, 0, iters, count, t * kMaxIters, unique_hi, no_lo);
         int rc = enqueue_read_off(ctx, b, t, t * kMaxIters + iters - 1);
         if (rc) return rc;
     }
@@ -438,13 +498,13 @@
 {
     PALACE_REQUIRE(rounds >= 1 && rounds <= kMaxRounds, "round count out of range");
     constexpr int kBatch = 16;
-    hipLaunchKernelGGL(dec_init_kernel, wide_grid(ctx), kBlock, 0, ctx->stream, b, comp_cap, vert_cap, kBatch, 0);
+    hipLaunchKernelGGL(dec_init_kernel, wide_grid(ctx), kBlock, 0, ctx->stream, b, comp_cap, vert_cap, kBatch, 0, 0);
     uint64_t count = 0;
     for (int t = 0; t < rounds; t++) {
         hipLaunchKernelGGL(dec_round_begin_kernel, wide_grid(ctx), kBlock, 0, ctx->stream, b, (aggressive && t == rounds - 1) ? 1 : 0);
         for (int first = 0;; first += kBatch) {
             PALACE_HIP_TRY(hipMemsetAsync(b.changed, 0, kBatch * sizeof(uint32_t), ctx->stream));
-            enqueue_iterations(ctx, b, first, kBatch, &count, 0, unique_hi);
+            enqueue_iterations(ctx, b, first, kBatch, &count, 0, unique_hi, false);
             uint32_t last = 0;
             PALACE_HIP_TRY(hipMemcpyAsync(&last, b.changed + kBatch - 1, sizeof last, hipMemcpyDeviceToHost, ctx->stream));
             PALACE_HIP_TRY(hipStreamSynchronize(ctx->stream));
@@ -467,7 +527,7 @@
     const int t0 = run.next_round, t1 = std::min(rounds, t0 + (t0 == 0 ? first : kRoundsPerGroup));
     for (int t = t0; t < t1; t++) {
         const int iters = ctx->match_iters > 0 ? std::min(ctx->match_iters, kMaxIters) : (t == 0 ? kFirstRoundIters : kLaterRoundIters);
-        int rc = decomp_rounds(ctx, b, t, t + 1, rounds, aggressive, iters, unique_hi, &run.count);
+        int rc = decomp_rounds(ctx, b, t, t + 1, rounds, aggressive, iters, unique_hi, run.no_lo, &run.count);
         if (rc) return rc;
     }
     run.next_round = t1;
@@ -481,6 +541,7 @@
         PALACE_HIP_TRY(hipMemcpyAsync(h_state, b.st, sizeof *h_state, hipMemcpyDeviceToHost, ctx->stream));
         PALACE_HIP_TRY(hipStreamSynchronize(ctx->stream));
         if (h_state->unsettled) {
+            run.redone = true;
             int rc = reset_left();
             if (rc) return rc;
             rc = decomp_run_checked(ctx, b, rounds, aggressive, unique_hi, comp_cap, vert_cap, max_iterations);
diff --git a/palace_amd/csrc/decomp.hpp b/palace_amd/csrc/decomp.hpp
--- a/palace_amd/csrc/decomp.hpp
+++ b/palace_amd/csrc/decomp.hpp
@@ -20,6 +20,7 @@
 constexpr int kDecompBlock = 256;
 constexpr int kMaxRounds = 1024;
 constexpr int kMaxIters = 64;
+constexpr int kMaxRangeParts = 2048;
 
 struct DecompState {
     int32_t S, V;
@@ -28,9 +29,10 @@
     int64_t comp_cap, vert_cap;
     uint32_t unsettled;
     uint32_t overflow;
-    uint32_t bad;
+    uint32_t stalled;
     uint32_t dead;
     uint32_t packed;
+    uint32_t ticket;
     uint64_t scan_total;
     int64_t alive_after;
 };
@@ -48,10 +50,11 @@
     uint64_t *nhi = nullptr, *nlo = nullptr;
     uint64_t *bo_hi = nullptr, *bi_hi = nullptr;
     uint64_t *bo_lo = nullptr, *bi_lo = nullptr;
-    uint64_t *len_a = nullptr, *pos = nullptr;
+    uint64_t *len_a = nullptr;
     int64_t *pay = nullptr;
     uint8_t *alive = nullptr, *kind = nullptr;
     uint64_t *partials = nullptr;
+    uint64_t *range_sums = nullptr;
     uint32_t *changed = nullptr;
     int64_t *o_off = nullptr;
     int32_t *o_verts = nullptr, *o_iter = nullptr, *o_open = nullptr;
@@ -61,11 +64,11 @@
 size_t decomp_bytes(int64_t s_cap, int64_t e_cap, int64_t comp_cap, int64_t vert_cap, int rounds, int iters);
 void decomp_carve(DecompBufs &b, char *base, int64_t s_cap, int64_t e_cap, int64_t comp_cap, int64_t vert_cap, int rounds, int iters);
 constexpr int kFirstRoundIters = 7, kLaterRoundIters = 4, kRoundsPerGroup = 5, kFirstGroupRounds = 5;
-int decomp_begin(palace_ctx *ctx, const DecompBufs &b, int rounds, int64_t comp_cap, int64_t vert_cap);
+struct DecompRun { int next_round = 0; uint64_t count = 0; bool no_lo = false, redone = false; };
+int decomp_begin(palace_ctx *ctx, const DecompBufs &b, DecompRun &run, int rounds, int64_t comp_cap, int64_t vert_cap, bool unique_hi);
 int decomp_rounds(palace_ctx *ctx, const DecompBufs &b, int t0, int t1, int rounds, int aggressive, int iters, bool unique_hi,
-                  uint64_t *count);
+                  bool no_lo, uint64_t *count);
 
-struct DecompRun { int next_round = 0; uint64_t count = 0; };
 int decomp_group(palace_ctx *ctx, const DecompBufs &b, DecompRun &run, int rounds, int aggressive, bool unique_hi);
 int decomp_finish(palace_ctx *ctx, const DecompBufs &b, DecompRun &run, int rounds, int aggressive, bool unique_hi, int64_t comp_cap,
                   int64_t vert_cap, int64_t max_iterations, DecompState *h_state, const std::function<int()> &reset_left);
diff --git a/palace_amd/csrc/filter.hip b/palace_amd/csrc/filter.hip
--- a/palace_amd/csrc/filter.hip
+++ b/palace_amd/csrc/filter.hip
@@ -115,7 +115,7 @@
     if (kept) atomicAdd(reinterpret_cast<unsigned long long *>(&f.fs->n_kept2), static_cast<unsigned long long>(kept));
 }
 
-__global__ void st4_pass3_kernel(F f, const palace_graph_edge *__restrict__ edges)
+__device__ void pass3_body(const F &f, const palace_graph_edge *__restrict__ edges)
 {
     const int64_t n = f.fs->n_edges;
     int64_t kept = 0;
@@ -132,7 +132,7 @@
     if (kept) atomicAdd(reinterpret_cast<unsigned long long *>(&f.fs->n_kept3), static_cast<unsigned long long>(kept));
 }
 
-__global__ void st4_paths_kernel(F f)
+__device__ void paths_body(const F &f)
 {
     for (int64_t p = gtid(); p < f.n_paths; p += gsize()) {
         const int64_t a = f.path_off[p], b = f.path_off[p + 1];
@@ -149,6 +149,12 @@
         if (backed > 0 && (static_cast<double>(backed) / static_cast<double>(total) >= 0.5 || backed > 2000))
             for (int64_t k = a; k < b; k++) f.resc[f.path_tok[k] >> 1] = 1;
     }
+}
+
+__global__ void st4_pass3_paths_kernel(F f, const palace_graph_edge *__restrict__ edges)
+{
+    pass3_body(f, edges);
+    paths_body(f);
 }
 
 __global__ void st4_order_kernel(F f)
@@ -352,6 +358,17 @@
     for (int i = gtid(); i < n; i += gsize()) f.scan_in[i] = f.has_arc[i];
 }
 
+__device__ void bare_body(const F &f)
+{
+    const int n = f.fs->S_f, words = (n + 63) / 64;
+    for (int w = gtid(); w < words; w += gsize()) {
+        uint64_t bits = 0;
+        for (int k = 0; k < 64 && w * 64 + k < n; k++)
+            if (!f.has_arc[w * 64 + k]) bits |= 1ull << k;
+        f.bare[w] = bits;
+    }
+}
+
 __global__ void st4_sub_kernel(F f, DecompBufs b, const int32_t *__restrict__ cn)
 {
     FilterState *fs = f.fs;
@@ -381,6 +398,7 @@
         }
     }
     if (gtid() == 0) { b.st->S = n_sub; b.st->V = 2 * n_sub; b.st->E = n_arcs; }
+    bare_body(f);
 }
 
 __global__ void st4_left_kernel(F f, DecompBufs b, const int32_t *__restrict__ cn)
@@ -390,16 +408,6 @@
         if (f.has_arc[i]) b.left[static_cast<int32_t>(f.scan_out[i])] = max(1, cn[f.contig_of[i]]);
 }
 
-__global__ void st4_bare_kernel(F f)
-{
-    const int n = f.fs->S_f, words = (n + 63) / 64;
-    for (int w = gtid(); w < words; w += gsize()) {
-        uint64_t bits = 0;
-        for (int k = 0; k < 64 && w * 64 + k < n; k++)
-            if (!f.has_arc[w * 64 + k]) bits |= 1ull << k;
-        f.bare[w] = bits;
-    }
-}
 
 size_t up(size_t v) { return (v + 255) / 256 * 256; }
 uint64_t pow2_at_least(uint64_t v) { uint64_t p = 1024; while (p < v) p <<= 1; return p; }
@@ -603,8 +611,7 @@
         hipStream_t st = ctx->stream;
         hipLaunchKernelGGL(st4_begin_kernel, kG, kB, 0, st, f, d_n_edges, edge_bound);
         hipLaunchKernelGGL(st4_pass2_kernel, kG, kB, 0, st, f, d_edges);
-        hipLaunchKernelGGL(st4_pass3_kernel, kG, kB, 0, st, f, d_edges);
-        hipLaunchKernelGGL(st4_paths_kernel, kG, kB, 0, st, f);
+        hipLaunchKernelGGL(st4_pass3_paths_kernel, kG, kB, 0, st, f, d_edges);
         hipLaunchKernelGGL(st4_order_kernel, kG, kB, 0, st, f);
         PALACE_HIP_TRY(hipGetLastError());
         int rc2 = scan_u64(ctx, f.scan_in, f.scan_out, &f.fs->n_segs, s->b.partials, &f.fs->scan_total);
@@ -633,7 +640,6 @@
     int rc = scan_u64(ctx, f.scan_in, f.scan_out, &f.fs->S_f, s->b.partials, &f.fs->scan_total);
     if (rc) return rc;
     hipLaunchKernelGGL(st4_sub_kernel, kG, kB, 0, st, f, s->b, s->d_cn);
-    hipLaunchKernelGGL(st4_bare_kernel, kG, kB, 0, st, f);
     PALACE_HIP_TRY(hipGetLastError());
     return PALACE_OK;
 }
@@ -651,8 +657,7 @@
     s->f.use_paths = use_paths ? 1 : 0;
     int rc = enqueue_match(ctx, s, d_edges, use_paths != 0);
     if (rc) return rc;
-    s->run = DecompRun{};
-    if ((rc = decomp_begin(ctx, s->b, rounds, s->comp_cap, s->vert_cap))) return rc;
+    if ((rc = decomp_begin(ctx, s->b, s->run, rounds, s->comp_cap, s->vert_cap, false))) return rc;
     if ((rc = decomp_group(ctx, s->b, s->run, rounds, s->aggressive, false))) return rc;
     PALACE_HIP_TRY(hipMemcpyAsync(s->h_fs, s->f.fs, sizeof(FilterState), hipMemcpyDeviceToHost, ctx->stream));
     s->rounds = std::max(s->rounds, rounds);
@@ -692,6 +697,11 @@
         PALACE_HIP_TRY(hipMemcpyAsync(h_edge_flags, s->f.edge_flags, static_cast<size_t>(n_edges), hipMemcpyDeviceToHost, ctx->stream));
     PALACE_HIP_TRY(hipStreamSynchronize(ctx->stream));
     return PALACE_OK;
+}
+
+int palace_stage04_redone(const palace_stage04 *s)
+{
+    return s && s->matched && s->run.redone ? 1 : 0;
 }
 
 int palace_stage04_result(palace_ctx *ctx, palace_stage04 *s, palace_match_result **out, const int32_t **contig_of_out,
diff --git a/palace_amd/csrc/match.hip b/palace_amd/csrc/match.hip
--- a/palace_amd/csrc/match.hip
+++ b/palace_amd/csrc/match.hip
@@ -244,8 +244,8 @@
     auto fail = [&](int code) { (void)hipStreamSynchronize(st); return code; };
     hipError_t e = hipSuccess;
     if ((rc = upload())) return fail(rc);
-    if ((rc = decomp_begin(ctx, b, rounds, comp_cap, vert_cap))) return fail(rc);
     DecompRun run;
+    if ((rc = decomp_begin(ctx, b, run, rounds, comp_cap, vert_cap, true))) return fail(rc);
     if ((rc = decomp_group(ctx, b, run, rounds, aggressive, true))) return fail(rc);
     auto reset_left = [&]() -> int {
         PALACE_HIP_TRY(hipMemcpyAsync(b.left, p_left, static_cast<size_t>(S) * 8, hipMemcpyHostToDevice, st));
```

Result: no change. 111.9 million (-0.9%).
